# OpenGene/repaq

Hardware: AMD Instinct MI355X
Metric: raw FASTQ MB/s encode+decode (higher is better)
Workload: dtype u8; 1 GPU; configs[2]: synthetic NovaSeq PE150 two files (-i/-I), 2 x 4.01 GB FASTQ (fqgen profile 1, 11200000 pairs, seed 3, N 20 ppm), -k 1000, encode + decode; chunks_per_gpu=3360, parity=unchecked (checked with --full)

## Files before the change

### repaq_amd/csrc/enc/gather_tiles.h

```cpp
#pragma once
#define G2_CAP 23552u
#define G2_SE_OK 1
#define G2_CNT 256u
struct __attribute__((packed, aligned(1))) GU16g { uint32_t a, b, c, d; };
__device__ __forceinline__ void pack4_codes(uint32_t w, uint32_t& code, uint32_t& nb, uint32_t& bad) {
    const uint32_t idx = (w >> 1) & 0x03030303u;
    const uint32_t ok = eq_bytes_full(__builtin_amdgcn_perm(0u, 0x47544341u, idx), w);
    code = ((__builtin_amdgcn_perm(0u, 0x00020301u, idx) & ok) * 0x01041040u) >> 24;
    nb = 0; bad = 0;
    if (ok != 0xFFFFFFFFu) { const uint32_t isn = eq_bytes_full(w, 0x4E4E4E4Eu); nb = ((isn & 0x01010101u) * 0x01020408u) >> 24;
            bad = (((~ok & ~isn) & 0x01010101u) * 0x01020408u) >> 24; }
}
__device__ __forceinline__ void pack4_codes_rc(uint32_t w, uint32_t& code, uint32_t& nb) {
    const uint32_t u = w & 0xDFDFDFDFu, idx = (u >> 1) & 0x03030303u;
    const uint32_t ok = eq_bytes_full(__builtin_amdgcn_perm(0u, 0x47544341u, idx), u);
    code = ((__builtin_amdgcn_perm(0u, 0x03010002u, idx) & ok) * 0x01041040u) >> 24;
    nb = ((~ok & 0x01010101u) * 0x01020408u) >> 24;
}
__device__ __forceinline__ bool pack16_fast(const uint32_t (&w)[4], uint32_t& code) {
    uint32_t diff = 0; code = 0;
#pragma unroll
    for (int i = 0; i < 4; i++) {
        const uint32_t idx = (w[i] >> 1) & 0x03030303u;
        diff |= __builtin_amdgcn_perm(0u, 0x47544341u, idx) ^ w[i];
        code |= ((__builtin_amdgcn_perm(0u, 0x00020301u, idx) * 0x01041040u) >> 24) << (8 * i);
    }
    return diff == 0;
}
__device__ __forceinline__ uint32_t g2_rev2x16(uint32_t v) {
    v = bswap32(v); v = ((v >> 4) & 0x0F0F0F0Fu) | ((v & 0x0F0F0F0Fu) << 4); return ((v >> 2) & 0x33333333u) | ((v & 0x33333333u) << 2);
}
struct G2Geo { uint32_t a00, a01, end0, end1, base1; };
struct G2Read { bool on, rc; uint32_t len, qsrc, ssrc, qpos, ld, gi; };
struct G2Bound { uint32_t l0, l1, q; };
struct G2MRaw { uint4 lo4; uint32_t pg; };
#ifdef RFQ_SIMT_EMULATION
__device__ __forceinline__ uint32_t ld_uniform(const uint32_t* p) { return *p; }
#else
__device__ __forceinline__ uint32_t ld_uniform(const uint32_t* p) { return *(const __attribute__((address_space(4))) uint32_t*)(uintptr_t)p; }
#endif
__device__ __forceinline__ G2Bound g2_bound(const Text& T, bool two, const uint32_t* __restrict__ pq, uint32_t r) {
    G2Bound b;
    if (two) { const size_t k = 4 * (size_t)(r >> 1); b.l0 = ld_uniform(T.lo[0] + k); b.l1 = ld_uniform(T.lo[1] + k); }
    else { b.l0 = ld_uniform(T.lo[0] + 4 * (size_t)r); b.l1 = 0u; }
    b.q = ld_uniform(pq + r);
    return b;
}
__device__ __forceinline__ G2Geo g2_geo(const G2Bound& b, const G2Bound& e, bool two) {
    G2Geo g; g.a00 = b.l0 & ~15u; g.end0 = e.l0; g.a01 = two ? b.l1 & ~15u : 0u; g.end1 = two ? e.l1 : 0u;
    g.base1 = two ? (((g.end0 - g.a00 + 15u) & ~15u) + 16u) : 0u;
    return g;
}
__device__ __forceinline__ void g2_stage1(const uint8_t* __restrict__ fq, uint32_t n, uint32_t a0, uint32_t end, uint4* l4, uint32_t tid) {
    const uint32_t nb = end - a0, ng = (nb + 15u) / 16u;
    const uint8_t* src = fq + a0;
    const uint32_t nfull = (uint64_t)a0 + 16ull * ng <= (uint64_t)n ? ng : ng - 1u;
    for (uint32_t i = tid; i < nfull; i += blockDim.x)
        __builtin_amdgcn_global_load_lds((const __attribute__((address_space(1))) void*)(src + 16 * (size_t)i),
                (__attribute__((address_space(3))) void*)(l4 + (i - (tid & 63u))), 16, 0, 0);
    if (nfull < ng && tid == 0) { uint8_t* const bytes = (uint8_t*)l4;
            for (uint32_t k = 0; k < 16 && a0 + 16 * nfull + k < n; k++) bytes[16 * nfull + k] = src[16 * (size_t)nfull + k]; }
}
__device__ __forceinline__ void g2_stage(const Text& T, bool two, const G2Geo& g, uint4* buf4, uint32_t tid) {
    g2_stage1(T.fq[0], T.n[0], g.a00, g.end0, buf4, tid);
    if (two) g2_stage1(T.fq[1], T.n[1], g.a01, g.end1, buf4 + g.base1 / 16, tid);
}
__device__ __forceinline__ G2MRaw g2_mraw(const Text& T, const uint32_t* __restrict__ pq, uint32_t cur, uint32_t j, uint32_t cnt) {
    G2MRaw r; r.lo4 = make_uint4(0, 0, 0, 0); r.pg = 0;
    if (j < cnt) { const uint32_t gi = cur + j; int s_; uint32_t r_; read_loc(T, gi, s_, r_); r.lo4 = *(const uint4*)(t_lo(T, s_) + 4 * (size_t)r_); r.pg = pq[gi]; }
    return r;
}
__device__ __forceinline__ G2Read g2_read(const Text& T, const G2MRaw& r, const G2Geo& g, uint32_t f, uint32_t pq0, bool il, uint32_t cur, uint32_t j, uint32_t cnt) {
    G2Read m; m.on = j < cnt; m.rc = false; m.len = m.qsrc = m.ssrc = m.qpos = m.ld = 0; m.gi = cur + j;
    if (m.on) {
        const uint32_t gi = cur + j; int s_; uint32_t r_; read_loc(T, gi, s_, r_);
        const uint32_t lb = s_ ? g.base1 : 0u, a = s_ ? g.a01 : g.a00;
        m.len = r.lo4.z - 1u - r.lo4.y; m.ssrc = lb + (r.lo4.y - a); m.qsrc = lb + (r.lo4.w - a);
        m.qpos = r.pg - pq0; m.ld = (r.pg >> 4) + gi;
        m.rc = il && ((gi - f) & 1u);
    }
    return m;
}
__device__ __forceinline__ void g2_bases(const uint8_t* s_text, const G2Read& m, uint32_t part, uint32_t P, uint32_t* __restrict__ lpk, uint16_t* __restrict__ lnb,
        uint8_t* __restrict__ rflag, uint8_t* __restrict__ rn) {
    const uint32_t ng = (m.len + 15u) >> 4;
    for (uint32_t gi = part; gi < ng; gi += P) {
        uint32_t w[4], code = 0, nbits = 0;
        const uint32_t nv0 = m.len - 16u * gi;
        const bool tail = nv0 < 16u && m.len >= 16u; const uint32_t tsh = tail ? 16u - nv0 : 0u;
        auto blank = [&](uint32_t from, uint32_t to) { for (uint32_t k = from; k < to; k++) { uint32_t& x = w[k >> 2]; const uint32_t sh = 8u * (k & 3u);
                x = (x & ~(0xFFu << sh)) | (0x41u << sh); } };
        if (!m.rc) {
            lds_get16(s_text, m.ssrc + (tail ? m.len - 16u : 16u * gi), w);
            if (nv0 < 16u && !tail) blank(nv0, 16u);
            if (!pack16_fast(w, code)) {
                uint32_t bad = 0; code = 0;
#pragma unroll
                for (int i = 0; i < 4; i++) { uint32_t c4, n4, b4; pack4_codes(w[i], c4, n4, b4); code |= c4 << (8 * i); nbits |= n4 << (4 * i); bad |= b4 << (4 * i); }
                if (bad) rflag[m.gi] = 1;
            }
        } else {
            lds_get16(s_text, tail ? m.ssrc : m.ssrc + m.len - 16u * gi - 16u, w);
            if (nv0 < 16u && !tail) blank(0u, 16u - nv0);
            if (pack16_fast(w, code)) code = ~g2_rev2x16(code);
            else {
                const uint32_t x0 = bswap32(w[3]), x1 = bswap32(w[2]), x2 = bswap32(w[1]), x3 = bswap32(w[0]); w[0] = x0; w[1] = x1; w[2] = x2; w[3] = x3; code = 0;
#pragma unroll
                for (int i = 0; i < 4; i++) { uint32_t c4, n4; pack4_codes_rc(w[i], c4, n4); code |= c4 << (8 * i); nbits |= n4 << (4 * i); }
            }
        }
        code >>= 2u * tsh; nbits >>= tsh;
        if (nv0 < 16u) { code &= (1u << (2u * nv0)) - 1u; nbits &= (1u << nv0) - 1u; }
        lpk[m.ld + gi] = code; lnb[m.ld + gi] = (uint16_t)nbits;
        if (nbits) rn[m.gi] = 1;
    }
}
__device__ __forceinline__ void g2_compose(const uint8_t* s_text, const G2Read& m, uint32_t part, uint32_t P, uint8_t* qd, uint32_t* __restrict__ lpk,
        uint16_t* __restrict__ lnb, uint8_t* __restrict__ rflag, uint8_t* __restrict__ rn, QualCount& qc) {
    if (!m.on) return;
    {
        const uint32_t n = m.len; uint8_t* const o = qd + m.qpos; const bool rc = m.rc;
        if (n >= 16u) {
            const uint32_t ng = (n + 15u) >> 4;
            for (uint32_t gi = part; gi < ng; gi += P) {
                uint32_t p0 = 16u * gi, dup = 0; if (p0 + 16u > n) { dup = p0 + 16u - n; p0 = n - 16u; }
                uint32_t w[4]; lds_get16(s_text, rc ? m.qsrc + n - p0 - 16u : m.qsrc + p0, w);
                if (rc) { const uint32_t x0 = bswap32(w[3]), x1 = bswap32(w[2]), x2 = bswap32(w[1]), x3 = bswap32(w[0]); w[0] = x0; w[1] = x1; w[2] = x2; w[3] = x3; }
                { GU16g v; v.a = w[0]; v.b = w[1]; v.c = w[2]; v.d = w[3]; *(GU16g*)(o + p0) = v; }
                if (!dup) qc.group(m.qpos + p0, w[0], w[1], w[2], w[3]);
                else for (uint32_t k = dup; k < 16u; k++) qc(m.qpos + p0 + k, (uint8_t)(w[k >> 2] >> (8u * (k & 3u))));
            }
        } else for (uint32_t i = part; i < n; i += P) { const uint8_t q = s_text[rc ? m.qsrc + n - 1u - i : m.qsrc + i]; o[i] = q; qc(m.qpos + i, q); }
    }
    g2_bases(s_text, m, part, P, lpk, lnb, rflag, rn);
}
#define G2_REFN 256u
#define G2_REFS 128u
struct G2Ref { uint32_t nl, n1l, n2o, len, stl, lane, tile, nb, tb; int s; };
struct G2Acc { uint32_t bits, fail; };
__device__ __forceinline__ bool lane_bytes_eq(const uint8_t* tx, uint32_t a, uint32_t b, uint32_t n, bool on) {
    bool eq = true;
    for (uint32_t o = 0; __any(on && eq && o < n); o += 16u) {
        if (on && eq && o < n) {
            uint32_t p0 = o, v = n - o; if (v < 16u && n >= 16u) { p0 = n - 16u; v = 16u; }
// ... 54 lines not shown
        for (int p = 0; p < 4; p++) { uint32_t w[4]; lds_get16(tx, nsrc + 16u * (uint32_t)p, w); const uint4 q = make_uint4(w[0], w[1], w[2], w[3]);
                c[p] = eq_mask16c(q, 0x3A3A3A3Au); sp_[p] = eq_mask16c(q, 0x20202020u); }
        const unsigned long long keep = !on ? 0ull : (nl >= 64u ? ~0ull : (1ull << nl) - 1ull);
        Cm = ((((unsigned long long)(c[2] | (c[3] << 16))) << 32) | (c[0] | (c[1] << 16))) & keep;
        Sm = ((((unsigned long long)(sp_[2] | (sp_[3] << 16))) << 32) | (sp_[0] | (sp_[1] << 16))) & keep;
    }
    const uint32_t sp = ctz64_or64(Sm);
    unsigned long long cb = sp < 64u ? Cm & ((1ull << sp) - 1ull) : Cm;
    const uint32_t k = (uint32_t)__popcll(cb);
    uint32_t cpos[8];
#pragma unroll
    for (int i = 1; i <= 7; i++) { cpos[i] = ctz64_or64(cb); cb &= cb - 1ull; }
    const bool at7 = cpos[7] < 64u, at_sp = !at7 && sp < 64u;
    const bool undecided = on && !at7 && !at_sp && nl > 64u;
    uint32_t ok = 0, n1l = nl, n2o = nl, lane_v = 0, tile_v = 0, x_v = 0, y_v = 0;
    if (on && (at7 || (at_sp && k >= 4u))) {
        ok = 1; n2o = at7 ? cpos[7] : sp;
        const bool k4 = at_sp && k == 4u, k5 = at_sp && k == 5u;
        n1l = k4 ? cpos[4] : cpos[3];
        const uint32_t ls = (k4 ? cpos[4] : cpos[3]) + 1u, le = k4 ? sp : cpos[4];
        lane_v = g2_atoi(tx, nsrc + ls, le - ls) & 0xFFu;
        if (k >= 5u) { const uint32_t ts = (k5 ? cpos[5] : cpos[4]) + 1u, te = k5 ? sp : cpos[5]; tile_v = g2_atoi(tx, nsrc + ts, te - ts) & 0xFFFFu; }
        if (k >= 6u) x_v = g2_atoi(tx, nsrc + cpos[5] + 1u, cpos[6] - cpos[5] - 1u);
        if (at7) y_v = g2_atoi(tx, nsrc + cpos[6] + 1u, cpos[7] - cpos[6] - 1u);
        else if (k == 6u) y_v = g2_atoi(tx, nsrc + cpos[6] + 1u, sp - cpos[6] - 1u);
    }
    if (__any(undecided)) {
        if (undecided) { const Meta m = dev_parse_name(tx + nsrc, nl); ok = m.ok; n1l = m.name1_len; n2o = m.name2_off; lane_v = m.lane; tile_v = m.tile; x_v = m.x;
                y_v = m.y; }
    }
    if (on) { R.name1_len[gi] = n1l; R.name2_off[gi] = n2o; R.x[gi] = x_v; R.y[gi] = y_v; R.tile[gi] = (uint16_t)tile_v; R.lane[gi] = (uint8_t)lane_v;
            R.ok[gi] = (uint8_t)ok; }
    const uint32_t n2l = nl - n2o, n2l0 = r0.nl - r0.n2o;
    const uint8_t* g0n = t_fq(T, r0.s) + r0.nb; const uint8_t* g0s = t_fq(T, r0.s) + r0.tb;
    const bool st_eq = g2_eq_ref(tx, tsrc, refs, G2_REFS, g0s, 0u, r0.stl, tl, on && tl == r0.stl);
    const bool n1_eq = g2_eq_ref(tx, nsrc, refn, G2_REFN, g0n, 0u, r0.nl, n1l, on && n1l == r0.n1l);
    const bool n2_eq = g2_eq_ref(tx, nsrc + n2o, refn, G2_REFN, g0n, r0.n2o, r0.nl, n2l, on && n2l == n2l0);
    const uint32_t pn = wave_shr1(nsrc, 0u), pnl = wave_shr1(nl, 0u), pn2o = wave_shr1(n2o, 0u), plane = wave_shr1(lane_v, 0u), ptile = wave_shr1(tile_v,
            0u), px = wave_shr1(x_v, 0u), py = wave_shr1(y_v, 0u);
    const uint32_t rel = gi - f; const bool odd = on && can0 && (rel & 1u);
    bool fa = false;
    if (__any(odd)) {
        const uint32_t pn2l = pnl - pn2o; const bool same_len = odd && pn2l == n2l;
        if (odd && !same_len) fa = true;
        const uint32_t ma = pn + pn2o, mb = nsrc + n2o; const bool small = same_len && n2l <= 16u, big = same_len && !small;
        if (small && n2l) {
            uint32_t x[4], y[4]; lds_get16(tx, ma, x); lds_get16(tx, mb, y);
            if (dch != 0u && dpos < n2l) {
                const uint32_t sh = 8u * (dpos & 3u);
#pragma unroll
                for (int q = 0; q < 4; q++) if ((dpos >> 2) == (uint32_t)q) x[q] = (x[q] & ~(0xFFu << sh)) | (dch << sh);
            }
            unsigned long long dl = (((unsigned long long)(x[1] ^ y[1])) << 32) | (x[0] ^ y[0]), dh = (((unsigned long long)(x[3] ^ y[3])) << 32) | (x[2] ^ y[2]);
            if (n2l < 16u) { dl &= n2l >= 8u ? ~0ull : (1ull << (8u * n2l)) - 1ull; dh &= n2l > 8u ? (1ull << (8u * (n2l - 8u))) - 1ull : 0ull; }
            if (dl | dh) fa = true;
        }
        if (__any(big)) {
            if (!lane_bytes_eq(tx, ma, mb, dpos < n2l ? dpos : n2l, big)) fa = true;
            if (big && dpos < n2l) { if ((dch != 0u ? dch : (uint32_t)tx[ma + dpos]) != (uint32_t)tx[mb + dpos]) fa = true; }
            if (!lane_bytes_eq(tx, ma + dpos + 1u, mb + dpos + 1u, n2l > dpos + 1u ? n2l - dpos - 1u : 0u, big && dpos + 1u < n2l)) fa = true;
        }
    }
    if (on) {
        uint32_t b = 0;
        if (sl == r0.len) b |= 1u << 0;
        if (n1l == r0.n1l) b |= 1u << 1;
        if (n2l == n2l0) b |= 1u << 2;
        if (tl == r0.stl) b |= 1u << 3;
        if (tl == r0.stl && st_eq) b |= 1u << 4;
        if (lane_v == r0.lane) b |= 1u << 5;
        if (tile_v == r0.tile) b |= 1u << 6;
        if (n1l == r0.n1l && n1_eq) b |= 1u << 7;
        const bool e2 = n2l == n2l0 && n2_eq;
        if (e2) b |= 1u << 8;
        if (e2 || (rel & 1u)) b |= 1u << 9;
        acc.bits &= b;
        R.eq2[gi] = e2 ? 1 : 0;
        if (odd) {
            const bool fb = plane != lane_v || ptile != tile_v || px != x_v || py != y_v;
            if (fa || fb) { const uint32_t key = (rel << 1) | (fa ? 0u : 1u); if (key < acc.fail) acc.fail = key; }
        }
    }
}
#define G2_PLANES 5u
#define G2_PLANE_EXC 4u
#define G2_RARE_LIST 255u
struct G2Planes { uint32_t* planes; uint64_t pstride; uint32_t pw, nd; uint32_t* rare; };
__device__ __forceinline__ void g2_rare_or(uint32_t* __restrict__ gpl, uint64_t pstride, uint32_t* __restrict__ rare_c, uint32_t plane, uint32_t pos) {
    const uint32_t old = atomicOr(&gpl[(size_t)plane * pstride + (pos >> 5)], 1u << (pos & 31u));
    if (old == 0u) { const uint32_t k = atomicAdd(rare_c, 1u); if (k < G2_RARE_LIST) rare_c[1u + k] = (plane << 28) | (pos >> 5); }
}
__device__ __forceinline__ void g2_quals_masks(const uint8_t* tx, const G2Read& m, uint32_t part, uint32_t P, uint32_t* pl, uint32_t pw, uint32_t wbase, uint32_t nd,
                                               uint32_t pat0, uint32_t pat1, uint32_t pat2, uint32_t patm, const DevHeader* __restrict__ D, uint8_t* qd, uint32_t* __restrict__ gpl, uint64_t pstride,
                                               uint32_t* __restrict__ segm_c, int* __restrict__ segc_c, uint32_t n_seg, uint32_t* __restrict__ rare_c) {
    if (!m.on) return;
    const uint32_t n = m.len, ng = (n + 15u) >> 4; const bool rc = m.rc;
    for (uint32_t gi = part; gi < ng; gi += P) {
        const uint32_t p0 = 16u * gi, nv = n - p0;
        uint32_t w[4]; lds_get16(tx, rc ? m.qsrc + n - p0 - 16u : m.qsrc + p0, w);
        if (rc) { const uint32_t x0 = bswap32(w[3]), x1 = bswap32(w[2]), x2 = bswap32(w[1]), x3 = bswap32(w[0]); w[0] = x0; w[1] = x1; w[2] = x2; w[3] = x3; }
        const uint32_t valid = nv >= 16u ? 0xFFFFu : (1u << nv) - 1u;
        const uint4 q = make_uint4(w[0], w[1], w[2], w[3]);
        const uint32_t bit = m.qpos + p0 - wbase, wi = bit >> 5, sh = bit & 31u;
        uint32_t known = eq_mask16c(q, patm);
        auto plane = [&](uint32_t d, uint32_t pat) {
            const uint32_t mv = eq_mask16c(q, pat); known |= mv;
            const unsigned long long x = (unsigned long long)(mv & valid) << sh;
            if ((uint32_t)x) atomicOr(&pl[d * pw + wi], (uint32_t)x);
            if ((uint32_t)(x >> 32)) atomicOr(&pl[d * pw + wi + 1u], (uint32_t)(x >> 32));
        };
        if (nd > 0u) plane(0u, pat0);
        if (nd > 1u) plane(1u, pat1);
        if (nd > 2u) plane(2u, pat2);
        uint32_t rest = ~known & valid;
        while (rest) {
            const uint32_t k = (uint32_t)__ffs((int)rest) - 1u; rest &= rest - 1u;
            const uint32_t ww = k < 8u ? (k < 4u ? w[0] : w[1]) : (k < 12u ? w[2] : w[3]), pos = m.qpos + p0 + k, b = (ww >> (8u * (k & 3u))) & 0xFFu;
            const uint32_t j = D->stream_of[b];
            if (j < 4u && j < D->n_normal) { const size_t si = (size_t)j * n_seg + pos / PC_SEG_POS; g2_rare_or(gpl, pstride, rare_c, j, pos); atomicAdd(&segm_c[si], 1u);
                    atomicMax(&segc_c[si], (int)pos); }
            else { qd[pos] = (uint8_t)b; g2_rare_or(gpl, pstride, rare_c, G2_PLANE_EXC, pos); atomicAdd(&segm_c[(size_t)EXC_SLOT * n_seg + pos / PC_SEG_POS], 1u); }
        }
    }
}
__device__ __forceinline__ void g2_flush_masks(uint32_t* pl, uint32_t pw, uint32_t nd, uint32_t dense3 , uint32_t* s_carry, uint32_t* __restrict__ gpl, uint64_t pstride,
                                               uint32_t gw0, uint32_t nw, bool carry, bool or_first, bool or_last,
                                               size_t seg_index0 , uint32_t n_seg, uint32_t* __restrict__ segm, int* __restrict__ segc) {
    const uint32_t tid = threadIdx.x, seg0 = (gw0 << 5) / PC_SEG_POS;
    for (uint32_t d = 0; d < nd; d++) {
        const uint32_t v = (dense3 >> (8u * d)) & 0xFFu;
        uint32_t c01 = 0; int l0 = -1, l1 = -1;
        for (uint32_t i = tid; i < nw; i += blockDim.x) {
            const uint32_t x = pl[d * pw + i]; pl[d * pw + i] = 0u;
            const bool last = i + 1u == nw;
            if (last && carry) { s_carry[d] = x; continue; }
            const uint32_t gw = gw0 + i; uint32_t* const dst = gpl + (size_t)v * pstride + gw;
            if ((i == 0u && or_first) || (last && or_last)) { if (x) atomicOr(dst, x); } else *dst = x;
            if (x) { const uint32_t sg = ((gw << 5) / PC_SEG_POS) - seg0; const int lp = (int)((gw << 5) + 31u - (uint32_t)__clz((int)x));
                     c01 += (uint32_t)__popc(x) << (16u * sg); if (sg) { if (lp > l1) l1 = lp; } else if (lp > l0) l0 = lp; }
        }
        if (!carry && tid == 0) s_carry[d] = 0u;
        c01 = wave_sum(c01); l0 = wave_max(l0); l1 = wave_max(l1);
        if ((tid & 63u) == 0 && c01) {
            const size_t si = seg_index0 + (size_t)v * n_seg + seg0;
            if (c01 & 0xFFFFu) { atomicAdd(&segm[si], c01 & 0xFFFFu); atomicMax(&segc[si], l0); }
            if ((c01 >> 16) && seg0 + 1u < n_seg) { atomicAdd(&segm[si + 1u], c01 >> 16); atomicMax(&segc[si + 1u], l1); }
        }
    }
}
__global__ void k_mask_bounds(const uint32_t* __restrict__ pq, const uint32_t* __restrict__ first, const uint64_t* __restrict__ qbase, uint32_t* __restrict__ planes,
        uint64_t pstride, const DevHeader* __restrict__ D, uint32_t nd, uint32_t bx,
                              const uint32_t* __restrict__ only) {
    const uint32_t c = blockIdx.x; if (only && !only[c]) return;
    const uint32_t f = first[c], e = first[c + 1], pq0 = pq[f];
    uint32_t per = ((e - f) + bx - 1) / bx; per = (per + 1u) & ~1u;
    for (uint32_t b = 1u + threadIdx.x; b < bx; b += blockDim.x) {
        const uint32_t gs = f + b * per; if (gs >= e) break;
        const uint32_t w = (uint32_t)(qbase[c] >> 5) + ((pq[gs] - pq0) >> 5);
        for (uint32_t d = 0; d < nd; d++) planes[(size_t)D->dense[d] * pstride + w] = 0u;
    }
}
template <bool MASKS, int PAIRED = -1> __global__ void __launch_bounds__(256, 6) k_gather2(Text T_, ReadTab R, const uint32_t* __restrict__ first, const uint64_t* __restrict__ qbase,
                                                 const DevHeader* __restrict__ D, uint8_t* __restrict__ qcat, uint32_t* __restrict__ lpk, uint16_t* __restrict__ lnb, uint8_t* __restrict__ rflag,
                                                 uint8_t* __restrict__ rn, uint32_t* __restrict__ segm, int* __restrict__ segc, uint32_t n_seg, uint32_t kshift,
                                                 uint32_t* __restrict__ cbits, uint32_t* __restrict__ cfail, const uint32_t* __restrict__ only, uint32_t text4, G2Planes M) {
    Text T = T_; if (PAIRED >= 0) T.paired = PAIRED;
    constexpr bool PE = PAIRED != 0;
    RFQ_DYN_SHARED(uint4, g2_lds);
    __shared__ uint32_t sh[MASKS ? 1 : G2_CNT]; __shared__ int sh_last[MASKS ? 1 : G2_CNT]; __shared__ uint8_t s_slot[MASKS ? 16 : 256];
            __shared__ uint32_t s_r0[8], s_carry[4];
    const uint32_t REFN = (text4 - 1u) * 16u, REFS = REFN + G2_REFN + 16u;
    uint32_t* const pl = (uint32_t*)(g2_lds + text4 + (G2_REFN + G2_REFS + 32u) / 16u);
    const uint32_t c = blockIdx.y;
    const bool redo = only != nullptr;
    if (redo && !only[c]) return;
    const uint32_t tid = threadIdx.x;
    const uint32_t* __restrict__ pq = R.pq;
    const uint32_t nn_s = D->n_normal < NPOS_SLOT ? D->n_normal : NPOS_SLOT, nslot = nn_s + 1u;
    uint32_t nrep = 1;
    if (!MASKS) {
        for (uint32_t i = tid; i < G2_CNT; i += blockDim.x) { sh[i] = 0; sh_last[i] = -1; }
        while (nrep < 16u && 4u * nrep * nslot <= G2_CNT) nrep *= 2u;
        for (uint32_t i = tid; i < 256; i += blockDim.x) { const uint32_t j = D->stream_of[i]; s_slot[i] = (uint8_t)(j < nn_s ? j : nn_s); }
    } else {
        for (uint32_t i = tid; i < M.nd * M.pw; i += blockDim.x) pl[i] = 0u;
        if (tid < 4u) s_carry[tid] = 0u;
    }
    const uint32_t f = first[c], e = first[c + 1];
    const bool two = PE && T.paired == 1, can0 = PE && T.paired != 0 && D->support_interleaved != 0, il = can0 && !redo;
    const uint32_t dpos = D->name2_diff_pos, dch = D->name2_diff_char;
    uint8_t* const qd = qcat + qbase[c]; const uint32_t pq0 = pq[f];
    uint32_t per = ((e - f) + gridDim.x - 1) / gridDim.x; per = (per + 1u) & ~1u;
    const uint32_t gs = f + blockIdx.x * per, ge = gs + per < e ? gs + per : e;
    const uint32_t K = 1u << kshift, pshift = 8u - kshift, P = 1u << pshift;
    const uint32_t jj = tid >> pshift, j = ((jj << 1) & (K - 1u)) | (jj >> (kshift - 1u)), part = tid & (P - 1u);
    QualCount qc; qc.cnt = sh; qc.last = sh_last; qc.slot = s_slot; qc.major = D->major & 0xFFu; qc.seg0 = 0; qc.nslot = nslot; qc.rep = tid & (nrep - 1u);
            qc.hot_ok = D->stream_of[D->major & 0xFFu] == 0xFF;
    const uint32_t nd = MASKS ? M.nd : 0u, dense3 = (uint32_t)D->dense[0] | ((uint32_t)D->dense[1] << 8) | ((uint32_t)D->dense[2] << 16);
    const uint32_t pat0 = (uint32_t)D->normal[dense3 & 0xFFu] * 0x01010101u, pat1 = (uint32_t)D->normal[(dense3 >> 8) & 0xFFu] * 0x01010101u, pat2 = (uint32_t)D->normal[(dense3 >> 16) & 0xFFu] * 0x01010101u, patm = (D->major & 0xFFu) * 0x01010101u;
    uint32_t* const gpl = M.planes + (MASKS ? (size_t)(qbase[c] >> 5) : (size_t)0);
    uint4* const buf4 = g2_lds + 1; const uint8_t* const tx = (const uint8_t*)buf4;
    G2Ref r0 = {}; G2Acc acc; acc.bits = CF_ALL; acc.fail = 0xFFFFFFFFu;
    const bool parse = !redo && gs < ge;
    if (parse) {
        uint32_t r_; read_loc(T, f, r0.s, r_); const uint32_t* p = t_lo(T, r0.s) + 4 * (size_t)r_;
        const uint32_t p0 = p[0], p1 = p[1], p2 = p[2], p3 = p[3];
        r0.nb = p0; r0.nl = p1 - 1u - p0; r0.len = p2 - 1u - p1; r0.tb = p2; r0.stl = p3 - 1u - p2;
        uint8_t* const wr = (uint8_t*)buf4;
        if (tid < r0.nl) wr[REFN + tid] = t_fq(T, r0.s)[r0.nb + tid];
        if (tid < G2_REFS && tid < r0.stl) wr[REFS + tid] = t_fq(T, r0.s)[r0.tb + tid];
        __syncthreads();
        if (tid == 0) {
            const Meta m0 = r0.nl <= G2_REFN ? dev_parse_name(tx + REFN, r0.nl) : dev_parse_name(t_fq(T, r0.s) + r0.nb, r0.nl);
            s_r0[0] = m0.name1_len; s_r0[1] = m0.name2_off; s_r0[2] = m0.lane; s_r0[3] = m0.tile;
        }
    }
    __syncthreads();
    if (parse) { r0.n1l = s_r0[0]; r0.n2o = s_r0[1]; r0.lane = s_r0[2]; r0.tile = s_r0[3]; }
    uint32_t tix = blockIdx.x + blockIdx.y;
    const uint32_t ntile = gs < ge ? (ge - gs + K - 1u) >> kshift : 0u;
    auto tile_at = [&](uint32_t t_) -> uint32_t { const uint32_t x = gs + (t_ << kshift); return x < ge ? x : ge; };
    G2Bound b0 = g2_bound(T, two, pq, tile_at(0)), b1 = g2_bound(T, two, pq, tile_at(1)), b2 = g2_bound(T, two, pq, tile_at(2));
    G2MRaw mr = g2_mraw(T, pq, gs, j, ntile ? tile_at(1) - gs : 0u);
    if (ntile) g2_stage(T, two, g2_geo(b0, b1, two), buf4, tid);
    for (uint32_t t = 0; t < ntile; t++, tix++) {
        const uint32_t cur = tile_at(t), cnt = tile_at(t + 1u) - cur;
        const G2Geo g = g2_geo(b0, b1, two);
        const G2Read m = g2_read(T, mr, g, f, pq0, il, cur, j, cnt);
        const uint32_t qbeg = b0.q - pq0, qend = b1.q - pq0;
        { const uint32_t ncur = tile_at(t + 1u); mr = g2_mraw(T, pq, ncur, j, tile_at(t + 2u) - ncur); }
        const G2Bound b3 = g2_bound(T, two, pq, tile_at(t + 3u));
        __syncthreads();
        qc.seg0 = qbeg / PC_SEG_POS;
        if (parse && (uint32_t)wave_id() == (tix & 3u)) g2_parse(T, R, tx, REFN, REFS, g, r0, f, cur, cnt, can0, dpos, dch, acc);
        if (MASKS) {
            if (tid < nd && s_carry[tid]) atomicOr(&pl[tid * M.pw], s_carry[tid]);
            g2_quals_masks(tx, m, part, P, pl, M.pw, qbeg & ~31u, nd, pat0, pat1, pat2, patm, D, qd, gpl, M.pstride, segm + (size_t)c * MAX_STREAMS * n_seg,
                    segc + (size_t)c * MAX_STREAMS * n_seg, n_seg, M.rare + (size_t)c * (1u + G2_RARE_LIST));
            g2_bases(tx, m, part, P, lpk, lnb, rflag, rn);
        } else g2_compose(tx, m, part, P, qd, lpk, lnb, rflag, rn, qc);
        __syncthreads();
        if (t + 1u < ntile) g2_stage(T, two, g2_geo(b1, b2, two), buf4, tid);
        if (MASKS) {
            const uint32_t gw0 = qbeg >> 5, nw = ((qend + 31u) >> 5) - gw0; const bool last_tile = cur + cnt >= ge;
            g2_flush_masks(pl, M.pw, nd, dense3, s_carry, gpl, M.pstride, gw0, nw, !last_tile && (qend & 31u) != 0u, cur == gs && gs > f && (qbeg & 31u) != 0u,
                    last_tile && ge < e && (qend & 31u) != 0u,
                           (size_t)c * MAX_STREAMS * n_seg, n_seg, segm, segc);
        } else qual_flush(sh, sh_last, nrep, nslot, qc.seg0, c, nn_s, segm, segc, n_seg);
        b0 = b1; b1 = b2; b2 = b3;
    }
    if (parse) {
        const uint32_t bits = wave_and(acc.bits), fail = wave_min(acc.fail);
        if ((tid & 63u) == 0) { if (bits != CF_ALL) atomicAnd(&cbits[c], bits); if (fail != 0xFFFFFFFFu) atomicMin(&cfail[c], fail); }
    }
}
__device__ __forceinline__ uint32_t dense_mask_of(const DevHeader* __restrict__ D, uint32_t nd) { uint32_t m = 0;
        for (uint32_t d = 0; d < nd; d++) m |= 1u << D->dense[d]; return m; }
__device__ __forceinline__ void k_rare_zero_chunk(uint32_t* __restrict__ planes, uint64_t pstride, uint32_t dense_mask, const uint32_t* __restrict__ pq,
        const uint32_t* __restrict__ first, const uint64_t* __restrict__ qbase, uint32_t c) {
    const uint32_t nw = (pq[first[c + 1]] - pq[first[c]] + 31u) >> 5; const size_t w0 = (size_t)(qbase[c] >> 5);
    for (uint32_t v = 0; v < G2_PLANES; v++) if (!((dense_mask >> v) & 1u)) for (uint32_t i = threadIdx.x; i < nw; i += blockDim.x) planes[(size_t)v * pstride + w0 + i] = 0u;
}
__global__ void k_gather_redo_reset(const uint32_t* __restrict__ only, uint32_t* __restrict__ segm, int* __restrict__ segc, uint32_t n_seg,
                                    uint32_t* __restrict__ xplane, uint64_t pstride, const DevHeader* __restrict__ D, uint32_t nd, const uint32_t* __restrict__ pq, const uint32_t* __restrict__ first, const uint64_t* __restrict__ qbase) {
    const uint32_t c = blockIdx.x; if (!only[c]) return;
    const size_t k = (size_t)c * MAX_STREAMS * n_seg;
    for (uint32_t i = threadIdx.x; i < MAX_STREAMS * n_seg; i += blockDim.x) { segm[k + i] = 0u; segc[k + i] = -1; }
    if (xplane) { k_rare_zero_chunk(xplane, pstride, dense_mask_of(D, nd), pq, first, qbase, c);
            if (threadIdx.x == 0) xplane[(size_t)G2_PLANES * pstride + (size_t)c * (1u + G2_RARE_LIST)] = 0u; }
}
__global__ void k_rare_cleanup(uint32_t* __restrict__ rare, uint32_t* __restrict__ planes, uint64_t pstride, const DevHeader* __restrict__ D, uint32_t nd,
        const uint32_t* __restrict__ pq, const uint32_t* __restrict__ first, const uint64_t* __restrict__ qbase) {
    const uint32_t c = blockIdx.x; uint32_t* const rc = rare + (size_t)c * (1u + G2_RARE_LIST); const uint32_t n = rc[0]; if (!n) return;
    if (n <= G2_RARE_LIST) { const size_t w0 = (size_t)(qbase[c] >> 5); for (uint32_t i = threadIdx.x; i < n; i += blockDim.x) { const uint32_t e = rc[1u + i];
            planes[(size_t)(e >> 28) * pstride + w0 + (e & 0x0FFFFFFFu)] = 0u; } }
    else k_rare_zero_chunk(planes, pstride, dense_mask_of(D, nd), pq, first, qbase, c);
    __syncthreads();
    if (threadIdx.x == 0) rc[0] = 0u;
}
__device__ __forceinline__ uint32_t loose_codes(const uint32_t* __restrict__ lpk, uint32_t ld, uint32_t b) {
    const uint32_t d = ld + (b >> 4), sh = 2u * (b & 15u); const uint32_t lo = lpk[d];
    return sh ? (uint32_t)(((((unsigned long long)lpk[d + 1]) << 32) | lo) >> sh) : lo;
}
__device__ __forceinline__ uint32_t loose_nbits(const uint16_t* __restrict__ lnb, uint32_t ld, uint32_t b) {
    const uint32_t d = ld + (b >> 4), sh = b & 15u; const uint32_t lo = lnb[d];
    return (sh ? ((((uint32_t)lnb[d + 1]) << 16) | lo) >> sh : lo) & 0xFFFFu;
}
#define SP_OWN 4096u
#define SP_EXTRA 8u
#define SP_U 3
struct __attribute__((packed, aligned(4))) SpU8 { uint32_t a, b; };
struct __attribute__((packed, aligned(2))) SpU4 { uint32_t a; };
__global__ void __launch_bounds__(256) k_seqpack(const uint32_t* __restrict__ pq, const uint32_t* __restrict__ sd, const U4* __restrict__ ptot,
        const uint32_t* __restrict__ first, const uint32_t* __restrict__ ilv, const int8_t* __restrict__ ovb,
                                                 const DevHeader* __restrict__ D, const uint64_t* __restrict__ sbase, const uint32_t* __restrict__ lpk, const uint16_t* __restrict__ lnb, const uint8_t* __restrict__ rn,
                                                 uint32_t* __restrict__ spk, uint16_t* __restrict__ snm, uint32_t* __restrict__ ncount, uint32_t* __restrict__ nmap, uint32_t* __restrict__ segm, int* __restrict__ segc, uint32_t n_seg,
                                                 uint32_t rshift) {
    __shared__ uint32_t s_sd[256 + SP_EXTRA + 1], s_ld[256 + SP_EXTRA], s_sk[256 + SP_EXTRA]; __shared__ uint8_t s_own[SP_OWN];
    __shared__ uint8_t s_hn[256 + SP_EXTRA + 8];
    const uint32_t c = blockIdx.y, f = first[c], e = first[c + 1], tid = threadIdx.x;
    const uint32_t ps0 = sd[f], S = ptot[c].d;
    const bool il = ilv[c] != 0, enc = il && (D->flags & H_PE_OVERLAP); const int shift = D->overlap_shift;
    uint32_t* const ok = spk + (size_t)(sbase[c] >> 4); uint16_t* const on = snm + (size_t)(sbase[c] >> 4);
    const uint32_t nshift = nmap_shift(S); uint32_t* const nm = nmap + (size_t)c * NMAP_WORDS;
    const size_t nsi = ((size_t)c * MAX_STREAMS + NPOS_SLOT) * n_seg;
    uint32_t nsum = 0;
    auto skip_of = [&](uint32_t g) -> uint32_t {
        if (enc && ((g - f) & 1u)) { const int ov = (int)ovb[g >> 1] - shift; if (ov > 0) return (uint32_t)ov; }
        return 0u;
    };
    const uint32_t R = 1u << rshift;
    for (uint32_t r0 = f + blockIdx.x * R; r0 < e; r0 += gridDim.x * R) {
        const uint32_t nr = e - r0 < R ? e - r0 : R, nx = e - r0 < R + SP_EXTRA ? e - r0 : R + SP_EXTRA;
        for (uint32_t t = tid; t <= nx; t += blockDim.x) {
            const uint32_t g = r0 + t; s_sd[t] = g < e ? sd[g] - ps0 : S;
            if (t < nx) { s_ld[t] = (pq[g] >> 4) + g; s_sk[t] = skip_of(g); s_hn[t] = rn[g]; } else s_hn[t] = 0;
        }
        __syncthreads();
        const uint32_t kbase = (s_sd[0] + 15u) >> 4, kend = (s_sd[nr] + 15u) >> 4;
        if (tid < nr) { const uint32_t ka = (s_sd[tid] + 15u) >> 4, kb = (s_sd[tid + 1] + 15u) >> 4; for (uint32_t k = ka; k < kb; k++) s_own[k - kbase] = (uint8_t)tid; }
        __syncthreads();
        const uint32_t ndw = kend - kbase;
        for (uint32_t i0 = 0; i0 < ndw; i0 += blockDim.x * SP_U) {
            struct Dw { uint32_t k, need, t1, jj, sh, sh2, take2, n, n2; unsigned long long c, c2; } q[SP_U]; uint32_t nres[SP_U];
#pragma unroll
            for (int u = 0; u < SP_U; u++) nres[u] = 0;
#pragma unroll
            for (int u = 0; u < SP_U; u++) {
                Dw& x = q[u]; x.need = 0; x.take2 = 0; x.k = x.t1 = x.jj = x.sh = x.sh2 = x.n = x.n2 = 0; x.c = x.c2 = 0;
                const uint32_t i = i0 + (uint32_t)u * blockDim.x + tid;
                if (i < ndw) {
                    const uint32_t k = kbase + i, j = s_own[i];
                    const uint32_t B = 16u * k, si = B - s_sd[j], need = S - B < 16u ? S - B : 16u, av = s_sd[j + 1] - B, t1 = need < av ? need : av;
                    const uint32_t b0 = s_sk[j] + si, d = s_ld[j] + (b0 >> 4);
                    x.k = k; x.need = need; x.t1 = t1; x.sh = b0 & 15u; x.jj = j + 1u;
                    { const SpU8 v = *(const SpU8*)(lpk + d); x.c = (((unsigned long long)v.b) << 32) | v.a; x.n = s_hn[j] ? ((const SpU4*)(lnb + d))->a : 0u; }
// ... 104 lines not shown
```

### repaq_amd/csrc/enc/index.h

```cpp
#pragma once
__device__ __forceinline__ uint32_t eq_mask4(uint32_t w, uint32_t pat) {
    uint32_t v = w ^ pat;
    uint32_t t = ~(((v & 0x7F7F7F7Fu) + 0x7F7F7F7Fu) | v | 0x7F7F7F7Fu);
    return (((t >> 7) * 0x00204081u) >> 21) & 0xFu;
}
__device__ __forceinline__ uint32_t eq_flags4(uint32_t w, uint32_t pat) { const uint32_t v = w ^ pat; return ~(((v & 0x7F7F7F7Fu) + 0x7F7F7F7Fu) | v | 0x7F7F7F7Fu); }
__device__ __forceinline__ uint32_t eq_mask8(uint32_t a, uint32_t b, uint32_t pat) {
    return udot4(eq_flags4(b, pat), 0x80402010u, udot4(eq_flags4(a, pat), 0x08040201u, 0u)) >> 7;
}
__device__ __forceinline__ uint32_t eq_mask16c(const uint4& q, uint32_t pat) {
    const uint32_t lo = udot4(eq_flags4(q.y, pat), 0x80402010u, udot4(eq_flags4(q.x, pat), 0x08040201u, 0u));
    const uint32_t hi = udot4(eq_flags4(q.w, pat), 0x80402010u, udot4(eq_flags4(q.z, pat), 0x08040201u, 0u));
    return ((hi << 8) | lo) >> 7;
}
__device__ __forceinline__ uint32_t has_byte16(const uint4& q, uint32_t pat) {
    const uint32_t a = q.x ^ pat, b = q.y ^ pat, c = q.z ^ pat, d = q.w ^ pat;
    return (((a - 0x01010101u) & ~a) | ((b - 0x01010101u) & ~b) | ((c - 0x01010101u) & ~c) | ((d - 0x01010101u) & ~d)) & 0x80808080u;
}
__device__ __forceinline__ uint32_t eq_mask16(const uint4& q, uint32_t pat) {
    return eq_mask4(q.x, pat) | (eq_mask4(q.y, pat) << 4) | (eq_mask4(q.z, pat) << 8) | (eq_mask4(q.w, pat) << 12);
}
__global__ void k_nl_bitmap(const uint8_t* __restrict__ fq, uint32_t n, uint32_t skip, uint64_t* __restrict__ bitmap, uint32_t* __restrict__ blkcnt, DevStatus* st) {
    const uint64_t w = (uint64_t)blockIdx.x * 256 + threadIdx.x;
    const uint64_t base = w * 64;
// ... 31 lines not shown
typedef __attribute__((address_space(1))) unsigned long long nlf_gu64;
__device__ __forceinline__ void nlf_store(unsigned long long* p, unsigned long long v) { __hip_atomic_store((nlf_gu64*)p, v, __ATOMIC_RELAXED, __HIP_MEMORY_SCOPE_AGENT);
        }
__device__ __forceinline__ unsigned long long nlf_load(const unsigned long long* p) { return __hip_atomic_load((nlf_gu64*)p, __ATOMIC_RELAXED, __HIP_MEMORY_SCOPE_AGENT);
        }
__device__ __forceinline__ void nlf_pause() { __builtin_amdgcn_s_sleep(2); }
#endif
template <int NLF_T> __global__ void __launch_bounds__(256) k_line_index(const uint8_t* __restrict__ fq, uint32_t n, uint32_t skip, uint32_t* __restrict__ lo,
        uint32_t lo_cap, unsigned long long* state,
                                                    uint32_t* ticket, uint32_t* total, DevStatus* st) {
    constexpr uint32_t NLF_BYTES = NLF_T * 16384u;
    __shared__ uint32_t s_blk, s_base, s_wave[4];
    if (threadIdx.x == 0) s_blk = atomicAdd(ticket, 1u);
    __syncthreads();
    const uint32_t blk = s_blk;
    const int lane = lane_id(), wv = wave_id();
    const uint64_t wbase = (uint64_t)blk * NLF_BYTES + (uint64_t)wv * (NLF_T * 4096u) + (uint32_t)lane * 64u;
    uint64_t m[NLF_T]; uint32_t incl[NLF_T], tsum[NLF_T]; bool cr = false;
#pragma unroll
    for (int k = 0; k < NLF_T; k++) {
        const uint64_t base = wbase + (uint32_t)k * 4096u;
        uint64_t mk = 0, crm = 0;
        if (base + 64 <= n) {
            const uint4* p = (const uint4*)(fq + base);
#pragma unroll
            for (int q4 = 0; q4 < 4; q4++) { uint4 q = p[q4]; mk |= (uint64_t)eq_mask16c(q, 0x0A0A0A0Au) << (16 * q4); crm |= has_byte16(q, 0x0D0D0D0Du); }
            if (base == 0 && skip && crm) { crm = 0; for (uint32_t i = skip; i < 64; i++) if (fq[i] == '\r') crm = 1ull << 63; }
        } else if (base < n) {
            for (uint32_t i = 0; i < 64 && base + i < n; i++) { uint8_t c = fq[base + i]; if (c == '\n') mk |= 1ull << i; if (c == '\r') crm |= 1ull << i; }
        }
        if (base == 0 && skip) { const uint64_t keep = ~((1ull << skip) - 1ull); mk &= keep; crm &= keep; }
        m[k] = mk; cr |= crm != 0;
    }
    if (__any(cr) && lane == 0) atomicOr(&st->err, (uint32_t)DE_HAS_CR);
    uint32_t wtot = 0;
#pragma unroll
    for (int k = 0; k < NLF_T; k++) { incl[k] = wave_incl_sum<uint32_t>((uint32_t)__popcll(m[k])); tsum[k] = wave_last(incl[k]); wtot += tsum[k]; }
    if (lane == 0) s_wave[wv] = wtot;
    __syncthreads();
    const uint32_t tot = s_wave[0] + s_wave[1] + s_wave[2] + s_wave[3];
    uint32_t wavebase = 0;
    for (int k = 0; k < wv; k++) wavebase += s_wave[k];
    if (threadIdx.x < 64) {
        if (lane == 0) nlf_store(&state[blk], ((blk == 0 ? 2ull : 1ull) << 62) | tot);
        uint32_t before = 0;
        if (blk) {
            int64_t newest = (int64_t)blk - 1;
            for (uint32_t spins = 0;;) {
                const int64_t j = newest - lane;
                const unsigned long long v = j >= 0 ? nlf_load(&state[j]) : (2ull << 62);
                const unsigned long long pm = __ballot((v >> 62) == 2), zm = __ballot((v >> 62) == 0);
                const int fp = pm ? __ffsll((long long)pm) - 1 : 63;
                const unsigned long long need = (2ull << fp) - 1ull;
                if (zm & need) {
                    if (++spins > NLF_SPINS) { if (lane == 0) atomicOr(&st->err, (uint32_t)DE_INDEX_RETRY); break; }
                    nlf_pause(); continue;
                }
                before += wave_sum<uint32_t>(lane <= fp ? (uint32_t)v : 0u);
                if (pm) break;
                newest -= 64;
            }
            if (lane == 0) nlf_store(&state[blk], (2ull << 62) | (unsigned long long)(uint32_t)(before + tot));
        }
        if (lane == 0) {
            s_base = before;
            if ((uint64_t)(blk + 1) * NLF_BYTES >= n) *total = before + tot;
        }
    }
    __syncthreads();
    uint32_t tbase = s_base + wavebase;
    if ((uint64_t)tbase + wtot + 1u > lo_cap) { if (wtot && lane == 0) atomicOr(&st->err, (uint32_t)DE_INDEX_RETRY); }
    else {
#pragma unroll
        for (int k = 0; k < NLF_T; k++) {
            uint64_t mk = m[k]; uint32_t rank = tbase + incl[k] - (uint32_t)__popcll(mk);
            const uint32_t base = (uint32_t)(wbase + (uint32_t)k * 4096u);
            while (mk) { const int b = __ffsll((long long)mk) - 1; mk &= mk - 1; lo[rank + 1] = base + (uint32_t)b + 1u; rank++; }
            tbase += tsum[k];
        }
    }
    if (blk == 0 && threadIdx.x == 0) lo[0] = skip;
}
__global__ void k_index_totals(const uint32_t* __restrict__ tot0, const uint32_t* __restrict__ tot1, const uint8_t* __restrict__ fq0, uint32_t n0, const uint8_t* __restrict__ fq1, uint32_t n1,
                               uint32_t* lo0, uint32_t* lo1, int final_batch, int paired, uint32_t unit_cap, uint32_t guess, DevStatus* st) {
    if (threadIdx.x || blockIdx.x) return;
    uint32_t rec[2] = { 0, 0 };
    for (int s = 0; s < (paired == 1 ? 2 : 1); s++) {
        const uint32_t nl = s ? *tot1 : *tot0, n = s ? n1 : n0; const uint8_t* fq = s ? fq1 : fq0; uint32_t* lo = s ? lo1 : lo0;
        const uint32_t unterm = (final_batch && n > 0 && fq[n - 1] != '\n') ? 1u : 0u;
        if (unterm) lo[nl + 1] = n + 1;
        st->idx_lines[s] = n ? nl + unterm : 0u; rec[s] = n ? (nl + unterm) / 4 : 0u;
    }
    uint32_t units = paired == 0 ? rec[0] : (paired == 1 ? (rec[0] < rec[1] ? rec[0] : rec[1]) : rec[0] / 2);
    if (units > unit_cap) units = unit_cap;
    st->idx_units_true = units; st->idx_units = units < guess ? units : guess;
    if (units > guess) atomicOr(&st->err, (uint32_t)DE_UNITS_GUESS);
}
__global__ void k_line_tail(uint32_t* lo, uint32_t n_newlines, uint32_t n, int unterminated) {
    if (threadIdx.x == 0 && blockIdx.x == 0 && unterminated) lo[n_newlines + 1] = n + 1;
}

#define FQ_BLOCK_BYTES (1u << 20)
struct NormIn { const uint8_t* fq; uint32_t n; uint64_t file_off, file_end; };
__device__ __forceinline__ bool norm_exc(const NormIn& c, uint32_t j) {
    const uint64_t e = c.file_off + j - 1;
    uint64_t bend = (e | (uint64_t)(FQ_BLOCK_BYTES - 1)) + 1; if (bend > c.file_end) bend = c.file_end;
    return !(e + 1 < bend - 1);
}
__device__ __forceinline__ bool norm_state_at(const NormIn& c, uint32_t j) {
    if (j == 0) return false;
    uint32_t k = 0; while (k < 4 && k < j && c.fq[j - 1 - k] == '\n') k++;
    bool st = (k < 4 && j - k > 0) ? c.fq[j - k - 1] == '\r' : false;
    for (uint32_t i = j - k; i < j; i++) { if (st && !norm_exc(c, i)) st = false; else st = true; }
    return st;
}
__global__ void k_norm_classify(NormIn c, uint64_t* __restrict__ tbits, uint64_t* __restrict__ sbits, uint32_t* __restrict__ blk_keep, uint32_t* __restrict__ blk_term) {
    const uint64_t w = (uint64_t)blockIdx.x * 256 + threadIdx.x; const uint64_t base = w * 64;
    uint64_t tm = 0, sm = 0; uint32_t valid = 0;
    if (base < c.n) {
        valid = (uint32_t)(c.n - base < 64 ? c.n - base : 64);
        bool st = norm_state_at(c, (uint32_t)base);
        for (uint32_t i = 0; i < valid; i++) {
            const uint8_t ch = c.fq[base + i];
            if (ch == '\r') { tm |= 1ull << i; st = true; }
            else if (ch == '\n') { if (st && !norm_exc(c, (uint32_t)base + i)) { sm |= 1ull << i; st = false; } else { tm |= 1ull << i; st = true; } }
            else st = false;
        }
        tbits[w] = tm; sbits[w] = sm;
    }
    uint32_t tk, tt; (void)block_excl_sum<uint32_t>(valid - (uint32_t)__popcll(sm), &tk); (void)block_excl_sum<uint32_t>((uint32_t)__popcll(tm), &tt);
    if (threadIdx.x == 0) { blk_keep[blockIdx.x] = tk; blk_term[blockIdx.x] = tt; }
}
__global__ void k_norm_emit(NormIn c, const uint64_t* __restrict__ tbits, const uint64_t* __restrict__ sbits, const uint32_t* __restrict__ keep_base,
        const uint32_t* __restrict__ term_base,
                            uint8_t* __restrict__ out, uint32_t* __restrict__ ot, uint32_t* __restrict__ onx) {
    const uint64_t w = (uint64_t)blockIdx.x * 256 + threadIdx.x; const uint64_t base = w * 64;
    uint64_t tm = 0, sm = 0; uint32_t valid = 0;
    if (base < c.n) { valid = (uint32_t)(c.n - base < 64 ? c.n - base : 64); tm = tbits[w]; sm = sbits[w]; }
    uint32_t kp = keep_base[blockIdx.x] + block_excl_sum<uint32_t>(valid - (uint32_t)__popcll(sm), (uint32_t*)nullptr);
    uint32_t tr = term_base[blockIdx.x] + block_excl_sum<uint32_t>((uint32_t)__popcll(tm), (uint32_t*)nullptr);
    for (uint32_t i = 0; i < valid; i++) {
        if ((sm >> i) & 1ull) continue;
        const bool t = ((tm >> i) & 1ull) != 0;
        out[kp++] = t ? (uint8_t)'\n' : c.fq[base + i];
        if (t) {
            const uint32_t pos = (uint32_t)base + i;
            bool sw = false;
            if (pos + 1 < c.n) sw = i + 1 < 64 ? ((sm >> (i + 1)) & 1ull) != 0 : (sbits[w + 1] & 1ull) != 0;
            ot[tr] = pos; onx[tr] = pos + 1 + (sw ? 1u : 0u); tr++;
        }
    }
}
__global__ void k_norm_tail(uint32_t* ot, uint32_t* onx, uint32_t n_terms, uint32_t n) {
    if (threadIdx.x == 0 && blockIdx.x == 0) { ot[n_terms] = n; onx[n_terms] = n; }
}
```

### repaq_amd/csrc/rfq_api.hip

```cpp
#include "rfq_ctx.h"
#include <cstring>
#include <algorithm>
#include <new>
#include <cstdlib>
#include <string>
#include <cerrno>

extern "C" const char* rfq_version(void) {
#ifdef RFQ_SIMT_EMULATION
    return "rfq_hip 0.1.0 simt-emulation (test build, not a product path)";
#else
    return "rfq_hip 0.1.0 gfx950";
#endif
}

static bool opt_num(const std::string& v, long long lo, long long hi, long long* out) {
    if (v.empty()) return false;
    errno = 0; char* end = nullptr; const long long x = strtoll(v.c_str(), &end, 10);
    if (errno || !end || *end || end == v.c_str() || x < lo || x > hi) return false;
    *out = x; return true;
}
extern "C" int rfq_set_option(rfq_ctx* c, const char* name, const char* value) {
    if (!c || !name) return RFQ_E_ARG;
    const std::string n = name, v = value ? value : ""; const bool set = !v.empty(); const RfqOpts d; long long num = 0;
#define RFQ_OPT_NUM(LO, HI, WHAT) if (set && !opt_num(v, LO, HI, &num)) return rfq_fail(c, RFQ_E_ARG, "%s is " WHAT " (got \"%s\")", name, v.c_str());
    if (n == "RFQ_GATHER") { if (set && v != "old" && v != "tile") return rfq_fail(c, RFQ_E_ARG, "RFQ_GATHER is old or tile"); c->opt.gather_old = v == "old"; }
    else if (n == "RFQ_QUAL") { if (set && v != "bytes" && v != "masks") return rfq_fail(c, RFQ_E_ARG, "RFQ_QUAL is bytes or masks"); c->opt.qual_bytes = v == "bytes"; }
    else if (n == "RFQ_CODER") { if (set && v != "list" && v != "mask") return rfq_fail(c, RFQ_E_ARG, "RFQ_CODER is list or mask");
            c->opt.coder = v == "list" ? 1 : (v == "mask" ? 2 : 0); }
    else if (n == "RFQ_INDEX") { if (set && v != "2pass" && v != "1pass") return rfq_fail(c, RFQ_E_ARG, "RFQ_INDEX is 2pass or 1pass"); c->opt.index_2pass = v == "2pass"; }
    else if (n == "RFQ_IDX_TILES") { if (set && v != "4" && v != "8" && v != "16") return rfq_fail(c, RFQ_E_ARG, "RFQ_IDX_TILES is 4, 8 or 16");
            c->opt.idx_tiles = set ? atoi(v.c_str()) : d.idx_tiles; }
    else if (n == "RFQ_STREAMS") { if (set && v != "1" && v != "2") return rfq_fail(c, RFQ_E_ARG, "RFQ_STREAMS is 1 or 2"); c->opt.one_stream = v == "1"; }
    else if (n == "RFQ_SLICE_BYTES") { RFQ_OPT_NUM(1024, 0xFFFFFFF0ll - 16, "a number of bytes in 1024 .. 2^32 - 32") c->opt.slice_bytes = set ? (size_t)num : 0; }
    else if (n == "RFQ_SLICE_BASES") { RFQ_OPT_NUM(1, 0xFFFFFFF0ll, "a number of bases in 1 .. 2^32 - 16") c->opt.slice_bases = set ? (uint64_t)num : 0; }
    else if (n == "RFQ_WALK") { if (set && v != "exact" && v != "guess") return rfq_fail(c, RFQ_E_ARG, "RFQ_WALK is guess or exact"); c->opt.walk_exact = v == "exact"; }
    else if (n == "RFQ_GW_SHIFT") { RFQ_OPT_NUM(4, 30, "4 .. 30") c->opt.gw_shift = set ? (int)num : d.gw_shift; }
    else if (n == "RFQ_MATERIALISE") { if (set && v != "0" && v != "1") return rfq_fail(c, RFQ_E_ARG, "RFQ_MATERIALISE is 0 or 1"); c->opt.materialise = v == "1"; }
    else if (n == "RFQ_TRACE") { if (set && v != "0" && v != "1") return rfq_fail(c, RFQ_E_ARG, "RFQ_TRACE is 0 or 1"); c->opt.trace = v == "1"; }
    else if (n == "RFQ_G2_PAD") { RFQ_OPT_NUM(0, 150000, "0 .. 150000 bytes of LDS") c->opt.g2_pad = set ? (uint32_t)num : 0u; }
    else if (n == "RFQ_SP_PAD") { RFQ_OPT_NUM(0, 150000, "0 .. 150000 bytes of LDS") c->opt.sp_pad = set ? (uint32_t)num : d.sp_pad; }
    else if (n == "RFQ_POS_SEG") { if (set && v != "1024" && v != "2048") return rfq_fail(c, RFQ_E_ARG, "RFQ_POS_SEG is 1024 or 2048"); c->opt.pos_seg = set ? atoi(v.c_str()) : 0; }
    else if (n == "RFQ_SPEC") { if (set && v != "0" && v != "1") return rfq_fail(c, RFQ_E_ARG, "RFQ_SPEC is 0 or 1"); c->opt.no_spec = v == "0"; }
    else return rfq_fail(c, RFQ_E_ARG, "unknown option %s", name);
#undef RFQ_OPT_NUM
    return RFQ_OK;
}
static const char* const RFQ_OPTION_NAMES[] = { "RFQ_GATHER", "RFQ_QUAL", "RFQ_CODER", "RFQ_INDEX", "RFQ_IDX_TILES", "RFQ_STREAMS", "RFQ_SLICE_BYTES", "RFQ_SLICE_BASES", "RFQ_WALK", "RFQ_GW_SHIFT", "RFQ_MATERIALISE", "RFQ_TRACE", "RFQ_G2_PAD", "RFQ_SP_PAD", "RFQ_POS_SEG", "RFQ_SPEC" };
extern "C" const char* rfq_option_name(int i) { return (i >= 0 && i < (int)(sizeof RFQ_OPTION_NAMES / sizeof RFQ_OPTION_NAMES[0])) ? RFQ_OPTION_NAMES[i] : nullptr; }
extern "C" int rfq_get_option(const rfq_ctx* c, const char* name, char* out, size_t cap) {
    if (!c || !name || !out || !cap) return RFQ_E_ARG;
    const std::string n = name; const RfqOpts& o = c->opt; const RfqOpts d; std::string v;
    if (n == "RFQ_GATHER") v = o.gather_old ? "old" : "";
    else if (n == "RFQ_QUAL") v = o.qual_bytes ? "bytes" : "";
    else if (n == "RFQ_CODER") v = o.coder == 1 ? "list" : (o.coder == 2 ? "mask" : "");
    else if (n == "RFQ_INDEX") v = o.index_2pass ? "2pass" : "";
    else if (n == "RFQ_IDX_TILES") v = o.idx_tiles != d.idx_tiles ? std::to_string(o.idx_tiles) : "";
    else if (n == "RFQ_STREAMS") v = o.one_stream ? "1" : "";
    else if (n == "RFQ_SLICE_BYTES") v = o.slice_bytes ? std::to_string(o.slice_bytes) : "";
    else if (n == "RFQ_SLICE_BASES") v = o.slice_bases ? std::to_string(o.slice_bases) : "";
    else if (n == "RFQ_WALK") v = o.walk_exact ? "exact" : "";
    else if (n == "RFQ_GW_SHIFT") v = o.gw_shift != d.gw_shift ? std::to_string(o.gw_shift) : "";
    else if (n == "RFQ_MATERIALISE") v = o.materialise ? "1" : "";
    else if (n == "RFQ_TRACE") v = o.trace ? "1" : "";
    else if (n == "RFQ_G2_PAD") v = o.g2_pad ? std::to_string(o.g2_pad) : "";
    else if (n == "RFQ_SP_PAD") v = o.sp_pad != d.sp_pad ? std::to_string(o.sp_pad) : "";
    else if (n == "RFQ_POS_SEG") v = o.pos_seg ? std::to_string(o.pos_seg) : "";
    else if (n == "RFQ_SPEC") v = o.no_spec ? "0" : "";
    else return RFQ_E_ARG;
    if (v.size() + 1 > cap) return RFQ_E_NOSPACE;
    memcpy(out, v.c_str(), v.size() + 1);
    return RFQ_OK;
}

extern "C" int rfq_create(rfq_ctx** out, int device_id) {
    if (!out) return RFQ_E_ARG;
    *out = nullptr;
    int n = 0;
    if (hipGetDeviceCount(&n) != hipSuccess || n <= 0) return RFQ_E_NO_DEVICE;
    if (device_id < 0 || device_id >= n) return RFQ_E_NO_DEVICE;
    if (hipSetDevice(device_id) != hipSuccess) return RFQ_E_NO_DEVICE;
    rfq_ctx* c = new (std::nothrow) rfq_ctx();
    if (!c) return RFQ_E_HIP;
    c->device = device_id;
    { int cu = 0; if (hipDeviceGetAttribute(&cu, hipDeviceAttributeMultiprocessorCount, device_id) == hipSuccess && cu > 0) c->n_cu = (uint32_t)cu; }
    if (hipStreamCreate(&c->stream) != hipSuccess) { delete c; return RFQ_E_NO_DEVICE; }
    c->own_stream = true;
    memset(&c->h_hdr, 0, sizeof c->h_hdr);
    for (const char* nm : RFQ_OPTION_NAMES) { const char* v = getenv(nm); if (v && *v && rfq_set_option(c, nm, v) != RFQ_OK) fprintf(stderr, "rfq_hip: ignoring %s=%s (%s)\n", nm, v, c->err.c_str()); }
    c->err.clear();
    *out = c;
    return RFQ_OK;
}

extern "C" void rfq_destroy(rfq_ctx* c) {
    if (!c) return;
    (void)hipSetDevice(c->device);
    (void)hipDeviceSynchronize();
    for (auto& b : c->b) b.release();
    c->d_hdr.release(); c->d_status.release(); c->d_cmp.release(); c->out_img.release(); c->out_fq1.release(); c->out_fq2.release(); c->out_acc.release();
            c->out_acc1.release(); c->out_acc2.release();
    for (auto& b : c->rows_off) b.release();
    for (auto& b : c->rows_txt) b.release();
    c->rows_stat.release(); c->names_blob.release(); c->names_off.release();
    c->timer.destroy();
    if (c->copy) { (void)hipStreamDestroy(c->copy); for (auto& e : c->copy_ev) if (e) (void)hipEventDestroy(e); }
    if (c->own_stream && c->stream) (void)hipStreamDestroy(c->stream);
    if (c->pin) (void)hipHostFree(c->pin);
    if (c->pin_up) (void)hipHostFree(c->pin_up);
    if (c->ev_up) (void)hipEventDestroy(c->ev_up);
    if (c->aux) (void)hipStreamDestroy(c->aux);
    if (c->ev_fork) (void)hipEventDestroy(c->ev_fork);
    if (c->ev_join) (void)hipEventDestroy(c->ev_join);
    if (c->ev_mid) (void)hipEventDestroy(c->ev_mid);
    if (c->aux2) (void)hipStreamDestroy(c->aux2);
    if (c->ev_f) (void)hipEventDestroy(c->ev_f);
    delete c;
}

extern "C" const char* rfq_last_error(const rfq_ctx* c) { return c ? c->err.c_str() : "null context"; }

extern "C" int rfq_set_stream(rfq_ctx* c, void* s) {
    if (!c) return RFQ_E_ARG;
    if (s) {
        if (c->own_stream && c->stream) (void)hipStreamDestroy(c->stream);
        c->stream = (hipStream_t)s; c->own_stream = false;
    } else if (!c->own_stream) {
        if (hipStreamCreate(&c->stream) != hipSuccess) return rfq_fail(c, RFQ_E_HIP, "hipStreamCreate failed");
        c->own_stream = true;
    }
    return RFQ_OK;
}

int rfq_upload_header(rfq_ctx* c, const uint8_t* h, size_t n);

extern "C" int rfq_set_header(rfq_ctx* c, const uint8_t* h, size_t n) {
    if (!c || !h) return RFQ_E_ARG;
    c->err.clear();
    return rfq_upload_header(c, h, n);
}
extern "C" int rfq_get_header(rfq_ctx* c, uint8_t* out, size_t* len) {
    if (!c || !out || !len) return RFQ_E_ARG;
    if (!c->have_hdr) return rfq_fail(c, RFQ_E_STATE, "no header has been made or set on this context");
    memcpy(out, c->h_hdr.bytes, c->h_hdr.len); *len = c->h_hdr.len;
    return RFQ_OK;
}
extern "C" void rfq_clear_header(rfq_ctx* c) { if (c) { c->have_hdr = false; c->hdr_on_device = false; c->new_file(); memset(&c->h_hdr, 0, sizeof c->h_hdr); } }

extern "C" int rfq_last_timings(const rfq_ctx* c, const char** names, float* ms, int cap) {
    if (!c) return 0;
    int n = 0;
// ... 155 lines not shown
```

### repaq_amd/csrc/rfq_common.h

```cpp
#pragma once
#include <hip/hip_runtime.h>
#include <stdint.h>
#include <stddef.h>

#define H_LANE        (1u << 0)
#define H_TILE        (1u << 1)
#define H_X           (1u << 2)
#define H_Y           (1u << 3)
#define H_NAME2       (1u << 4)
#define H_PAIRED      (1u << 5)
#define H_PE_OVERLAP  (1u << 6)
#define H_QUAL_BY_COL (1u << 7)
#define H_DONT_QUAL   (1u << 8)
#define H_N_POS       (1u << 9)
#define C_READ_LEN_SAME   (1u << 0)
#define C_NAME1_LEN_SAME  (1u << 1)
#define C_NAME2_LEN_SAME  (1u << 2)
#define C_STRAND_LEN_SAME (1u << 3)
#define C_LANE_SAME       (1u << 4)
#define C_TILE_SAME       (1u << 5)
#define C_NAME1_SAME      (1u << 6)
#define C_NAME2_SAME      (1u << 7)
#define C_STRAND_SAME     (1u << 8)
#define C_PE_INTERLEAVED  (1u << 9)
#define C_NO_LB           (1u << 10)
#define C_NO_LB_R2        (1u << 11)

#define WAVE 64
#define NL_BLOCK_BYTES 16384u
#define MAX_STREAMS 66
#define NPOS_SLOT 64
#define EXC_SLOT 65

#define DE_HAS_CR          (1u << 0)
#define DE_EMPTY_LINE      (1u << 1)
#define DE_QUAL_SHORT      (1u << 2)
#define DE_BAD_QUAL        (1u << 3)
#define DE_BAD_BASE        (1u << 4)
#define DE_COORD_RANGE     (1u << 5)
#define DE_QUAL_OVERFLOW   (1u << 6)
#define DE_NO_QUAL_BINS    (1u << 7)
#define DE_CORRUPT         (1u << 8)
#define DE_LIST_ALIAS      (1u << 28)
#define DE_E3_RETRY        (1u << 29)
#define DE_INDEX_RETRY     (1u << 30)
#define DE_CORRUPT_OV      (1u << 10)
#define DE_INTERNAL        (1u << 11)
#define DE_SCRATCH_SMALL   (1u << 12)
#define DE_SCRATCHN_SMALL  (1u << 13)
#define DE_NEED_SCAN       (1u << 14)
#define DE_UNITS_GUESS     (1u << 15)
#define DE_TAIL_BLANK      (1u << 9)

struct DevHeader {
    uint8_t  bytes[17 + 255];
    uint32_t len;
    uint32_t flags;
    uint32_t read_len_bytes;
    uint32_t support_interleaved;
    uint32_t name2_diff_pos, name2_diff_char;
    uint32_t n_base_qual;
    int32_t  overlap_shift;
    uint32_t major;
    uint32_t n_normal;
    uint8_t  normal[256];
    uint8_t  stream_of[256];
    uint8_t  is_exception[256];
    uint8_t  dense[4];
    uint32_t dense_valid;
    uint32_t valid;
};

struct DevStatus {
    uint32_t err;
    uint32_t err_read;
    uint64_t err_key;
    uint64_t coord_key;
    uint64_t total_scratch;
    uint64_t total_scratch_n;
    uint64_t image_bound;
    uint32_t n_chunks;
    uint32_t max_chunk_reads;
    uint32_t max_chunk_bases;
    uint32_t n_units_used;
    uint64_t total_image;
    uint64_t total_bases;
    uint32_t first_empty;
    uint32_t max_rec;
    uint32_t unit_bases;
    uint32_t max_len;
    uint32_t idx_lines[2], idx_units_true, idx_units;
};

struct U4 { uint32_t a, b, c, d; };
__device__ __host__ __forceinline__ U4 operator+(const U4& x, const U4& y) { U4 r; r.a = x.a + y.a; r.b = x.b + y.b; r.c = x.c + y.c; r.d = x.d + y.d; return r; }
__device__ __host__ __forceinline__ U4 operator-(const U4& x, const U4& y) { U4 r; r.a = x.a - y.a; r.b = x.b - y.b; r.c = x.c - y.c; r.d = x.d - y.d; return r; }

#ifdef RFQ_SIMT_EMULATION
#define RFQ_DYN_SHARED(type, name) type* const name = (type*)emu::dyn_shared()
#else
#define RFQ_DYN_SHARED(type, name) extern __shared__ type name[]
#endif

__device__ __forceinline__ int lane_id() { return (int)(threadIdx.x & 63u); }
__device__ __forceinline__ int wave_id() { return (int)(threadIdx.x >> 6); }

#ifdef RFQ_SIMT_EMULATION
template <class T> __device__ __forceinline__ T wave_incl_sum(T v) {
    const int l = lane_id();
#pragma unroll
    for (int d = 1; d < WAVE; d <<= 1) { T t = __shfl_up(v, (unsigned)d); if (l >= d) v = t + v; }
    return v;
}
template <class T> __device__ __forceinline__ T wave_incl_max(T v) {
    const int l = lane_id();
#pragma unroll
    for (int d = 1; d < WAVE; d <<= 1) { T t = __shfl_up(v, (unsigned)d); if (l >= d && t > v) v = t; }
    return v;
}
template <class T> __device__ __forceinline__ T wave_sum(T v) {
#pragma unroll
    for (int d = 32; d >= 1; d >>= 1) v += __shfl_xor(v, d);
    return v;
}
template <class T> __device__ __forceinline__ T wave_min(T v) {
#pragma unroll
    for (int d = 32; d >= 1; d >>= 1) { T t = __shfl_xor(v, d); if (t < v) v = t; }
    return v;
}
template <class T> __device__ __forceinline__ T wave_max(T v) {
#pragma unroll
    for (int d = 32; d >= 1; d >>= 1) { T t = __shfl_xor(v, d); if (t > v) v = t; }
    return v;
}
// ... 130 lines not shown
```

### repaq_amd/csrc/rfq_ctx.h

```cpp
#pragma once
#include "rfq_common.h"
#include "../../include/rfq_hip.h"
#include <cstring>
#include <string>
#include <vector>
#include <cstdio>
#include <cstdarg>
#include <algorithm>

struct DBuf {
    void* p = nullptr; size_t cap = 0;
    hipError_t ensure(size_t n) {
        if (n <= cap) return hipSuccess;
        if (p) { (void)hipFree(p); p = nullptr; cap = 0; }
        size_t want = n + n / 4 + 4096;
        hipError_t e = hipMalloc(&p, want);
        if (e != hipSuccess) { p = nullptr; return e; }
        cap = want; return hipSuccess;
    }
    hipError_t ensure_keep(size_t n, size_t keep, hipStream_t s) {
        if (n <= cap) return hipSuccess;
        void* q = nullptr; const size_t want = n + n / 2 + 4096;
        hipError_t e = hipMalloc(&q, want);
        if (e != hipSuccess) return e;
        if (p && keep) { e = hipMemcpyAsync(q, p, keep, hipMemcpyDeviceToDevice, s); if (e == hipSuccess) e = hipStreamSynchronize(s);
                if (e != hipSuccess) { (void)hipFree(q); return e; } }
        if (p) (void)hipFree(p);
        p = q; cap = want; return hipSuccess;
    }
    void release() { if (p) (void)hipFree(p); p = nullptr; cap = 0; }
    template <class T> T* as() const { return (T*)p; }
};

struct StageTimer {
    struct Stage { const char* name; hipEvent_t a, b; };
    std::vector<Stage> stages; size_t used = 0; std::vector<float> ms; std::vector<const char*> names;
    void reset() { used = 0; }
    void begin(const char* name, hipStream_t s) {
        if (used == stages.size()) { Stage st; st.name = name; (void)hipEventCreate(&st.a); (void)hipEventCreate(&st.b); stages.push_back(st); }
        stages[used].name = name; (void)hipEventRecord(stages[used].a, s);
    }
    void end(hipStream_t s) { (void)hipEventRecord(stages[used].b, s); used++; }
    void collect() {
        ms.assign(used, 0.f); names.assign(used, nullptr);
        for (size_t i = 0; i < used; i++) { (void)hipEventElapsedTime(&ms[i], stages[i].a, stages[i].b); names[i] = stages[i].name; }
    }
    void destroy() { for (auto& s : stages) { (void)hipEventDestroy(s.a); (void)hipEventDestroy(s.b); } stages.clear(); }
};
struct StageSums {
    std::vector<std::pair<const char*, float>> v;
    void add(const StageTimer& t) {
        for (size_t i = 0; i < t.names.size(); i++) {
            auto q = std::find_if(v.begin(), v.end(), [&](const std::pair<const char*, float>& e) { return e.first == t.names[i]; });
            if (q == v.end()) v.emplace_back(t.names[i], t.ms[i]); else q->second += t.ms[i];
        }
    }
    void publish(StageTimer& t) const { t.names.clear(); t.ms.clear(); for (auto& q : v) { t.names.push_back(q.first); t.ms.push_back(q.second); } }
};

static inline uint32_t grid_x_for(uint32_t n_chunks, uint32_t tiles_per_chunk, uint32_t slots) {
    uint32_t best = 1; double best_eff = 0.0;
    if (!n_chunks || !slots) return 1;
    for (uint32_t k = 6; k <= 12; k++) {
        uint32_t bx = (uint32_t)(((uint64_t)k * slots + n_chunks / 2) / n_chunks);
        bx = std::max<uint32_t>(1u, std::min<uint32_t>(std::max<uint32_t>(bx, 1u), tiles_per_chunk));
        const double rounds = (double)bx * n_chunks / slots, full = (double)(uint64_t)(rounds + 0.999999), eff = full > 0 ? rounds / full : 0.0;
        if (eff > best_eff + 1e-3) { best = bx; best_eff = eff; }
    }
    return best;
}
struct RfqOpts {
    int  coder = 0;
    bool qual_bytes = false;
    bool gather_old = false;
    bool index_2pass = false;
    int  idx_tiles = 0;
    bool one_stream = false;
    size_t slice_bytes = 0;
    uint64_t slice_bases = 0;
    bool walk_exact = false;
    int  gw_shift = 16;
    bool materialise = false;
    bool trace = false;
    uint32_t g2_pad = 0;
    uint32_t sp_pad = 0;
    bool no_spec = false;
    int  pos_seg = 0;
};
struct rfq_ctx {
    RfqOpts opt;
    bool e3_pieces_failed = false;
    int device = 0; uint32_t n_cu = 256;
    hipStream_t stream = nullptr; bool own_stream = false;
    hipStream_t aux = nullptr; hipEvent_t ev_fork = nullptr, ev_join = nullptr, ev_mid = nullptr;
    hipStream_t aux2 = nullptr; hipEvent_t ev_f = nullptr;
    hipEvent_t ev_ovl = nullptr;
    hipStream_t copy = nullptr; hipEvent_t copy_ev[64] = {}; uint64_t copy_next = 0, copy_done = 0;
    bool aux_ready() {
        if (aux) return true;
        if (hipStreamCreateWithFlags(&aux, hipStreamNonBlocking) != hipSuccess) { aux = nullptr; return false; }
        if (hipEventCreateWithFlags(&ev_fork, hipEventDisableTiming) != hipSuccess || hipEventCreateWithFlags(&ev_join, hipEventDisableTiming) != hipSuccess ||
            hipEventCreateWithFlags(&ev_mid, hipEventDisableTiming) != hipSuccess) return false;
        if (hipStreamCreateWithFlags(&aux2, hipStreamNonBlocking) != hipSuccess) { aux2 = nullptr; return false; }
        if (hipEventCreateWithFlags(&ev_f, hipEventDisableTiming) != hipSuccess) return false;
        if (hipEventCreateWithFlags(&ev_ovl, hipEventDisableTiming) != hipSuccess) return false;
        return true;
    }
    std::string err;
    uint8_t* pin = nullptr; size_t pin_cap = 0, pin_used = 0;
    struct Pend { void* host; size_t off, n; }; std::vector<Pend> pend;
    hipError_t fetch(void* host, const void* dev, size_t n, hipStream_t s) {
        if (!n) return hipSuccess;
        if (!pin) { if (hipHostMalloc((void**)&pin, 1 << 16, 0) != hipSuccess) { pin = nullptr; (void)hipGetLastError(); } else pin_cap = 1 << 16; }
        const size_t off = (pin_used + 15) & ~(size_t)15;
        if (!pin || off + n > pin_cap) return hipMemcpyAsync(host, dev, n, hipMemcpyDeviceToHost, s);
        pend.push_back(Pend{ host, off, n }); pin_used = off + n;
        return hipMemcpyAsync(pin + off, dev, n, hipMemcpyDeviceToHost, s);
    }
    hipError_t fetch_sync(hipStream_t s) {
        const hipError_t e = hipStreamSynchronize(s);
        if (e == hipSuccess) for (const Pend& q : pend) memcpy(q.host, pin + q.off, q.n);
        pend.clear(); pin_used = 0;
        return e;
    }
    DBuf d_hdr;
    DevHeader h_hdr; bool have_hdr = false;
    bool hdr_on_device = false; uint8_t* pin_up = nullptr; hipEvent_t ev_up = nullptr; bool ev_up_pending = false;
    DBuf d_status; DevStatus h_status;
    DBuf d_cmp;
    DBuf b[120];
    DBuf out_img, out_fq1, out_fq2, out_acc, out_acc1, out_acc2;
    double rec_per_byte = 0.0; bool lazy_block = false;
    bool retried_room = false;
    bool mixed_lengths = false;
    bool dense_ok = false;
    void new_file() { dense_ok = false; e3_pieces_failed = false; mixed_lengths = false; }
    bool qplane_dirty = true;
    uint32_t qplane_nd = 0, qplane_mask = 0;
    size_t qplane_stride = 0;
    DBuf rows_off[2], rows_stat, rows_txt[2];
    DBuf names_blob, names_off;
    std::vector<uint64_t> chunk_off;
    std::vector<uint64_t> scan_end[2];
    StageTimer timer;
};

static inline int rfq_fail(rfq_ctx* c, int code, const char* fmt, ...) {
    char buf[1024]; va_list ap; va_start(ap, fmt); vsnprintf(buf, sizeof buf, fmt, ap); va_end(ap);
    if (c) c->err = buf;
    return code;
}
#define HIPCHK(ctx, call) do { hipError_t e_ = (call); if (e_ != hipSuccess) return rfq_fail(ctx, RFQ_E_HIP, "%s failed: %s", #call, hipGetErrorString(e_)); } while (0)
#define KCHK(ctx, what) do { hipError_t e_ = hipGetLastError(); if (e_ != hipSuccess) return rfq_fail(ctx, RFQ_E_HIP, "launch of %s failed: %s", what, hipGetErrorString(e_)); } while (0)

#define SCAN_TPB 256
#define SCAN_ITEMS 8
#define SCAN_TILE (SCAN_TPB * SCAN_ITEMS)

template <class T> __global__ void k_scan_reduce(const T* __restrict__ in, T* __restrict__ partial, uint64_t n, const uint32_t* __restrict__ skip) {
    if (skip && *skip) return;
    const uint64_t base = (uint64_t)blockIdx.x * SCAN_TILE + (uint64_t)threadIdx.x;
    T v[SCAN_ITEMS];
#pragma unroll
    for (int i = 0; i < SCAN_ITEMS; i++) v[i] = base + (uint64_t)i * SCAN_TPB < n ? in[base + (uint64_t)i * SCAN_TPB] : T();
    T acc = T();
#pragma unroll
    for (int i = 0; i < SCAN_ITEMS; i++) acc = acc + v[i];
    T tot; (void)block_excl_sum<T>(acc, &tot);
    if (threadIdx.x == 0) partial[blockIdx.x] = tot;
}
template <class T> __global__ void k_scan_partials(T* __restrict__ partial, uint32_t nb, T* __restrict__ grand, const uint32_t* __restrict__ skip) {
    if (skip && *skip) return;
    const uint32_t K = (nb + SCAN_TPB - 1) / SCAN_TPB, i0 = threadIdx.x * K, i1 = i0 + K < nb ? i0 + K : nb;
    T acc = T();
    for (uint32_t i = i0; i < i1; i++) acc = acc + partial[i];
    T tot; T run = block_excl_sum<T>(acc, &tot);
    for (uint32_t i = i0; i < i1; i++) { const T v = partial[i]; partial[i] = run; run = run + v; }
    if (threadIdx.x == 0 && grand) *grand = tot;
}
template <class T> __global__ void k_scan_apply(const T* __restrict__ in, T* __restrict__ out, const T* __restrict__ partial, uint64_t n, int write_total, const uint32_t* __restrict__ skip) {
    if (skip && *skip) return;
    const uint64_t base = (uint64_t)blockIdx.x * SCAN_TILE + (uint64_t)threadIdx.x * SCAN_ITEMS;
    T v[SCAN_ITEMS]; T acc = T();
    for (int i = 0; i < SCAN_ITEMS; i++) { v[i] = base + i < n ? in[base + i] : T(); acc = acc + v[i]; }
    T tot; T ex = block_excl_sum<T>(acc, &tot);
    T run = partial[blockIdx.x] + ex;
    for (int i = 0; i < SCAN_ITEMS; i++) { if (base + i < n) out[base + i] = run; run = run + v[i]; }
    if (write_total && base < n && base + SCAN_ITEMS >= n) out[n] = run;
}
#define SCAN_SMALL 16384u
template <class T> __global__ void k_scan_small(const T* in, T* out, uint32_t n, int write_total, const uint32_t* __restrict__ skip) {
    if (skip && *skip) return;
    const uint32_t K = (n + SCAN_TPB - 1) / SCAN_TPB, i0 = threadIdx.x * K, i1 = i0 + K < n ? i0 + K : n;
    T acc = T();
    for (uint32_t i = i0; i < i1; i++) acc = acc + in[i];
    T tot; T run = block_excl_sum<T>(acc, &tot);
    for (uint32_t i = i0; i < i1; i++) { const T v = in[i]; out[i] = run; run = run + v; }
    if (write_total && threadIdx.x == 0) out[n] = tot;
}
template <class T> static inline void scan_exclusive(hipStream_t s, const T* in, T* out, uint64_t n, T* tmp, int write_total, const uint32_t* skip = nullptr) {
    if (n == 0) { if (write_total) (void)hipMemsetAsync(out, 0, sizeof(T), s); return; }
    if (n <= SCAN_SMALL) { hipLaunchKernelGGL((k_scan_small<T>), dim3(1), dim3(SCAN_TPB), 0, s, in, out, (uint32_t)n, write_total, skip); return; }
    const uint32_t nb = (uint32_t)((n + SCAN_TILE - 1) / SCAN_TILE);
    hipLaunchKernelGGL((k_scan_reduce<T>), dim3(nb), dim3(SCAN_TPB), 0, s, in, tmp, n, skip);
    hipLaunchKernelGGL((k_scan_partials<T>), dim3(1), dim3(SCAN_TPB), 0, s, tmp, nb, (T*)nullptr, skip);
    hipLaunchKernelGGL((k_scan_apply<T>), dim3(nb), dim3(SCAN_TPB), 0, s, in, out, (const T*)tmp, n, write_total, skip);
}

#define CLEAR_MAX 8
struct ClearList { uint32_t* p[CLEAR_MAX]; uint64_t words[CLEAR_MAX]; uint32_t val[CLEAR_MAX]; uint32_t n;
    bool add(void* p_, size_t bytes, uint32_t v) { if (n >= CLEAR_MAX) return false; p[n] = (uint32_t*)p_; words[n] = (bytes + 3) / 4; val[n] = v; n++; return true; } };
template <int UNUSED> __global__ void k_clear_list(ClearList z) {
    const uint64_t t0 = (uint64_t)blockIdx.x * blockDim.x + threadIdx.x, NT = (uint64_t)gridDim.x * blockDim.x;
    for (uint32_t r = 0; r < z.n; r++) {
        uint32_t* const p = z.p[r]; const uint32_t v = z.val[r]; const uint64_t n4 = z.words[r] >> 2;
        for (uint64_t i = t0; i < n4; i += NT) ((uint4*)p)[i] = make_uint4(v, v, v, v);
        for (uint64_t i = (n4 << 2) + t0; i < z.words[r]; i += NT) p[i] = v;
    }
}
// ... 5 lines not shown
```

### repaq_amd/csrc/rfq_encode.hip

```cpp
#include "rfq_ctx.h"
#include "rfq_encode_kernels.h"
#include <algorithm>
#include <cstring>
#include <cstdlib>
#include <cstddef>

enum EncBuf {
    B_BITMAP0 = 0, B_BITMAP1, B_BLK0, B_BLK1, B_LO0, B_LO1, B_SCANTMP,
    B_LEN, B_N1LEN, B_N2OFF, B_X, B_Y, B_TILE, B_LANE, B_OK, B_CHUNK, B_STORED, B_EQ2, B_PQ, B_PV, B_PVIN,
    B_ULEN, B_P, B_MINMAX, B_FIRST, B_CFLAGS, B_IL, B_HIST, B_NCOUNT, B_SCAP, B_SOFF, B_SSIZE, B_XSIZE, B_YSIZE, B_QBASE, B_SBASE,
    B_IMGSIZE, B_IMGOFF, B_CTOTAL, B_CBASE, B_LAYOUT, B_HSTATS, B_OVB, B_OVRAW, B_QCAT, B_SCAT, B_SCRATCH, B_XS, B_YS, B_SEGB, B_SEGC,
    B_NORM0, B_NORM1, B_OT0, B_OT1, B_ONX0, B_ONX1, B_TBITS, B_SBITS, B_NKEEP, B_NTERM, B_NMAP, B_ADJ, B_PINFO, B_SEGM, B_LPK, B_LNB, B_SPK, B_SNM, B_RFLAG, B_SCANTMP2, B_CTOTALN, B_CBASEN, B_SCRATCHN, B_PTOT, B_QPLANE, B_SEGD, B_SEGS, B_SD, B_RN, B_ENC_END
};

static_assert(B_ENC_END <= 80, "encode buffers must stay below the decode buffer indices of rfq_ctx::b");

static int fetch_bytes(rfq_ctx* ctx, const uint8_t* d, size_t n, std::string& out) {
    out.resize(n);
    if (n) HIPCHK(ctx, hipMemcpy(&out[0], d, n, hipMemcpyDeviceToHost));
    return RFQ_OK;
}
static int fetch_line(rfq_ctx* ctx, const Text& T, uint32_t g, int k, std::string& out) {
    int s = 0; uint32_t r = g; if (T.paired == 1) { s = (int)(g & 1u); r = g >> 1; }
    uint32_t lo2[2];
    HIPCHK(ctx, hipMemcpy(lo2, T.lo[s] + 4 * (size_t)r + k, 8, hipMemcpyDeviceToHost));
    return fetch_bytes(ctx, T.fq[s] + lo2[0], lo2[1] - 1 - lo2[0], out);
}

int rfq_upload_header(rfq_ctx* c, const uint8_t* h, size_t n) {
    if (n < 17) return rfq_fail(c, RFQ_E_FORMAT, "Not a valid repaq file!");
    if (h[8] != 2) return rfq_fail(c, RFQ_E_FORMAT, "The data is encoded by different version of repaq, please try repaq v%.5s. \nSee: https://github.com/OpenGene/repaq/releases", (const char*)h + 3);
    const size_t len = 17u + h[16];
    if (n < len) return rfq_fail(c, RFQ_E_FORMAT, "Not a valid repaq file!");
    if (h[0] != 'R' || h[1] != 'F' || h[2] != 'Q') return rfq_fail(c, RFQ_E_FORMAT, "Not a valid repaq file!");
    HIPCHK(c, hipSetDevice(c->device));
    HIPCHK(c, c->d_hdr.ensure(sizeof(DevHeader)));
    DevHeader tmp; memset(&tmp, 0, sizeof tmp); memcpy(tmp.bytes, h, len); hdr_derive(&tmp);
    const bool same = c->have_hdr && c->hdr_on_device && c->h_hdr.len == tmp.len && !memcmp(c->h_hdr.bytes, tmp.bytes, tmp.len);
    if (!same) {
        if (!c->pin_up) { if (hipHostMalloc((void**)&c->pin_up, sizeof(DevHeader), 0) != hipSuccess) { c->pin_up = nullptr; (void)hipGetLastError(); } }
        if (c->pin_up) {
            if (c->ev_up_pending) { HIPCHK(c, hipEventSynchronize(c->ev_up)); c->ev_up_pending = false; }
            if (!c->ev_up) HIPCHK(c, hipEventCreateWithFlags(&c->ev_up, hipEventDisableTiming));
            memcpy(c->pin_up, &tmp, sizeof tmp);
            HIPCHK(c, hipMemcpyAsync(c->d_hdr.p, c->pin_up, sizeof tmp, hipMemcpyHostToDevice, c->stream));
            HIPCHK(c, hipEventRecord(c->ev_up, c->stream)); c->ev_up_pending = true;
        } else { HIPCHK(c, hipMemcpyAsync(c->d_hdr.p, &tmp, sizeof tmp, hipMemcpyHostToDevice, c->stream)); HIPCHK(c, hipStreamSynchronize(c->stream)); }
        c->h_hdr = tmp; c->hdr_on_device = true;
    }
    c->have_hdr = true; c->new_file();
    return RFQ_OK;
}

struct NormMap { const uint32_t* ot[2]; const uint32_t* onx[2]; size_t orig_n[2]; };
#define RFQ_NEED_NORM 1
#define RFQ_RETRY_ROOM 3

static int normalize_stream(rfq_ctx* ctx, const uint8_t* fq, size_t n, uint64_t file_off, bool final, int s, NormMap& nm, const uint8_t** out, size_t* out_n) {
    hipStream_t S = ctx->stream; DBuf* B = ctx->b;
    nm.orig_n[s] = n; nm.ot[s] = nm.onx[s] = nullptr; *out = nullptr; *out_n = 0;
    if (n == 0) return RFQ_OK;
    const uint64_t nwords = (n + 63) / 64; const uint32_t nblk = (uint32_t)((nwords + 255) / 256);
    HIPCHK(ctx, B[B_TBITS].ensure(nwords * 8 + 64)); HIPCHK(ctx, B[B_SBITS].ensure(nwords * 8 + 64));
    HIPCHK(ctx, B[B_NKEEP].ensure(((size_t)nblk + 2) * 4)); HIPCHK(ctx, B[B_NTERM].ensure(((size_t)nblk + 2) * 4));
    HIPCHK(ctx, B[B_SCANTMP].ensure(std::max<size_t>(1024, ((size_t)nblk / SCAN_TILE + 2) * 16)));
    NormIn in; in.fq = fq; in.n = (uint32_t)n; in.file_off = file_off; in.file_end = final ? file_off + n : ~0ull;
    hipLaunchKernelGGL(k_norm_classify, dim3(nblk), dim3(256), 0, S, in, B[B_TBITS].as<uint64_t>(), B[B_SBITS].as<uint64_t>(), B[B_NKEEP].as<uint32_t>(),
            B[B_NTERM].as<uint32_t>());
    KCHK(ctx, "k_norm_classify");
    scan_exclusive<uint32_t>(S, B[B_NKEEP].as<uint32_t>(), B[B_NKEEP].as<uint32_t>(), nblk, B[B_SCANTMP].as<uint32_t>(), 1);
    scan_exclusive<uint32_t>(S, B[B_NTERM].as<uint32_t>(), B[B_NTERM].as<uint32_t>(), nblk, B[B_SCANTMP].as<uint32_t>(), 1);
    uint32_t keep = 0, terms = 0;
    HIPCHK(ctx, ctx->fetch(&keep, B[B_NKEEP].as<uint32_t>() + nblk, 4, S));
    HIPCHK(ctx, ctx->fetch(&terms, B[B_NTERM].as<uint32_t>() + nblk, 4, S));
    HIPCHK(ctx, ctx->fetch_sync(S));
    HIPCHK(ctx, B[B_NORM0 + s].ensure((size_t)keep + 64)); HIPCHK(ctx, B[B_OT0 + s].ensure(((size_t)terms + 4) * 4));
            HIPCHK(ctx, B[B_ONX0 + s].ensure(((size_t)terms + 4) * 4));
    hipLaunchKernelGGL(k_norm_emit, dim3(nblk), dim3(256), 0, S, in, (const uint64_t*)B[B_TBITS].as<uint64_t>(), (const uint64_t*)B[B_SBITS].as<uint64_t>(),
                       (const uint32_t*)B[B_NKEEP].as<uint32_t>(), (const uint32_t*)B[B_NTERM].as<uint32_t>(), B[B_NORM0 + s].as<uint8_t>(), B[B_OT0 + s].as<uint32_t>(), B[B_ONX0 + s].as<uint32_t>());
    hipLaunchKernelGGL(k_norm_tail, dim3(1), dim3(64), 0, S, B[B_OT0 + s].as<uint32_t>(), B[B_ONX0 + s].as<uint32_t>(), terms, (uint32_t)n);
    KCHK(ctx, "k_norm_emit");
    nm.ot[s] = B[B_OT0 + s].as<uint32_t>(); nm.onx[s] = B[B_ONX0 + s].as<uint32_t>();
    *out = B[B_NORM0 + s].as<uint8_t>(); *out_n = keep;
    return RFQ_OK;
}
#define RFQ_AGAIN_LAZY 2
#define RFQ_AGAIN_ENDED 4
struct EncAgain { uint32_t unit_cap = ~0u; bool ended = false; };
struct EncBatch {
    const rfq_encode_args* a; const NormMap* nm; const uint32_t* skip; bool scan_only, ended, fin, is_pe; uint32_t unit_cap; int nstreams; const uint8_t* fq[2]; size_t nbytes[2]; Text T; DevStatus* dst; DevStatus hs;
    uint64_t orig_n(int s) const { return nm ? nm->orig_n[s] : nbytes[s]; }
};
struct EncCut {
    bool lazy; uint32_t guess_units, nlines[2], nrec[2], n_units, n_reads, n_chunks, cap_chunks, units_used, reads_used, max_reads, max_rec, max_len, max_chunk_bases; uint64_t total_bases;
};
struct EncTables {
    ReadTab R; ChunkTab C; Layout* L; DevHeader* D; int8_t* ovb; int16_t* ovraw; uint32_t *cbits, *cfail, *redo; void* scantmp;
    size_t nr, nc, nsb, catbytes; uint32_t n_seg; uint32_t *segb, *segm; int* segc; uint64_t *ctot, *cbase, *ctot_n, *cbase_n;
    uint8_t* qcat; uint32_t* spk; uint16_t* snm; uint32_t* qplane; uint8_t *scratch, *scratch_n, *xs, *ys, *img; uint64_t img_cap, hdr_bytes;
};
struct EncForm { bool fast; uint32_t kshift; bool make_header, hdr_aside, masks, coder_list; uint32_t nqg; bool aux_chain, coder_waits; };
struct AuxGuard { rfq_ctx* c; bool armed; ~AuxGuard() { if (armed) (void)hipStreamSynchronize(c->aux); } };
template <class T> static hipError_t table(DBuf& d, size_t bytes, T*& p) { const hipError_t e = d.ensure(bytes); p = (T*)d.p; return e; }
static int empty_result(rfq_ctx* ctx, rfq_encode_result* res) { ctx->chunk_off.assign(1, 0); res->h_chunk_off = ctx->chunk_off.data(); return RFQ_OK; }
static hipError_t fresh_status(rfq_ctx* ctx, EncBatch& b) {
    memset(&b.hs, 0, sizeof b.hs); b.hs.err_key = ~0ull; b.hs.coord_key = ~0ull; b.hs.first_empty = ~0u;
    return hipMemcpyAsync(b.dst, &b.hs, sizeof b.hs, hipMemcpyHostToDevice, ctx->stream);
}
static uint64_t consumed_of(const EncBatch& b, int s, uint64_t v) { const uint64_t lim = b.orig_n(s); if (v > lim) v = lim; return b.nm ? v : v - b.skip[s]; }

static int enc_index(rfq_ctx* ctx, EncBatch& b, EncCut& cut) {
    hipStream_t S = ctx->stream; DBuf* B = ctx->b;
    ctx->timer.begin("index", S);
    uint32_t nblk[2] = { 0, 0 }; uint64_t nwords[2] = { 0, 0 };
    for (int s = 0; s < b.nstreams; s++) { nwords[s] = (b.nbytes[s] + 63) / 64; nblk[s] = (uint32_t)((nwords[s] + 255) / 256); }
    int idx_tiles = ctx->opt.idx_tiles ? ctx->opt.idx_tiles : NLF_TILES;
    if (idx_tiles != 4 && idx_tiles != 8 && idx_tiles != 16) idx_tiles = NLF_TILES;
    uint32_t nidx[2] = { 0, 0 };
    for (int s = 0; s < b.nstreams; s++) nidx[s] = (uint32_t)((b.nbytes[s] + idx_tiles * 16384u - 1) / (idx_tiles * 16384u));
    uint32_t n_newlines[2] = { 0, 0 }; uint8_t lastbyte[2] = { '\n', '\n' };
    bool one_pass = !ctx->opt.index_2pass;
    const bool lazy_allowed = !ctx->lazy_block; ctx->lazy_block = false;
    bool lazy = one_pass && lazy_allowed && ctx->rec_per_byte > 0.0 && !ctx->mixed_lengths && b.unit_cap == ~0u && !b.ended;
    uint32_t guess_units = 0;
    if (lazy) {
        double g = 1e300;
        for (int s = 0; s < b.nstreams; s++) g = std::min(g, (double)b.nbytes[s] * ctx->rec_per_byte * 1.03 + 64.0);
        if (b.a->paired == RFQ_PE_INTERLEAVED) g *= 0.5;
        if (g > 2.0e9 || g < 1.0) lazy = false; else guess_units = (uint32_t)g;
        for (int s = 0; s < b.nstreams; s++) if (!nblk[s]) lazy = false;
    }
    if (one_pass) {
        size_t cap[2] = { 0, 0 };
        for (int s = 0; s < b.nstreams; s++) {
            if (!nblk[s]) continue;
            cap[s] = std::max(B[B_LO0 + s].cap / 4, b.nbytes[s] / 16 + 4096);
            HIPCHK(ctx, B[B_LO0 + s].ensure(cap[s] * 4));
            HIPCHK(ctx, B[B_BLK0 + s].ensure((size_t)nidx[s] * 8 + 64));
            HIPCHK(ctx, hipMemsetAsync(B[B_BLK0 + s].p, 0, (size_t)nidx[s] * 8 + 64, S));
            unsigned long long* state = B[B_BLK0 + s].as<unsigned long long>();
            uint32_t* tt = (uint32_t*)(state + nidx[s]);
            const uint32_t lo_cap = (uint32_t)std::min<size_t>(cap[s] - 4, 0xFFFFFFF0u);
            auto kern = idx_tiles == 16 ? k_line_index<16> : (idx_tiles == 4 ? k_line_index<4> : k_line_index<8>);
            hipLaunchKernelGGL(kern, dim3(nidx[s]), dim3(256), 0, S, b.fq[s], (uint32_t)b.nbytes[s], b.skip[s], B[B_LO0 + s].as<uint32_t>(), lo_cap, state, tt, tt + 1, b.dst);
            KCHK(ctx, "k_line_index");
            if (lazy) continue;
            HIPCHK(ctx, ctx->fetch(&n_newlines[s], tt + 1, 4, S));
            HIPCHK(ctx, ctx->fetch(&lastbyte[s], b.fq[s] + b.nbytes[s] - 1, 1, S));
        }
        if (lazy) {
            const uint32_t* t0 = (const uint32_t*)(B[B_BLK0].as<unsigned long long>() + nidx[0]) + 1;
            const uint32_t* t1 = b.nstreams == 2 ? (const uint32_t*)(B[B_BLK1].as<unsigned long long>() + nidx[1]) + 1 : t0;
            hipLaunchKernelGGL(k_index_totals, dim3(1), dim3(64), 0, S, t0, t1, b.fq[0], (uint32_t)b.nbytes[0], b.fq[1], (uint32_t)b.nbytes[1], B[B_LO0].as<uint32_t>(),
                               b.nstreams == 2 ? B[B_LO1].as<uint32_t>() : (uint32_t*)nullptr, b.a->final ? 1 : 0, (int)b.a->paired, b.unit_cap, guess_units, b.dst);
            KCHK(ctx, "k_index_totals");
        } else {
            HIPCHK(ctx, ctx->fetch(&b.hs, b.dst, sizeof b.hs, S));
            HIPCHK(ctx, ctx->fetch_sync(S));
        }
        if (!lazy && (b.hs.err & DE_INDEX_RETRY)) {
            one_pass = false;
            HIPCHK(ctx, fresh_status(ctx, b));
            HIPCHK(ctx, hipStreamSynchronize(S));
            n_newlines[0] = n_newlines[1] = 0;
        }
    }
    if (!one_pass) {
        ctx->timer.end(S); ctx->timer.begin("index_2pass", S);
        size_t scantmp = 1024;
        for (int s = 0; s < b.nstreams; s++) {
            HIPCHK(ctx, B[B_BITMAP0 + s].ensure(nwords[s] * 8 + 64));
            HIPCHK(ctx, B[B_BLK0 + s].ensure(((size_t)nblk[s] + 2) * 4));
            scantmp = std::max(scantmp, ((size_t)nblk[s] / SCAN_TILE + 2) * 16);
        }
        HIPCHK(ctx, B[B_SCANTMP].ensure(scantmp));
        for (int s = 0; s < b.nstreams; s++) {
            if (!nblk[s]) continue;
            hipLaunchKernelGGL(k_nl_bitmap, dim3(nblk[s]), dim3(256), 0, S, b.fq[s], (uint32_t)b.nbytes[s], b.skip[s], B[B_BITMAP0 + s].as<uint64_t>(),
                    B[B_BLK0 + s].as<uint32_t>(), b.dst);
            KCHK(ctx, "k_nl_bitmap");
            scan_exclusive<uint32_t>(S, B[B_BLK0 + s].as<uint32_t>(), B[B_BLK0 + s].as<uint32_t>(), nblk[s], B[B_SCANTMP].as<uint32_t>(), 1);
        }
        for (int s = 0; s < b.nstreams; s++) {
            if (!nblk[s]) continue;
            HIPCHK(ctx, ctx->fetch(&n_newlines[s], B[B_BLK0 + s].as<uint32_t>() + nblk[s], 4, S));
            HIPCHK(ctx, ctx->fetch(&lastbyte[s], b.fq[s] + b.nbytes[s] - 1, 1, S));
        }
        HIPCHK(ctx, ctx->fetch(&b.hs, b.dst, sizeof b.hs, S));
        HIPCHK(ctx, ctx->fetch_sync(S));
    }
    if (!lazy && (b.hs.err & DE_HAS_CR)) return b.nm ? rfq_fail(ctx, RFQ_E_HIP, "internal: '\\r' in normalised text") : RFQ_NEED_NORM;
    cut.nlines[0] = cut.nlines[1] = cut.nrec[0] = cut.nrec[1] = 0;
    for (int s = 0; s < b.nstreams && !lazy; s++) {
        const int unterm = b.a->final && b.nbytes[s] > 0 && lastbyte[s] != '\n';
        cut.nlines[s] = n_newlines[s] + (unterm ? 1u : 0u); cut.nrec[s] = cut.nlines[s] / 4;
        if (!one_pass || !nblk[s]) HIPCHK(ctx, B[B_LO0 + s].ensure(((size_t)cut.nlines[s] + 4) * 4));
        if (nblk[s]) {
            if (!one_pass) hipLaunchKernelGGL(k_line_offsets, dim3(nblk[s]), dim3(256), 0, S, B[B_BITMAP0 + s].as<uint64_t>(), B[B_BLK0 + s].as<uint32_t>(),
                    (uint32_t)b.nbytes[s], b.skip[s], B[B_LO0 + s].as<uint32_t>());
            hipLaunchKernelGGL(k_line_tail, dim3(1), dim3(64), 0, S, B[B_LO0 + s].as<uint32_t>(), n_newlines[s], (uint32_t)b.nbytes[s], unterm);
            KCHK(ctx, "k_line_offsets");
        }
    }
    ctx->timer.end(S);
    if (lazy) { ctx->timer.begin("lazy_index", S); ctx->timer.end(S); }
    cut.lazy = lazy; cut.guess_units = guess_units;
    Text& T = b.T; memset(&T, 0, sizeof T);
    for (int s = 0; s < 2; s++) { T.fq[s] = b.fq[s]; T.n[s] = (uint32_t)b.nbytes[s]; T.lo[s] = s < b.nstreams ? B[B_LO0 + s].as<uint32_t>() : nullptr;
            T.ot[s] = b.nm && s < b.nstreams ? b.nm->ot[s] : nullptr; }
    T.paired = b.a->paired; T.upr = b.a->paired == RFQ_SE ? 1u : 2u;
    return RFQ_OK;
}
static int enc_cut(rfq_ctx* ctx, EncBatch& b, EncCut& cut, EncTables& t, rfq_encode_result* res, EncAgain* again) {
    hipStream_t S = ctx->stream; DBuf* B = ctx->b;
    uint32_t n_units = b.a->paired == RFQ_SE ? cut.nrec[0] : (b.a->paired == RFQ_PE_TWO_FILES ? std::min(cut.nrec[0], cut.nrec[1]) : cut.nrec[0] / 2);
    if (n_units > b.unit_cap) n_units = b.unit_cap;
    if (cut.lazy) n_units = cut.guess_units;
    uint32_t n_reads = n_units * b.T.upr; b.T.n_reads = n_reads;
    const uint32_t* const nu = cut.lazy ? &b.dst->idx_units : (const uint32_t*)nullptr;
    if (n_units == 0) return empty_result(ctx, res);
    ctx->timer.begin("lens+cut", S);
    const size_t nr = t.nr = (size_t)n_reads + 2;
    HIPCHK(ctx, table(B[B_LEN], nr * 4, t.R.len)); HIPCHK(ctx, table(B[B_N1LEN], nr * 4, t.R.name1_len)); HIPCHK(ctx, table(B[B_N2OFF], nr * 4, t.R.name2_off)); HIPCHK(ctx, table(B[B_X], nr * 4, t.R.x));
    HIPCHK(ctx, table(B[B_Y], nr * 4, t.R.y)); HIPCHK(ctx, table(B[B_TILE], nr * 2, t.R.tile)); HIPCHK(ctx, table(B[B_LANE], nr, t.R.lane)); HIPCHK(ctx, table(B[B_OK], nr, t.R.ok)); HIPCHK(ctx, table(B[B_CHUNK], nr * 4, t.R.chunk));
    HIPCHK(ctx, table(B[B_STORED], nr * 4, t.R.stored)); HIPCHK(ctx, table(B[B_EQ2], nr, t.R.eq2)); HIPCHK(ctx, table(B[B_PQ], nr * 4, t.R.pq)); HIPCHK(ctx, table(B[B_PV], nr * 16, t.R.pv)); HIPCHK(ctx, table(B[B_SD], nr * 4, t.R.sd));
    uint64_t *ulen, *P; HIPCHK(ctx, table(B[B_ULEN], ((size_t)n_units + 2) * 8, ulen)); HIPCHK(ctx, table(B[B_P], ((size_t)n_units + 2) * 8, P)); HIPCHK(ctx, B[B_PVIN].ensure(nr * 16));
    HIPCHK(ctx, table(B[B_SCANTMP], std::max<size_t>(1024, (nr / SCAN_TILE + 2) * 16), t.scantmp));
    const uint32_t ublocks = (n_units + 255) / 256; uint32_t* minmax; HIPCHK(ctx, table(B[B_MINMAX], ((size_t)ublocks + 2) * LENS_BLK * 4, minmax));
    hipLaunchKernelGGL(k_read_lens, dim3(ublocks), dim3(256), 0, S, b.T, t.R.len, t.R.stored, ulen, n_units, b.T.upr, minmax, b.dst, nu);
    KCHK(ctx, "k_read_lens");
    uint32_t* const uni = minmax + (size_t)ublocks * LENS_BLK;
    hipLaunchKernelGGL(k_lens_uniform, dim3(1), dim3(1024), 0, S, (const uint32_t*)minmax, ublocks, n_units, uni, nu);
    auto prefix_scans = [&]() {
        scan_exclusive<uint64_t>(S, ulen, P, n_units, (uint64_t*)t.scantmp, 1, uni);
        scan_exclusive<uint32_t>(S, t.R.len, t.R.pq, n_reads, (uint32_t*)t.scantmp, 1, uni);
    };
    bool have_scans = ctx->mixed_lengths;
    if (have_scans) prefix_scans();
    hipLaunchKernelGGL(k_fill_pq, dim3(n_reads / 256 + 1), dim3(256), 0, S, t.R.pq, n_reads, (const uint32_t*)uni, nu, b.T.upr);
    const uint64_t cap64 = (uint64_t)(b.nbytes[0] + b.nbytes[1]) / (2ull * b.a->chunk_bases) + 3;
    const uint32_t cap_chunks = cut.cap_chunks = (uint32_t)std::min<uint64_t>(cap64, (uint64_t)n_units + 1);
    HIPCHK(ctx, B[B_FIRST].ensure(((size_t)cap_chunks + 2) * 4));
    memset(&t.C, 0, sizeof t.C);
    t.C.first = B[B_FIRST].as<uint32_t>();
    if (b.a->carry_bases && !b.scan_only) return rfq_fail(ctx, RFQ_E_ARG, "carry_bases is for the plan pass (rfq_scan_batch): an encode starts on a chunk boundary");
    if (b.a->carry_bases >= b.a->chunk_bases) return rfq_fail(ctx, RFQ_E_ARG, "carry_bases must be < chunk_bases");
    for (;;) {
        hipLaunchKernelGGL(k_partition, dim3(1), dim3(1024), 0, S, (const uint64_t*)(P + 1), n_units, b.T.upr, b.a->chunk_bases, b.a->carry_bases, b.fin ? 1 : 0,
                           (const uint32_t*)minmax, ublocks, t.C.first, cap_chunks + 1, b.dst, (const uint32_t*)uni, have_scans ? 1 : 0, nu);
        KCHK(ctx, "k_partition");
        HIPCHK(ctx, ctx->fetch(&b.hs, b.dst, sizeof b.hs, S));
        HIPCHK(ctx, ctx->fetch_sync(S));
        if (have_scans || !(b.hs.err & DE_NEED_SCAN)) break;
        ctx->mixed_lengths = true; have_scans = true; prefix_scans();
    }
    b.hs.err &= ~(uint32_t)DE_NEED_SCAN;
    ctx->timer.end(S);
    if (cut.lazy) {
        if (b.hs.err & (DE_INDEX_RETRY | DE_UNITS_GUESS | DE_NEED_SCAN)) { ctx->lazy_block = true; if (b.hs.err & DE_NEED_SCAN) ctx->mixed_lengths = true;
                return RFQ_AGAIN_LAZY; }
        if (b.hs.err & DE_HAS_CR) return b.nm ? rfq_fail(ctx, RFQ_E_HIP, "internal: '\\r' in normalised text") : RFQ_NEED_NORM;
        for (int s = 0; s < b.nstreams; s++) { cut.nlines[s] = b.hs.idx_lines[s]; cut.nrec[s] = cut.nlines[s] / 4; }
        n_units = b.hs.idx_units_true; n_reads = n_units * b.T.upr; b.T.n_reads = n_reads;
        if (n_units == 0) return empty_result(ctx, res);
    }
    { double r = 0.0; for (int s = 0; s < b.nstreams; s++) if (b.nbytes[s]) r = std::max(r, (double)cut.nrec[s] / (double)b.nbytes[s]); if (r > 0.0) ctx->rec_per_byte = r; }
    if (b.hs.err & DE_EMPTY_LINE) {
        if (!b.nm) return RFQ_NEED_NORM;
        again->unit_cap = b.hs.first_empty / b.T.upr; again->ended = true;
        return RFQ_AGAIN_ENDED;
    }
    if (b.hs.err & DE_INTERNAL) return rfq_fail(ctx, RFQ_E_HIP, "internal: reads of one length, units of several (k_lens_uniform / k_partition disagree)");
    if (b.hs.err & DE_QUAL_SHORT) return rfq_fail(ctx, RFQ_E_UNPINNED, "a quality line is shorter than its sequence line (the reference reads past the string: undefined)");
    cut.n_units = n_units; cut.n_reads = n_reads; cut.n_chunks = b.hs.n_chunks;
    if (cut.n_chunks > cap_chunks) return rfq_fail(ctx, RFQ_E_HIP, "internal: chunk table overflow (%u > %u)", cut.n_chunks, cap_chunks);
    if (cut.n_chunks == 0) return empty_result(ctx, res);
    cut.units_used = b.hs.n_units_used; cut.reads_used = cut.units_used * b.T.upr; cut.total_bases = b.hs.total_bases;
    cut.max_reads = std::max(b.hs.max_chunk_reads, 1u); cut.max_rec = b.hs.max_rec; cut.max_len = b.hs.max_len; cut.max_chunk_bases = b.hs.max_chunk_bases;
    return RFQ_OK;
}
static int enc_chunk_ends(rfq_ctx* ctx, const EncBatch& b, const EncCut& cut, const EncTables& t, rfq_encode_result* res) {
    hipStream_t S = ctx->stream;
    HIPCHK(ctx, ctx->b[B_P].ensure(((size_t)cut.n_chunks + 2) * 16));
    uint64_t* e1 = ctx->b[B_P].as<uint64_t>(); uint64_t* e2 = e1 + cut.n_chunks + 1;
    hipLaunchKernelGGL(k_chunk_ends, dim3((cut.n_chunks + 255) / 256), dim3(256), 0, S, b.T, (const uint32_t*)t.C.first, cut.n_chunks,
                       b.nm ? b.nm->onx[0] : nullptr, (b.nm && b.nstreams == 2) ? b.nm->onx[1] : nullptr, e1, e2);
    KCHK(ctx, "k_chunk_ends");
    ctx->scan_end[0].assign(cut.n_chunks, 0); ctx->scan_end[1].assign(b.nstreams == 2 ? cut.n_chunks : 0, 0);
    HIPCHK(ctx, ctx->fetch(ctx->scan_end[0].data(), e1, (size_t)cut.n_chunks * 8, S));
    if (b.nstreams == 2) HIPCHK(ctx, ctx->fetch(ctx->scan_end[1].data(), e2, (size_t)cut.n_chunks * 8, S));
    HIPCHK(ctx, ctx->fetch_sync(S));
    for (int s = 0; s < 2; s++) for (auto& v : ctx->scan_end[s]) v = consumed_of(b, s, v);
    res->n_chunks = cut.n_chunks; res->n_reads = cut.reads_used; res->n_bases = cut.total_bases; res->reserved = (int32_t)b.hs.unit_bases;
    res->consumed1 = (size_t)ctx->scan_end[0].back(); res->consumed2 = b.nstreams == 2 ? (size_t)ctx->scan_end[1].back() : 0;
    ctx->timer.collect();
    return RFQ_OK;
}
static void enc_form(const rfq_ctx* ctx, const EncCut& cut, EncForm& f, bool header) {
    const DevHeader& HH = ctx->h_hdr;
    if (!header) { f.kshift = 6; while (f.kshift >= 1 && ((uint64_t)cut.max_rec << f.kshift) + 64u > G2_CAP) f.kshift--; f.fast = f.kshift >= 1 && !ctx->opt.gather_old; return; }
    f.masks = f.fast && !ctx->opt.qual_bytes && HH.valid && (HH.flags & H_QUAL_BY_COL) && !(HH.flags & H_DONT_QUAL) && HH.n_normal >= 1u && HH.n_normal <= 4u;
    f.nqg = (std::min<uint32_t>(HH.n_normal, NPOS_SLOT) + PC_G - 1) / PC_G;
    f.coder_list = !f.masks && !(HH.flags & H_DONT_QUAL) && (HH.flags & H_QUAL_BY_COL) && HH.n_normal >= 1 && (ctx->opt.coder == 1 || (ctx->opt.coder == 0 && HH.n_normal >= 5));
}
static int header_errors(rfq_ctx* ctx, const EncBatch& b, const EncForm& f) {
    if (b.hs.err & (DE_BAD_QUAL | DE_BAD_BASE)) {
        const uint32_t g = b.hs.err_read, i = (uint32_t)b.hs.err_key; std::string ln;
        if (b.hs.err & DE_BAD_QUAL) { if (fetch_line(ctx, b.T, g, 3, ln)) return RFQ_E_HIP; return rfq_fail(ctx, RFQ_E_DATA, "bad quality value: %d", (int)(int8_t)ln[i]); }
        if (fetch_line(ctx, b.T, g, 1, ln)) return RFQ_E_HIP;
        const char c = ln[i];
        if (c == 'a' || c == 't' || c == 'c') return rfq_fail(ctx, RFQ_E_DATA, "repaq doesn't support FASTQ with lowercase bases (a/t/c/g)\nbut we get:\n%s", ln.c_str());
        return rfq_fail(ctx, RFQ_E_DATA, "repaq only supports FASTQ with uppercase bases (A/T/C/G/N)\nbut we get:\n%s", ln.c_str());
    }
    if (b.hs.err & DE_NO_QUAL_BINS) return rfq_fail(ctx, RFQ_E_DATA, "bad quality string, is this a valid FASTQ file?");
    if (f.make_header) { if (!ctx->h_hdr.valid) return rfq_fail(ctx, RFQ_E_HIP, "internal: header was not finalised"); ctx->have_hdr = true; ctx->hdr_on_device = true; }
    return RFQ_OK;
}
static int enc_tables(rfq_ctx* ctx, const EncBatch& b, const EncCut& cut, EncTables& t) {
    DBuf* B = ctx->b; ChunkTab& C = t.C; const size_t nc = t.nc = (size_t)cut.n_chunks + 2;
    HIPCHK(ctx, table(B[B_CFLAGS], nc * 4, C.flags)); HIPCHK(ctx, table(B[B_IL], nc * 4, C.il)); HIPCHK(ctx, table(B[B_NCOUNT], nc * 4, C.ncount)); HIPCHK(ctx, table(B[B_NMAP], nc * NMAP_WORDS * 4, C.nmap));
    HIPCHK(ctx, table(B[B_SCAP], nc * MAX_STREAMS * 4, C.scap)); HIPCHK(ctx, table(B[B_SOFF], nc * MAX_STREAMS * 8, C.soff)); HIPCHK(ctx, table(B[B_SSIZE], nc * MAX_STREAMS * 4, C.ssize));
    HIPCHK(ctx, table(B[B_XSIZE], nc * 4, C.xsize)); HIPCHK(ctx, table(B[B_YSIZE], nc * 4, C.ysize)); HIPCHK(ctx, table(B[B_QBASE], nc * 8, C.qbase)); HIPCHK(ctx, table(B[B_SBASE], nc * 8, C.sbase)); HIPCHK(ctx, table(B[B_PTOT], nc * sizeof(U4), C.ptot));
    HIPCHK(ctx, table(B[B_IMGSIZE], nc * 8, C.img_size)); HIPCHK(ctx, table(B[B_IMGOFF], nc * 8, C.img_off)); HIPCHK(ctx, table(B[B_CTOTAL], nc * 8, t.ctot)); HIPCHK(ctx, table(B[B_CBASE], nc * 8, t.cbase));
    HIPCHK(ctx, table(B[B_CTOTALN], nc * 8, t.ctot_n)); HIPCHK(ctx, table(B[B_CBASEN], nc * 8, t.cbase_n)); HIPCHK(ctx, table(B[B_LAYOUT], nc * sizeof(Layout), t.L)); HIPCHK(ctx, table(B[B_OVB], t.nr / 2 + 16, t.ovb));
    HIPCHK(ctx, B[B_HSTATS].ensure(sizeof(HdrStats) + 8192)); HIPCHK(ctx, table(ctx->d_hdr, sizeof(DevHeader), t.D)); HIPCHK(ctx, table(B[B_OVRAW], (size_t)(b.is_pe ? cut.n_units : 0) * 2 + 64, t.ovraw));
    HIPCHK(ctx, B[B_SCANTMP2].ensure(std::max<size_t>(4096, (t.nr / SCAN_TILE + 2) * 16 + (nc / SCAN_TILE + 2) * 8)));
    t.catbytes = (size_t)cut.total_bases + 64 * nc + 256; HIPCHK(ctx, table(B[B_QCAT], t.catbytes, t.qcat));
    HIPCHK(ctx, table(B[B_SPK], (t.catbytes >> 4) * 4 + 64, t.spk)); HIPCHK(ctx, table(B[B_SNM], (t.catbytes >> 4) * 2 + 64, t.snm));
    HIPCHK(ctx, table(B[B_ADJ], 3 * nc * 4, t.cbits)); t.cfail = t.cbits + nc; t.redo = t.cfail + nc;
    const uint32_t pc_max_steps = (cut.max_chunk_bases + 4095u) / 4096u; t.n_seg = std::max(1u, (pc_max_steps + PC_SEG_STEPS - 1) / PC_SEG_STEPS);
    const size_t nsb = t.nsb = nc * MAX_STREAMS * (size_t)t.n_seg;
    HIPCHK(ctx, table(B[B_SEGB], nsb * 4, t.segb)); HIPCHK(ctx, table(B[B_SEGC], nsb * 4, t.segc)); HIPCHK(ctx, table(B[B_SEGM], nsb * 4, t.segm));
    return RFQ_OK;
}
static int enc_header(rfq_ctx* ctx, EncBatch& b, const EncCut& cut, EncTables& t, EncForm& f) {
    hipStream_t S = ctx->stream;
    const bool make_header = f.make_header = !ctx->have_hdr;
    const bool hdr_aside = f.hdr_aside = make_header && !b.is_pe && ctx->aux_ready();
    hipStream_t HS = hdr_aside ? ctx->aux : S;
    if (hdr_aside) { HIPCHK(ctx, hipEventRecord(ctx->ev_fork, S)); HIPCHK(ctx, hipStreamWaitEvent(HS, ctx->ev_fork, 0)); }
    ctx->timer.begin("header", S);
    if (!f.fast) hipLaunchKernelGGL(k_chunk_ids, dim3((cut.max_reads + 255) / 256, cut.n_chunks), dim3(256), 0, S, t.C, t.R);
    const uint32_t c0_reads = std::max(1u, std::min(cut.max_reads, cut.reads_used));
    if (!f.fast) hipLaunchKernelGGL(k_read_table, dim3((cut.n_reads + 255) / 256), dim3(256), 0, S, b.T, t.R, cut.n_reads);
    else if (make_header) hipLaunchKernelGGL(k_read_table, dim3((c0_reads + 255) / 256), dim3(256), 0, S, b.T, t.R, c0_reads);
    if (hdr_aside) { HIPCHK(ctx, hipEventRecord(ctx->ev_fork, S)); HIPCHK(ctx, hipStreamWaitEvent(HS, ctx->ev_fork, 0)); }
    HdrStats* H = ctx->b[B_HSTATS].as<HdrStats>();
    const uint32_t hb = std::min<uint32_t>(1024, (c0_reads + 3) / 4);
    if (make_header) {
        hipLaunchKernelGGL(k_hdr_init, dim3(1), dim3(128), 0, HS, H);
        hipLaunchKernelGGL(k_hdr_stats, dim3(hb), dim3(256), 0, HS, b.T, t.R, (const uint32_t*)t.C.first, H);
        hipLaunchKernelGGL(k_hdr_q0, dim3(1), dim3(64), 0, HS, b.T, H);
        hipLaunchKernelGGL(k_hdr_pass2, dim3(hb), dim3(256), 0, HS, b.T, t.R, (const uint32_t*)t.C.first, H);
        if (b.is_pe) hipLaunchKernelGGL(k_hdr_pe, dim3((c0_reads / 2 + 255) / 256), dim3(256), 0, HS, b.T, t.R, (const uint32_t*)t.C.first, H);
        hipLaunchKernelGGL(k_hdr_finalize, dim3(1), dim3(64), 0, HS, b.T, H, t.D, b.is_pe ? 1 : 0, b.dst);
        if (f.fast) { hipLaunchKernelGGL(k_dense_order, dim3(1), dim3(64), 0, HS, (const HdrStats*)H, t.D); ctx->dense_ok = true; }
        KCHK(ctx, "k_hdr_*");
        if (hdr_aside) HIPCHK(ctx, hipEventRecord(ctx->ev_mid, HS));
    } else if (f.fast && !ctx->dense_ok) {
        hipLaunchKernelGGL(k_hdr_init, dim3(1), dim3(128), 0, S, H);
        hipLaunchKernelGGL(k_hdr_stats, dim3(hb), dim3(256), 0, S, b.T, t.R, (const uint32_t*)t.C.first, H);
        hipLaunchKernelGGL(k_dense_order, dim3(1), dim3(64), 0, S, (const HdrStats*)H, t.D);
        ctx->dense_ok = true;
        HIPCHK(ctx, ctx->fetch(ctx->h_hdr.dense, (const uint8_t*)t.D + offsetof(DevHeader, dense), 4, S));
        HIPCHK(ctx, ctx->fetch_sync(S));
    }
    if (make_header && f.fast) {
        if (hdr_aside) HIPCHK(ctx, hipStreamWaitEvent(S, ctx->ev_mid, 0));
        HIPCHK(ctx, ctx->fetch(&ctx->h_hdr, t.D, sizeof(DevHeader), S));
        { DevStatus h2; HIPCHK(ctx, ctx->fetch(&h2, b.dst, sizeof h2, S)); HIPCHK(ctx, ctx->fetch_sync(S)); b.hs.err |= h2.err; b.hs.err_read = h2.err_read; b.hs.err_key = h2.err_key; }
    }
    ctx->timer.end(S);
    if (f.fast && make_header) { const int rc = header_errors(ctx, b, f); if (rc) return rc; }
    if (f.fast) enc_form(ctx, cut, f, true);
    return RFQ_OK;
}
static void chunk_layout(hipStream_t Q, const EncBatch& b, const EncCut& cut, const EncTables& t, uint64_t* tmp, int exact) {
    hipLaunchKernelGGL(k_chunk_layout, dim3((cut.n_chunks + 63) / 64), dim3(64), 0, Q, b.T, t.R, t.C, (const DevHeader*)t.D, t.L, cut.n_chunks, exact, b.dst);
    scan_exclusive<uint64_t>(Q, t.C.img_size, t.C.img_off, cut.n_chunks, tmp, 1);
}
static int enc_gather_tiles(rfq_ctx* ctx, const EncBatch& b, const EncCut& cut, EncTables& t, EncForm& f, AuxGuard& guard) {
    hipStream_t S = ctx->stream; DBuf* B = ctx->b;
    const uint32_t np = cut.reads_used / 2;
    uint8_t *rflag, *rn; HIPCHK(ctx, table(B[B_RFLAG], (t.nr + 15) & ~(size_t)15, rflag)); HIPCHK(ctx, table(B[B_RN], (t.nr + 15) & ~(size_t)15, rn));
    ClearList z; memset(&z, 0, sizeof z);
    if (!(z.add(t.cbits, 2 * t.nc * 4, 0xFFFFFFFFu) && z.add(t.C.ncount, t.nc * 4, 0u) && z.add(t.C.nmap, t.nc * NMAP_WORDS * 4, 0u) && z.add(t.segb, t.nsb * 4, 0u) &&
          z.add(t.segm, t.nsb * 4, 0u) && z.add(t.segc, t.nsb * 4, 0xFFFFFFFFu) && z.add(rflag, t.nr, 0u) && z.add(rn, t.nr, 0u)))
        return rfq_fail(ctx, RFQ_E_HIP, "internal: more than %d regions in one clear list", CLEAR_MAX);
    clear_list(S, z);
    ctx->timer.begin("chunk_flags", S);
    hipLaunchKernelGGL(k_chunk_bases, dim3((cut.n_chunks + 255) / 256), dim3(256), 0, S, t.R, t.C, cut.n_chunks, 1);
    if (f.hdr_aside) HIPCHK(ctx, hipStreamWaitEvent(S, ctx->ev_mid, 0));
    ctx->timer.end(S);

    if (f.masks) { ctx->timer.begin("quality_masks", S); ctx->timer.end(S); }
    ctx->timer.begin("gather", S);
    const size_t nld = (size_t)(cut.total_bases >> 4) + cut.reads_used + 16;
    uint32_t* lpk; uint16_t* lnb; HIPCHK(ctx, table(B[B_LPK], nld * 4, lpk)); HIPCHK(ctx, table(B[B_LNB], nld * 2, lnb));
    const uint32_t K = 1u << f.kshift;
    const uint32_t bx = grid_x_for(cut.n_chunks, (cut.max_reads + K - 1) / K, 6u * ctx->n_cu);
    const uint32_t text4 = (uint32_t)((((uint64_t)cut.max_rec << f.kshift) + 64u + 15u) / 16u) + 8u;
    G2Planes M; M.planes = nullptr; M.rare = nullptr; M.pstride = 0; M.nd = 0; M.pw = (uint32_t)((((uint64_t)cut.max_len << f.kshift) + 31u) / 32u) + 2u;
    auto dyn_of = [&](uint32_t nd_) -> uint32_t { return text4 * 16u + (G2_REFN + G2_REFS + 32u) + 4u * nd_ * M.pw; };
    if (f.masks) {
        M.nd = std::min<uint32_t>(ctx->h_hdr.n_normal, 3u);
        if (M.nd == 3u && dyn_of(3u) + 64u > 26880u) M.nd = 2u;
        const size_t need_w = (t.catbytes >> 5) + 16, extra_w = t.nc * (1u + G2_RARE_LIST) / G2_PLANES + 16;
        if (B[B_QPLANE].cap / 4 / G2_PLANES < need_w + extra_w || ctx->qplane_stride < need_w) {
            HIPCHK(ctx, B[B_QPLANE].ensure((need_w + extra_w) * G2_PLANES * 4)); ctx->qplane_stride = B[B_QPLANE].cap / 4 / G2_PLANES - extra_w;
                    ctx->qplane_dirty = true;
        }
        if ((ctx->qplane_stride + extra_w) * G2_PLANES * 4 > B[B_QPLANE].cap) { ctx->qplane_stride = B[B_QPLANE].cap / 4 / G2_PLANES - extra_w;
                ctx->qplane_dirty = true; }
        uint32_t dmask = 0; for (uint32_t d = 0; d < M.nd; d++) dmask |= 1u << (ctx->h_hdr.dense[d] & 7u);
        if (ctx->qplane_mask & ~dmask) ctx->qplane_dirty = true;
        ctx->qplane_mask = dmask;
        M.planes = B[B_QPLANE].as<uint32_t>(); M.pstride = ctx->qplane_stride; M.rare = M.planes + G2_PLANES * M.pstride;
        if (ctx->qplane_dirty) HIPCHK(ctx, hipMemsetAsync(M.planes, 0, ((size_t)M.pstride * G2_PLANES + t.nc * (1u + G2_RARE_LIST)) * 4, S));
        ctx->qplane_dirty = true; ctx->qplane_nd = M.nd;
    }
    t.qplane = f.masks ? M.planes : nullptr;
    const uint32_t dyn = dyn_of(M.nd) + ctx->opt.g2_pad; (void)dyn;
    for (int phase = 1; phase <= (b.is_pe ? 2 : 1); phase++) {
        const uint32_t* only = phase == 2 ? (const uint32_t*)t.redo : (const uint32_t*)nullptr;
        if (phase == 2) hipLaunchKernelGGL(k_gather_redo_reset, dim3(cut.n_chunks), dim3(64), 0, S, only, t.segm, t.segc, t.n_seg,
                                           f.masks ? M.planes : (uint32_t*)nullptr, M.pstride, (const DevHeader*)t.D, M.nd, (const uint32_t*)t.R.pq, (const uint32_t*)t.C.first, (const uint64_t*)t.C.qbase);
        if (f.masks) hipLaunchKernelGGL(k_mask_bounds, dim3(cut.n_chunks), dim3(64), 0, S, (const uint32_t*)t.R.pq, (const uint32_t*)t.C.first, (const uint64_t*)t.C.qbase,
                M.planes, M.pstride, (const DevHeader*)t.D, M.nd, bx, only);
#define RFQ_G2_ARGS b.T, t.R, (const uint32_t*)t.C.first, (const uint64_t*)t.C.qbase, (const DevHeader*)t.D, t.qcat, lpk, lnb, rflag, \
                    rn, t.segm, t.segc, t.n_seg, f.kshift, t.cbits, t.cfail, only, text4, M
        if (f.masks && !b.is_pe && G2_SE_OK) hipLaunchKernelGGL((k_gather2<true, 0>), dim3(bx, cut.n_chunks), dim3(256), dyn, S, RFQ_G2_ARGS);
        else if (f.masks && b.a->paired == RFQ_PE_TWO_FILES && G2_SE_OK) hipLaunchKernelGGL((k_gather2<true, 1>), dim3(bx, cut.n_chunks), dim3(256), dyn, S, RFQ_G2_ARGS);
        else if (f.masks) hipLaunchKernelGGL(k_gather2<true>, dim3(bx, cut.n_chunks), dim3(256), dyn, S, RFQ_G2_ARGS);
        else hipLaunchKernelGGL(k_gather2<false>, dim3(bx, cut.n_chunks), dim3(256), dyn, S, RFQ_G2_ARGS);
#undef RFQ_G2_ARGS
        if (phase == 1) hipLaunchKernelGGL(k_chunk_flags_b, dim3(cut.n_chunks), dim3(64), 0, S, t.R, t.C, (const DevHeader*)t.D, b.is_pe ? 1 : 0, (const uint32_t*)t.cbits,
                (const uint32_t*)t.cfail, t.redo);
    }
    HIPCHK(ctx, table(B[B_SCRATCH], std::max<size_t>(B[B_SCRATCH].cap, (size_t)(f.masks ? cut.total_bases / 8 : cut.total_bases + cut.total_bases / 4) + t.nc * 4096 + 256), t.scratch));
    HIPCHK(ctx, table(B[B_SCRATCHN], std::max<size_t>(B[B_SCRATCHN].cap, (size_t)(cut.total_bases / 64) + t.nc * 1024 + 256), t.scratch_n));
    hipLaunchKernelGGL(k_stream_plan, dim3(cut.n_chunks), dim3(64), 0, S, t.R, t.C, (const DevHeader*)t.D, t.ctot, t.ctot_n, cut.n_chunks, (const uint32_t*)t.segm, t.n_seg, 1);
    scan_exclusive<uint64_t>(S, t.ctot, t.cbase, cut.n_chunks, (uint64_t*)t.scantmp, 1);
    hipLaunchKernelGGL(k_enc_totals, dim3(1), dim3(64), 0, S, t.C, (const uint64_t*)t.cbase, cut.n_chunks, 0, b.dst, (uint64_t)B[B_SCRATCH].cap);
    const bool aux_chain = f.aux_chain = ctx->aux_ready() && !ctx->opt.one_stream; hipStream_t A = aux_chain ? ctx->aux : S;
    if (aux_chain) { HIPCHK(ctx, hipEventRecord(ctx->ev_fork, S)); HIPCHK(ctx, hipStreamWaitEvent(A, ctx->ev_fork, 0)); guard.armed = true; }
    if (b.is_pe) {
        const OvLoose Z = { (const uint32_t*)t.R.pq, (const uint32_t*)lpk, (const uint16_t*)lnb, (const uint8_t*)rflag };
        const uint32_t ob = std::min<uint32_t>((np + 255) / 256, 65535u * 16u);
        if (cut.max_len <= 160u) hipLaunchKernelGGL((k_overlap<true, 160u>), dim3(ob), dim3(256), 0, A, b.T, Z, t.ovraw, np);
        else hipLaunchKernelGGL(k_overlap<true>, dim3(ob), dim3(256), 0, A, b.T, Z, t.ovraw, np);
    }
    if (aux_chain) { HIPCHK(ctx, hipEventRecord(ctx->ev_ovl, A)); f.coder_waits = true; }
    hipLaunchKernelGGL(k_chunk_prefix, dim3(cut.n_chunks), dim3(256), 0, A, b.T, t.R, t.C, (const DevHeader*)t.D, (const int16_t*)t.ovraw, t.ovb);
    {
        const uint32_t max_len = cut.max_rec / 2u;
        uint32_t rshift = 8; while (rshift && ((uint64_t)(max_len / 16u + 1u) << rshift) > SP_OWN) rshift--;
        uint32_t sx = grid_x_for(cut.n_chunks, (cut.max_reads >> rshift) + 1u, 8u * ctx->n_cu);
        hipLaunchKernelGGL(k_seqpack, dim3(sx, cut.n_chunks), dim3(256), aux_chain ? ctx->opt.sp_pad : 0u, A, (const uint32_t*)t.R.pq, (const uint32_t*)t.R.sd, (const U4*)t.C.ptot,
                (const uint32_t*)t.C.first, (const uint32_t*)t.C.il, (const int8_t*)t.ovb, (const DevHeader*)t.D,
                           (const uint64_t*)t.C.sbase, (const uint32_t*)lpk, (const uint16_t*)lnb, (const uint8_t*)rn, t.spk, t.snm,
                           t.C.ncount, t.C.nmap, t.segm, t.segc, t.n_seg, rshift);
    }
    uint64_t* tmp2 = B[B_SCANTMP2].as<uint64_t>() + (t.nr / SCAN_TILE + 2) * 2;
    hipLaunchKernelGGL(k_stream_plan, dim3(cut.n_chunks), dim3(64), 0, A, t.R, t.C, (const DevHeader*)t.D, t.ctot, t.ctot_n, cut.n_chunks, (const uint32_t*)t.segm, t.n_seg, 2);
    scan_exclusive<uint64_t>(A, t.ctot_n, t.cbase_n, cut.n_chunks, tmp2, 1);
    chunk_layout(A, b, cut, t, tmp2, 0);
    hipLaunchKernelGGL(k_enc_totals, dim3(1), dim3(64), 0, A, t.C, (const uint64_t*)t.cbase_n, cut.n_chunks, 2, b.dst, (uint64_t)B[B_SCRATCHN].cap);
    KCHK(ctx, "k_gather2");
    ctx->timer.end(S);
    return RFQ_OK;
}
static int enc_gather_bytes(rfq_ctx* ctx, EncBatch& b, const EncCut& cut, EncTables& t, EncForm& f) {
    hipStream_t S = ctx->stream; DBuf* B = ctx->b;
    uint64_t* const tmp = (uint64_t*)t.scantmp;
    HIPCHK(ctx, hipMemsetAsync(t.cbits, 0xFF, 2 * t.nc * 4, S));
    ctx->timer.begin("chunk_flags", S);
    hipLaunchKernelGGL(k_chunk_bases, dim3((cut.n_chunks + 255) / 256), dim3(256), 0, S, t.R, t.C, cut.n_chunks, 1);
    if (f.hdr_aside) HIPCHK(ctx, hipStreamWaitEvent(S, ctx->ev_mid, 0));
    const uint32_t fbx = std::max(1u, std::min<uint32_t>((cut.max_reads + 255) / 256, std::max(1u, 4096u / cut.n_chunks)));
    hipLaunchKernelGGL(k_chunk_flags_a, dim3(fbx, cut.n_chunks), dim3(256), 0, S, b.T, t.R, t.C, (const DevHeader*)t.D, b.is_pe ? 1 : 0, t.cbits, t.cfail);
    hipLaunchKernelGGL(k_chunk_flags_b, dim3(cut.n_chunks), dim3(64), 0, S, t.R, t.C, (const DevHeader*)t.D, b.is_pe ? 1 : 0, (const uint32_t*)t.cbits, (const uint32_t*)t.cfail,
            (uint32_t*)nullptr);
    if (b.is_pe) {
        const OvLoose noz = { nullptr, nullptr, nullptr, nullptr };
        const uint32_t ob = std::min<uint32_t>((cut.n_units + 255) / 256, 65535u * 16u);
// ... 42 lines not shown
                (const uint8_t*)t.qcat, t.scratch, (const uint64_t*)t.cbase, t.segb, (const int*)t.segc, (const uint32_t*)t.segm, t.n_seg, cut.n_chunks, b.dst);
        g0 = f.nqg; gn -= f.nqg;
        if (gn == 0) return RFQ_OK;
    }
    const uint64_t pc_blocks = (uint64_t)((cut.n_chunks + 7) / 8) * 8ull * gn * t.n_seg;
    if (pc_blocks > 0x7FFFFFFFull) return rfq_fail(ctx, RFQ_E_ARG, "batch too large for the position-coder grid");
    hipLaunchKernelGGL(k_pos_coder, dim3((uint32_t)pc_blocks), dim3(64), 0, Q, t.R, t.C, (const DevHeader*)t.D, (const uint8_t*)t.qcat, (const uint16_t*)t.snm,
                       t.scratch, (const uint64_t*)t.cbase, t.scratch_n, (const uint64_t*)t.cbase_n,
                       t.segb, (const int*)t.segc, (const uint32_t*)t.segm, t.n_seg, cut.n_chunks, f.nqg, g0, gn, b.dst,
                       (const uint32_t*)t.qplane, (uint64_t)ctx->qplane_stride);
    return RFQ_OK;
}
static int enc_coders(rfq_ctx* ctx, const EncBatch& b, const EncCut& cut, EncTables& t, const EncForm& f) {
    hipStream_t S = ctx->stream; DBuf* B = ctx->b;
    HIPCHK(ctx, table(B[B_XS], 3 * t.nr + 64, t.xs)); HIPCHK(ctx, table(B[B_YS], 3 * t.nr + 64, t.ys));
    ctx->timer.begin("pos_coder", S);
    const bool fork_coords = ctx->aux_ready();
    if (f.fast) {
        if (f.coder_waits) HIPCHK(ctx, hipStreamWaitEvent(S, ctx->ev_ovl, 0));
        { const int rc = launch_coder(ctx, S, b, cut, t, f, 0, f.nqg + 1); if (rc) return rc; }
        hipLaunchKernelGGL(k_coords, dim3(2, cut.n_chunks), dim3(64), 0, S, t.R, t.C, (const DevHeader*)t.D, t.xs, t.ys, b.dst);
    } else if (fork_coords) { HIPCHK(ctx, hipEventRecord(ctx->ev_fork, S)); HIPCHK(ctx, hipStreamWaitEvent(ctx->aux, ctx->ev_fork, 0)); }
    t.hdr_bytes = b.a->emit_header ? ctx->h_hdr.len : 0;
    if (b.a->d_out) { t.img = b.a->d_out; t.img_cap = b.a->out_cap; } else {
        const size_t nb_all = b.nbytes[0] + b.nbytes[1];
        const size_t want = f.fast ? std::max<size_t>(ctx->out_img.cap, (f.masks ? nb_all / 3 : nb_all - nb_all / 8) + (1u << 20)) : (size_t)(b.hs.image_bound + t.hdr_bytes + 64);
        HIPCHK(ctx, ctx->out_img.ensure(want)); t.img = ctx->out_img.as<uint8_t>(); t.img_cap = ctx->out_img.cap;
    }
    if (t.hdr_bytes) {
        if (t.img_cap < t.hdr_bytes) return rfq_fail(ctx, RFQ_E_NOSPACE, "output buffer too small for the header");
        HIPCHK(ctx, hipMemcpyAsync(t.img, ctx->h_hdr.bytes, t.hdr_bytes, hipMemcpyHostToDevice, S));
    }
    hipStream_t A2 = (f.fast ? f.aux_chain : fork_coords) ? ctx->aux : S;
    if (f.fast) { const int rc = launch_coder(ctx, A2, b, cut, t, f, f.nqg + 1, 1); if (rc) return rc; }
    else { hipLaunchKernelGGL(k_coords, dim3(2, cut.n_chunks), dim3(64), 0, A2, t.R, t.C, (const DevHeader*)t.D, t.xs, t.ys, b.dst); const int rc = launch_coder(ctx, S, b, cut, t, f, 0, f.nqg + 2); if (rc) return rc; }
    if (A2 != S) { HIPCHK(ctx, hipEventRecord(ctx->ev_join, A2)); HIPCHK(ctx, hipStreamWaitEvent(S, ctx->ev_join, 0)); }
    KCHK(ctx, "k_pos_coder");
    if (f.masks) {
        hipLaunchKernelGGL(k_rare_cleanup, dim3(cut.n_chunks), dim3(256), 0, S, t.qplane + G2_PLANES * ctx->qplane_stride, t.qplane, (uint64_t)ctx->qplane_stride,
                           (const DevHeader*)t.D, ctx->qplane_nd, (const uint32_t*)t.R.pq, (const uint32_t*)t.C.first, (const uint64_t*)t.C.qbase);
        ctx->qplane_dirty = false;
    }
    ctx->timer.end(S);
    return RFQ_OK;
}
static int enc_assemble(rfq_ctx* ctx, const EncBatch& b, const EncCut& cut, EncTables& t) {
    hipStream_t S = ctx->stream; DBuf* B = ctx->b;
    ctx->timer.begin("coords+layout", S);
    uint32_t *segd, *segs; HIPCHK(ctx, table(B[B_SEGD], t.nsb * 4, segd)); HIPCHK(ctx, table(B[B_SEGS], t.nsb * 4, segs));
    hipLaunchKernelGGL(k_pos_sizes, dim3(cut.n_chunks), dim3(64), 0, S, t.C, (const DevHeader*)t.D, (const uint32_t*)t.segb, (const uint32_t*)t.segm, t.n_seg, segd, segs);
    chunk_layout(S, b, cut, t, (uint64_t*)t.scantmp, 1);
    hipLaunchKernelGGL(k_enc_totals, dim3(1), dim3(64), 0, S, t.C, (const uint64_t*)t.cbase, cut.n_chunks, 1, b.dst, ~0ull);
    KCHK(ctx, "k_coords");
    ctx->timer.end(S);
    ctx->timer.begin("assemble", S);
    const uint32_t tail_bases = ((b.a->final && !b.a->flush_all) || b.ended) ? b.a->chunk_bases : 0u;
    const uint32_t bpc = grid_x_for(cut.n_chunks, 64u, 8u * ctx->n_cu);
    hipLaunchKernelGGL(k_assemble, dim3(bpc, cut.n_chunks), dim3(256), 0, S, b.T, t.R, t.C, (const DevHeader*)t.D, (const Layout*)t.L,
                       (const uint8_t*)t.qcat, (const uint32_t*)t.spk, (const uint8_t*)t.scratch, (const uint64_t*)t.cbase,
                       (const uint8_t*)t.scratch_n, (const uint64_t*)t.cbase_n,
                       (const uint8_t*)t.xs, (const uint8_t*)t.ys, (const int8_t*)t.ovb, t.img, t.img_cap, t.hdr_bytes,
                       b.a->file_off1, b.a->file_off2, b.a->nolb_from1, b.a->nolb_from2,
                       (const uint32_t*)t.segb, (const uint32_t*)segd, (const uint32_t*)segs, t.n_seg, b.dst,
                       tail_bases, cut.units_used, cut.nlines[0], cut.nlines[1], b.orig_n(0), b.orig_n(1));
    const uint32_t bx = std::max(1u, std::min<uint32_t>((cut.max_reads + 31) / 32, std::max(1u, 16384u / cut.n_chunks)));
    hipLaunchKernelGGL(k_assemble_names, dim3(bx, cut.n_chunks), dim3(256), 0, S, b.T, t.R, t.C, (const DevHeader*)t.D, (const Layout*)t.L, t.img, t.img_cap, t.hdr_bytes);
    KCHK(ctx, "k_assemble");
    ctx->timer.end(S);
    return RFQ_OK;
}
static int enc_verdict(rfq_ctx* ctx, EncBatch& b, const EncCut& cut, const EncTables& t, const EncForm& f, AuxGuard& guard, rfq_encode_result* res) {
    hipStream_t S = ctx->stream; DBuf* B = ctx->b;
    ctx->chunk_off.resize((size_t)cut.n_chunks + 1);
    HIPCHK(ctx, ctx->fetch(ctx->chunk_off.data(), t.C.img_off, ((size_t)cut.n_chunks + 1) * 8, S));
    uint32_t cons[2] = { 0, 0 };
    for (int s = 0; s < b.nstreams; s++) {
        const uint32_t recs = b.a->paired == RFQ_PE_TWO_FILES ? cut.units_used : cut.reads_used;
        if (b.nm) { cons[s] = 0; if (recs) HIPCHK(ctx, ctx->fetch(&cons[s], b.nm->onx[s] + 4 * (size_t)recs - 1, 4, S)); }
        else HIPCHK(ctx, ctx->fetch(&cons[s], b.T.lo[s] + 4 * (size_t)recs, 4, S));
    }
    HIPCHK(ctx, ctx->fetch(&b.hs, b.dst, sizeof b.hs, S));
    HIPCHK(ctx, ctx->fetch_sync(S));
    guard.armed = false; ctx->timer.collect();
    if (b.hs.err & DE_COORD_RANGE) {
        const uint32_t c = (uint32_t)(b.hs.coord_key >> 34), axis = (uint32_t)((b.hs.coord_key >> 33) & 1u), i = (uint32_t)(b.hs.coord_key & 0xFFFFFFFFu);
        uint32_t first = 0, ilv = 0, v = 0;
        HIPCHK(ctx, hipMemcpy(&first, t.C.first + c, 4, hipMemcpyDeviceToHost)); HIPCHK(ctx, hipMemcpy(&ilv, t.C.il + c, 4, hipMemcpyDeviceToHost));
        HIPCHK(ctx, hipMemcpy(&v, (axis ? t.R.y : t.R.x) + first + (size_t)i * (ilv ? 2 : 1), 4, hipMemcpyDeviceToHost));
        return rfq_fail(ctx, RFQ_E_DATA, "The X/Y coordinate cannot be larger than 2M, but we get: %u", v);
    }
    if ((b.hs.err & DE_TAIL_BLANK) && !b.nm) return RFQ_NEED_NORM;
    if (f.fast && ((b.hs.err & (DE_SCRATCH_SMALL | DE_SCRATCHN_SMALL)) || ((b.hs.err & (1u << 31)) && !b.a->d_out))) {
        HIPCHK(ctx, B[B_SCRATCH].ensure((size_t)b.hs.total_scratch + 256)); HIPCHK(ctx, B[B_SCRATCHN].ensure((size_t)b.hs.total_scratch_n + 256));
        if (!b.a->d_out) HIPCHK(ctx, ctx->out_img.ensure((size_t)(b.hs.image_bound + t.hdr_bytes + 64)));
        ctx->retried_room = true; return RFQ_RETRY_ROOM;
    }
    if (b.hs.err & DE_QUAL_OVERFLOW) return rfq_fail(ctx, RFQ_E_UNPINNED, "quality payload exceeds the reference's 1.5x scratch buffer (reference heap overflow, SURVEY.md App. C Q6)");
    if (b.hs.err & DE_CORRUPT) return rfq_fail(ctx, RFQ_E_HIP, "internal: a stream exceeded its scratch capacity");
    if (b.hs.err & (1u << 31)) return rfq_fail(ctx, RFQ_E_NOSPACE, "output buffer too small: need %llu bytes", (unsigned long long)(b.hs.total_image + t.hdr_bytes));
    for (auto& o : ctx->chunk_off) o += t.hdr_bytes;
    res->d_rfq = t.img; res->rfq_len = (size_t)(b.hs.total_image + t.hdr_bytes); res->n_chunks = cut.n_chunks; res->n_reads = cut.reads_used; res->n_bases = cut.total_bases;
    res->consumed1 = (size_t)consumed_of(b, 0, cons[0]); res->consumed2 = b.nstreams == 2 ? (size_t)consumed_of(b, 1, cons[1]) : 0;
    res->h_chunk_off = ctx->chunk_off.data();
    return RFQ_OK;
}
static int encode_impl(rfq_ctx* ctx, const rfq_encode_args* a, rfq_encode_result* res, const NormMap* nm, EncAgain* again, bool scan_only, const uint32_t* skip) {
    EncBatch b = {}; EncCut cut = {}; EncTables t = {}; AuxGuard guard = { ctx, false }; int rc;
    memset(res, 0, sizeof *res); res->input_ended = again->ended ? 1 : 0;
    b.a = a; b.nm = nm; b.skip = skip; b.scan_only = scan_only; b.ended = again->ended; b.unit_cap = again->unit_cap;
    b.fin = a->final || again->ended || a->flush_all; b.is_pe = a->paired != RFQ_SE;
    if (a->chunk_bases == 0) return rfq_fail(ctx, RFQ_E_ARG, "chunk_bases must be >= 1");
    const int nstreams = b.nstreams = a->paired == RFQ_PE_TWO_FILES ? 2 : 1;
    b.fq[0] = a->d_fq1; b.fq[1] = nstreams == 2 ? a->d_fq2 : nullptr;
    b.nbytes[0] = a->n1 > skip[0] ? a->n1 : 0; b.nbytes[1] = nstreams == 2 ? (a->n2 > skip[1] ? a->n2 : 0) : 0;
    for (int s = 0; s < nstreams; s++) {
        if (b.nbytes[s] >= 0xFFFFFFF0ull) return rfq_fail(ctx, RFQ_E_ARG, "a FASTQ stream of one batch must be < 4 GiB (got %zu bytes); split at record boundaries",
                b.nbytes[s]);
        if (b.nbytes[s] && !b.fq[s]) return rfq_fail(ctx, RFQ_E_ARG, "null FASTQ pointer");
        if (((uintptr_t)b.fq[s]) & 15u) return rfq_fail(ctx, RFQ_E_ARG, "FASTQ device pointers must be 16-byte aligned");
    }
    ctx->timer.reset();
    ctx->pend.clear(); ctx->pin_used = 0;
    HIPCHK(ctx, hipSetDevice(ctx->device));
    if (ctx->retried_room) { ctx->timer.begin("retry_room", ctx->stream); ctx->timer.end(ctx->stream); ctx->retried_room = false; }
    HIPCHK(ctx, table(ctx->d_status, sizeof(DevStatus), b.dst));
    HIPCHK(ctx, fresh_status(ctx, b));
    if ((rc = enc_index(ctx, b, cut)) != RFQ_OK) return rc;
    if ((rc = enc_cut(ctx, b, cut, t, res, again)) != RFQ_OK || cut.n_chunks == 0) return rc;
    if (scan_only) return enc_chunk_ends(ctx, b, cut, t, res);
    EncForm f = {}; enc_form(ctx, cut, f, false);
    if ((rc = enc_tables(ctx, b, cut, t)) != RFQ_OK) return rc;
    if ((rc = enc_header(ctx, b, cut, t, f)) != RFQ_OK) return rc;
    if ((rc = f.fast ? enc_gather_tiles(ctx, b, cut, t, f, guard) : enc_gather_bytes(ctx, b, cut, t, f)) != RFQ_OK) return rc;
    if ((rc = enc_coders(ctx, b, cut, t, f)) != RFQ_OK) return rc;
    if ((rc = enc_assemble(ctx, b, cut, t)) != RFQ_OK) return rc;
    return enc_verdict(ctx, b, cut, t, f, guard, res);
}
static int encode_settled(rfq_ctx* ctx, const rfq_encode_args* a, rfq_encode_result* res, const NormMap* nm, bool scan_only, const uint32_t* skip) {
    for (int attempt = 0; attempt < 3; attempt++) {
        EncAgain g; int rc, lazy_repeats = 0;
        while ((rc = encode_impl(ctx, a, res, nm, &g, scan_only, skip)) == RFQ_AGAIN_LAZY || rc == RFQ_AGAIN_ENDED)
            if (rc == RFQ_AGAIN_LAZY && ++lazy_repeats > 1) return rfq_fail(ctx, RFQ_E_HIP, "internal: the index without a read-back ran again in the repeat it asked for");
        if (rc != RFQ_RETRY_ROOM) return rc;
    }
    return rfq_fail(ctx, RFQ_E_HIP, "internal: the stream arenas did not settle");
}

static void align_streams(const rfq_encode_args* a, rfq_encode_args& al, uint32_t (&skip)[2]) {
    al = *a; skip[0] = skip[1] = 0;
    if (a->n1 && a->d_fq1) { skip[0] = (uint32_t)((uintptr_t)a->d_fq1 & 15u); al.d_fq1 = a->d_fq1 - skip[0]; al.n1 = a->n1 + skip[0];
            al.file_off1 = a->file_off1 - skip[0]; }
    if (a->paired == RFQ_PE_TWO_FILES && a->n2 && a->d_fq2) { skip[1] = (uint32_t)((uintptr_t)a->d_fq2 & 15u); al.d_fq2 = a->d_fq2 - skip[1]; al.n2 = a->n2 + skip[1];
            al.file_off2 = a->file_off2 - skip[1]; }
}
static int normalize_streams(rfq_ctx* ctx, const rfq_encode_args* a, rfq_encode_args& a2, NormMap& nm) {
    memset(&nm, 0, sizeof nm); a2 = *a;
    const uint8_t* p; size_t pn; int rc;
    if ((rc = normalize_stream(ctx, a->d_fq1, a->n1, a->file_off1, a->final != 0, 0, nm, &p, &pn)) != RFQ_OK) return rc;
    a2.d_fq1 = p; a2.n1 = pn;
    if (a->paired == RFQ_PE_TWO_FILES) {
        if ((rc = normalize_stream(ctx, a->d_fq2, a->n2, a->file_off2, a->final != 0, 1, nm, &p, &pn)) != RFQ_OK) return rc;
        a2.d_fq2 = p; a2.n2 = pn;
    }
    return RFQ_OK;
}
#define RFQ_SLICE ((size_t)3 << 30)
static void slice_limits(const rfq_ctx* ctx, size_t& slice, size_t& lim) {
    const size_t slice_env = ctx->opt.slice_bytes;
    slice = slice_env ? slice_env : RFQ_SLICE; lim = slice_env ? slice_env : 0xFFFFFFF0ull - 16;
}
static int encode_one(rfq_ctx* ctx, const rfq_encode_args* a, rfq_encode_result* res, bool scan_only) {
    rfq_encode_args al; uint32_t skip[2];
    align_streams(a, al, skip);
    int rc = encode_settled(ctx, &al, res, nullptr, scan_only, skip);
    if (rc != RFQ_NEED_NORM) return rc;
    NormMap nm; rfq_encode_args a2; const uint32_t noskip[2] = { 0, 0 };
    if ((rc = normalize_streams(ctx, a, a2, nm)) != RFQ_OK) return rc;
    rc = encode_settled(ctx, &a2, res, &nm, scan_only, noskip);
    return rc == RFQ_NEED_NORM ? rfq_fail(ctx, RFQ_E_HIP, "internal: normalised text still needs normalisation") : rc;
}

static int encode_or_scan(rfq_ctx* ctx, const rfq_encode_args* a, rfq_encode_result* res, bool scan_only) {
    if (!ctx || !a || !res) return RFQ_E_ARG;
    memset(res, 0, sizeof *res);
    ctx->err.clear();
    if (a->paired < 0 || a->paired > 2) return rfq_fail(ctx, RFQ_E_ARG, "paired must be RFQ_SE, RFQ_PE_TWO_FILES or RFQ_PE_INTERLEAVED");
    const bool two = a->paired == RFQ_PE_TWO_FILES;
    const size_t slice_env = ctx->opt.slice_bytes; size_t slice, lim;
    slice_limits(ctx, slice, lim);
    if (a->n1 < lim && (!two || a->n2 < lim)) return encode_one(ctx, a, res, scan_only);
    HIPCHK(ctx, hipSetDevice(ctx->device));
    size_t pos1 = 0, pos2 = 0, written = 0; bool first = true;
    std::vector<uint64_t> offs(1, 0), e1, e2; StageSums sums;
    uint32_t chunks = 0; uint64_t reads = 0, bases = 0; int ended = 0; int32_t ub = 0;
    for (;;) {
        const size_t r1 = a->n1 - pos1, r2 = two ? a->n2 - pos2 : 0;
        size_t t1 = std::min(r1, slice), t2 = std::min(r2, slice);
        if (two && (t1 == r1) != (t2 == r2)) { const size_t grow = slice_env ? 64 * slice_env : lim; if (t1 == r1) t2 = std::min(r2, grow); else t1 = std::min(r1, grow);
                }
        const bool last = t1 == r1 && t2 == r2;
        rfq_encode_args s = *a;
        s.d_fq1 = a->d_fq1 + pos1; s.n1 = t1; s.file_off1 = a->file_off1 + pos1;
        if (two) { s.d_fq2 = a->d_fq2 + pos2; s.n2 = t2; s.file_off2 = a->file_off2 + pos2; }
        s.final = last ? a->final : 0; s.flush_all = last ? a->flush_all : 0; s.emit_header = first ? a->emit_header : 0; s.carry_bases = first ? a->carry_bases : 0u;
        if (a->d_out) { s.d_out = a->d_out + written; s.out_cap = a->out_cap > written ? a->out_cap - written : 0; }
        rfq_encode_result r;
        const int rc = encode_one(ctx, &s, &r, scan_only);
        if (rc != RFQ_OK) return rc;
        sums.add(ctx->timer);
        if (scan_only) {
            for (uint32_t c = 0; c < r.n_chunks; c++) { e1.push_back(ctx->scan_end[0][c] + pos1); if (two) e2.push_back(ctx->scan_end[1][c] + pos2); }
        } else if (r.rfq_len) {
            if (!a->d_out) {
                HIPCHK(ctx, ctx->out_acc.ensure_keep(written + r.rfq_len + 64, written, ctx->stream));
                HIPCHK(ctx, hipMemcpyAsync(ctx->out_acc.as<uint8_t>() + written, r.d_rfq, r.rfq_len, hipMemcpyDeviceToDevice, ctx->stream));
                HIPCHK(ctx, hipStreamSynchronize(ctx->stream));
            }
            for (uint32_t c = 1; c <= r.n_chunks; c++) offs.push_back(written + r.h_chunk_off[c]);
            if (first && r.n_chunks) offs[0] = r.h_chunk_off[0];
            written += r.rfq_len;
        }
        if (first) ub = r.reserved; else if (r.reserved != ub) ub = 0;
        chunks += r.n_chunks; reads += r.n_reads; bases += r.n_bases; pos1 += r.consumed1; pos2 += r.consumed2; first = false;
        if (r.input_ended) { ended = 1; break; }
        if (last) break;
        if (r.consumed1 == 0) return rfq_fail(ctx, RFQ_E_ARG, "no whole chunk inside %zu bytes of text: chunk_bases is too large for a sliced call", slice);
    }
    sums.publish(ctx->timer);
    res->n_chunks = chunks; res->n_reads = reads; res->n_bases = bases; res->consumed1 = pos1; res->consumed2 = pos2; res->input_ended = ended;
            res->reserved = scan_only ? ub : 0;
    if (scan_only) { ctx->scan_end[0] = e1; ctx->scan_end[1] = e2; return RFQ_OK; }
    ctx->chunk_off = offs; res->h_chunk_off = ctx->chunk_off.data();
    res->rfq_len = written; res->d_rfq = written ? (a->d_out ? a->d_out : ctx->out_acc.as<uint8_t>()) : nullptr;
    return RFQ_OK;
}
extern "C" int rfq_encode_batch(rfq_ctx* ctx, const rfq_encode_args* a, rfq_encode_result* res) { return encode_or_scan(ctx, a, res, false); }
extern "C" int rfq_scan_batch(rfq_ctx* ctx, const rfq_encode_args* a, rfq_scan_result* out) {
    if (!out) return RFQ_E_ARG;
    memset(out, 0, sizeof *out);
    rfq_encode_result r;
    const int rc = encode_or_scan(ctx, a, &r, true);
    if (rc != RFQ_OK) return rc;
    out->n_chunks = r.n_chunks; out->n_reads = r.n_reads; out->consumed1 = r.consumed1; out->consumed2 = r.consumed2; out->input_ended = r.input_ended;
            out->unit_bases = (uint32_t)r.reserved;
    out->h_end1 = r.n_chunks ? ctx->scan_end[0].data() : nullptr;
    out->h_end2 = (r.n_chunks && a->paired == RFQ_PE_TWO_FILES) ? ctx->scan_end[1].data() : nullptr;
    return RFQ_OK;
}
static int rows_text_impl(rfq_ctx* ctx, const rfq_rows_in* in, int32_t paired, uint8_t* d_out1, size_t cap1, uint8_t* d_out2, size_t cap2, bool size_only,
        rfq_rows_text_result* res) {
    memset(res, 0, sizeof *res);
    if (paired < 0 || paired > 2) return rfq_fail(ctx, RFQ_E_ARG, "paired must be RFQ_SE, RFQ_PE_TWO_FILES or RFQ_PE_INTERLEAVED");
    const bool two = paired == RFQ_PE_TWO_FILES; const int nt = two ? 2 : 1;
    const uint64_t n = in->n_rows;
    if (in->row_len == 0) return rfq_fail(ctx, RFQ_E_ARG, "row_len must be >= 1");
    if (in->base_mode != RFQ_ROWS_ASCII && in->base_mode != RFQ_ROWS_CODE) return rfq_fail(ctx, RFQ_E_ARG, "base_mode must be RFQ_ROWS_ASCII or RFQ_ROWS_CODE");
// ... 229 lines not shown
```

Before: 1.095 million MB/s.

## Reuse file-1 line index for file 2 when paired files mirror byte layout

When the two paired-end inputs have equal size and alignment, the encoder skips building the newline index for the second file and points its line-offset table at the first file's. The assumption is checked speculatively: the gather kernel confirms that file 2 has newlines at the borrowed record ends and counts control bytes per tile, and a new tail kernel compares newline and CR positions past the last used unit. If any check fails, the batch is re-encoded without mirroring and mirroring stays off for that file. This removes one full index pass over file 2, at the cost of extra verification work in the gather kernel and the risk of paying for a full re-encode on inputs that do not mirror.

```diff
diff --git a/repaq_amd/csrc/enc/gather_tiles.h b/repaq_amd/csrc/enc/gather_tiles.h
--- a/repaq_amd/csrc/enc/gather_tiles.h
+++ b/repaq_amd/csrc/enc/gather_tiles.h
@@ -59,7 +59,7 @@
         __builtin_amdgcn_global_load_lds((const __attribute__((address_space(1))) void*)(src + 16 * (size_t)i),
                 (__attribute__((address_space(3))) void*)(l4 + (i - (tid & 63u))), 16, 0, 0);
     if (nfull < ng && tid == 0) { uint8_t* const bytes = (uint8_t*)l4;
-            for (uint32_t k = 0; k < 16 && a0 + 16 * nfull + k < n; k++) bytes[16 * nfull + k] = src[16 * (size_t)nfull + k]; }
+            for (uint32_t k = 0; k < 16; k++) bytes[16 * nfull + k] = a0 + 16 * nfull + k < n ? src[16 * (size_t)nfull + k] : (uint8_t)0xFF; }
 }
 __device__ __forceinline__ void g2_stage(const Text& T, bool two, const G2Geo& g, uint4* buf4, uint32_t tid) {
     g2_stage1(T.fq[0], T.n[0], g.a00, g.end0, buf4, tid);
@@ -280,10 +280,35 @@
         }
     }
 }
+__device__ __forceinline__ void g2_mirror_ends(const Text& T, const uint8_t* tx, const G2Geo& g, uint32_t cur, uint32_t cnt, uint32_t* mirror_err) {
+    const uint32_t l = (uint32_t)lane_id(); bool bad = false;
+    if (l < cnt) {
+        int s_; uint32_t r_; read_loc(T, cur + l, s_, r_);
+        if (s_ == 1) {
+            const uint32_t* const p = t_lo(T, 1) + 4 * (size_t)r_; const uint32_t o = g.base1 - g.a01, n = T.n[1];
+            const uint32_t e1 = p[1], e2 = p[2], e3 = p[3], e4 = p[4];
+            bad = tx[o + e1 - 1u] != '\n' || tx[o + e2 - 1u] != '\n' || tx[o + e3 - 1u] != '\n' || (e4 - 1u < n && tx[o + e4 - 1u] != '\n');
+        }
+    }
+    if (__any(bad)) { if (l == 0u) atomicOr(mirror_err, (uint32_t)DE_MIRROR_FAIL); }
+}
 #define G2_PLANES 5u
 #define G2_PLANE_EXC 4u
 #define G2_RARE_LIST 255u
-struct G2Planes { uint32_t* planes; uint64_t pstride; uint32_t pw, nd; uint32_t* rare; };
+struct G2Planes { uint32_t* planes; uint64_t pstride; uint32_t pw, nd; uint32_t* rare; uint32_t* mirror_err; };
+__device__ __forceinline__ uint32_t ctl_flags4(uint32_t w) { return (w - 0x10101010u) & ~w & 0x80808080u; }
+__device__ __forceinline__ uint32_t ctl_count16(const uint4& q) {
+    return (uint32_t)__popc(ctl_flags4(q.x)) + (uint32_t)__popc(ctl_flags4(q.y)) + (uint32_t)__popc(ctl_flags4(q.z)) + (uint32_t)__popc(ctl_flags4(q.w));
+}
+__device__ __forceinline__ uint32_t g2_ctl_count(const uint4* l4, uint32_t head, uint32_t nb, uint32_t tid) {
+    const uint32_t ng = (nb + 15u) >> 4; uint32_t c = 0;
+    for (uint32_t i0 = 0; i0 < ng; i0 += 256u) { const uint32_t i = i0 + tid; if (i < ng) c += ctl_count16(l4[i]); }
+    if (tid < 32u) {
+        const uint32_t k = tid & 15u, p = tid < 16u ? k : nb + k;
+        if (tid < 16u ? k < head : p < 16u * ng) c -= ((const uint8_t*)l4)[p] < 0x10u ? 1u : 0u;
+    }
+    return c;
+}
 __device__ __forceinline__ void g2_rare_or(uint32_t* __restrict__ gpl, uint64_t pstride, uint32_t* __restrict__ rare_c, uint32_t plane, uint32_t pos) {
     const uint32_t old = atomicOr(&gpl[(size_t)plane * pstride + (pos >> 5)], 1u << (pos & 31u));
     if (old == 0u) { const uint32_t k = atomicAdd(rare_c, 1u); if (k < G2_RARE_LIST) rare_c[1u + k] = (plane << 28) | (pos >> 5); }
@@ -366,7 +391,7 @@
     constexpr bool PE = PAIRED != 0;
     RFQ_DYN_SHARED(uint4, g2_lds);
     __shared__ uint32_t sh[MASKS ? 1 : G2_CNT]; __shared__ int sh_last[MASKS ? 1 : G2_CNT]; __shared__ uint8_t s_slot[MASKS ? 16 : 256];
-            __shared__ uint32_t s_r0[8], s_carry[4];
+            __shared__ uint32_t s_r0[8], s_carry[4], s_mctl;
     const uint32_t REFN = (text4 - 1u) * 16u, REFS = REFN + G2_REFN + 16u;
     uint32_t* const pl = (uint32_t*)(g2_lds + text4 + (G2_REFN + G2_REFS + 32u) / 16u);
     const uint32_t c = blockIdx.y;
@@ -384,6 +409,7 @@
         for (uint32_t i = tid; i < M.nd * M.pw; i += blockDim.x) pl[i] = 0u;
         if (tid < 4u) s_carry[tid] = 0u;
     }
+    if (tid == 0) s_mctl = 0u;
     const uint32_t f = first[c], e = first[c + 1];
     const bool two = PE && T.paired == 1, can0 = PE && T.paired != 0 && D->support_interleaved != 0, il = can0 && !redo;
     const uint32_t dpos = D->name2_diff_pos, dch = D->name2_diff_char;
@@ -400,6 +426,8 @@
     uint4* const buf4 = g2_lds + 1; const uint8_t* const tx = (const uint8_t*)buf4;
     G2Ref r0 = {}; G2Acc acc; acc.bits = CF_ALL; acc.fail = 0xFFFFFFFFu;
     const bool parse = !redo && gs < ge;
+    const bool mirror = (PAIRED == 1 || (PAIRED == -1 && !MASKS)) && two && !redo && M.mirror_err != nullptr;
+    uint32_t mwant = 0;
     if (parse) {
         uint32_t r_; read_loc(T, f, r0.s, r_); const uint32_t* p = t_lo(T, r0.s) + 4 * (size_t)r_;
         const uint32_t p0 = p[0], p1 = p[1], p2 = p[2], p3 = p[3];
@@ -430,13 +458,20 @@
         const G2Bound b3 = g2_bound(T, two, pq, tile_at(t + 3u));
         __syncthreads();
         qc.seg0 = qbeg / PC_SEG_POS;
-        if (parse && (uint32_t)wave_id() == (tix & 3u)) g2_parse(T, R, tx, REFN, REFS, g, r0, f, cur, cnt, can0, dpos, dch, acc);
+        if (parse && (uint32_t)wave_id() == (tix & 3u)) { g2_parse(T, R, tx, REFN, REFS, g, r0, f, cur, cnt, can0, dpos, dch, acc);
+                if (mirror) g2_mirror_ends(T, tx, g, cur, cnt, M.mirror_err); }
         if (MASKS) {
             if (tid < nd && s_carry[tid]) atomicOr(&pl[tid * M.pw], s_carry[tid]);
             g2_quals_masks(tx, m, part, P, pl, M.pw, qbeg & ~31u, nd, pat0, pat1, pat2, patm, D, qd, gpl, M.pstride, segm + (size_t)c * MAX_STREAMS * n_seg,
                     segc + (size_t)c * MAX_STREAMS * n_seg, n_seg, M.rare + (size_t)c * (1u + G2_RARE_LIST));
             g2_bases(tx, m, part, P, lpk, lnb, rflag, rn);
         } else g2_compose(tx, m, part, P, qd, lpk, lnb, rflag, rn, qc);
+        if (mirror) {
+            const uint32_t end1 = g.end1 < T.n[1] ? g.end1 : T.n[1];
+            const uint32_t mctl = wave_sum(g2_ctl_count(buf4 + g.base1 / 16u, b0.l1 - g.a01, end1 - g.a01, tid));
+            if ((tid & 63u) == 0 && mctl) atomicAdd(&s_mctl, mctl);
+            mwant += 2u * cnt - (g.end1 > T.n[1] ? 1u : 0u);
+        }
         __syncthreads();
         if (t + 1u < ntile) g2_stage(T, two, g2_geo(b1, b2, two), buf4, tid);
         if (MASKS) {
@@ -450,6 +485,10 @@
     if (parse) {
         const uint32_t bits = wave_and(acc.bits), fail = wave_min(acc.fail);
         if ((tid & 63u) == 0) { if (bits != CF_ALL) atomicAnd(&cbits[c], bits); if (fail != 0xFFFFFFFFu) atomicMin(&cfail[c], fail); }
+    }
+    if (mirror) {
+        __syncthreads();
+        if (tid == 0 && s_mctl != mwant) atomicOr(M.mirror_err, (uint32_t)DE_MIRROR_FAIL);
     }
 }
 __device__ __forceinline__ uint32_t dense_mask_of(const DevHeader* __restrict__ D, uint32_t nd) { uint32_t m = 0;
diff --git a/repaq_amd/csrc/enc/index.h b/repaq_amd/csrc/enc/index.h
--- a/repaq_amd/csrc/enc/index.h
+++ b/repaq_amd/csrc/enc/index.h
@@ -137,9 +137,10 @@
     if (blk == 0 && threadIdx.x == 0) lo[0] = skip;
 }
 __global__ void k_index_totals(const uint32_t* __restrict__ tot0, const uint32_t* __restrict__ tot1, const uint8_t* __restrict__ fq0, uint32_t n0, const uint8_t* __restrict__ fq1, uint32_t n1,
-                               uint32_t* lo0, uint32_t* lo1, int final_batch, int paired, uint32_t unit_cap, uint32_t guess, DevStatus* st) {
+                               uint32_t* lo0, uint32_t* lo1, int final_batch, int paired, uint32_t unit_cap, uint32_t guess, DevStatus* st, int mirror) {
     if (threadIdx.x || blockIdx.x) return;
     uint32_t rec[2] = { 0, 0 };
+    if (mirror && n0 > 0 && (fq0[n0 - 1] != '\n') != (fq1[n1 - 1] != '\n')) atomicOr(&st->err, (uint32_t)DE_MIRROR_FAIL);
     for (int s = 0; s < (paired == 1 ? 2 : 1); s++) {
         const uint32_t nl = s ? *tot1 : *tot0, n = s ? n1 : n0; const uint8_t* fq = s ? fq1 : fq0; uint32_t* lo = s ? lo1 : lo0;
         const uint32_t unterm = (final_batch && n > 0 && fq[n - 1] != '\n') ? 1u : 0u;
@@ -150,6 +151,26 @@
     if (units > unit_cap) units = unit_cap;
     st->idx_units_true = units; st->idx_units = units < guess ? units : guess;
     if (units > guess) atomicOr(&st->err, (uint32_t)DE_UNITS_GUESS);
+}
+__global__ void __launch_bounds__(256) k_mirror_tail(const uint8_t* __restrict__ fq0, const uint8_t* __restrict__ fq1, uint32_t n, const uint32_t* __restrict__ lo0,
+        uint32_t units_used, DevStatus* st) {
+    uint32_t start = lo0[4 * (size_t)units_used]; if (start > n) start = n;
+    bool bad = false;
+    for (uint64_t g = (uint64_t)(start >> 4) + (uint64_t)blockIdx.x * blockDim.x + threadIdx.x; g * 16ull < n; g += (uint64_t)gridDim.x * blockDim.x) {
+        const uint32_t base = (uint32_t)(g * 16ull), have = n - base < 16u ? n - base : 16u;
+        uint32_t lf0 = 0, lf1 = 0, cr0 = 0, cr1 = 0;
+        if (have == 16u) {
+            const uint4 a = *(const uint4*)(fq0 + base), b = *(const uint4*)(fq1 + base);
+            lf0 = eq_mask16c(a, 0x0A0A0A0Au); lf1 = eq_mask16c(b, 0x0A0A0A0Au); cr0 = eq_mask16c(a, 0x0D0D0D0Du); cr1 = eq_mask16c(b, 0x0D0D0D0Du);
+        } else for (uint32_t i = 0; i < have; i++) {
+            const uint8_t a = fq0[base + i], b = fq1[base + i];
+            if (a == '\n') lf0 |= 1u << i; if (b == '\n') lf1 |= 1u << i; if (a == '\r') cr0 |= 1u << i; if (b == '\r') cr1 |= 1u << i;
+        }
+        const uint32_t from = start > base ? start - base : 0u;
+        const uint32_t valid = from >= 16u ? 0u : (0xFFFFu << from) & 0xFFFFu;
+        if (((lf0 ^ lf1) | (cr0 ^ cr1)) & valid) bad = true;
+    }
+    if (__any(bad) && lane_id() == 0) atomicOr(&st->err, (uint32_t)DE_MIRROR_FAIL);
 }
 __global__ void k_line_tail(uint32_t* lo, uint32_t n_newlines, uint32_t n, int unterminated) {
     if (threadIdx.x == 0 && blockIdx.x == 0 && unterminated) lo[n_newlines + 1] = n + 1;
diff --git a/repaq_amd/csrc/rfq_api.hip b/repaq_amd/csrc/rfq_api.hip
--- a/repaq_amd/csrc/rfq_api.hip
+++ b/repaq_amd/csrc/rfq_api.hip
@@ -42,11 +42,12 @@
     else if (n == "RFQ_SP_PAD") { RFQ_OPT_NUM(0, 150000, "0 .. 150000 bytes of LDS") c->opt.sp_pad = set ? (uint32_t)num : d.sp_pad; }
     else if (n == "RFQ_POS_SEG") { if (set && v != "1024" && v != "2048") return rfq_fail(c, RFQ_E_ARG, "RFQ_POS_SEG is 1024 or 2048"); c->opt.pos_seg = set ? atoi(v.c_str()) : 0; }
     else if (n == "RFQ_SPEC") { if (set && v != "0" && v != "1") return rfq_fail(c, RFQ_E_ARG, "RFQ_SPEC is 0 or 1"); c->opt.no_spec = v == "0"; }
+    else if (n == "RFQ_MIRROR") { if (set && v != "0" && v != "1") return rfq_fail(c, RFQ_E_ARG, "RFQ_MIRROR is 0 or 1"); c->opt.no_mirror = v == "0"; }
     else return rfq_fail(c, RFQ_E_ARG, "unknown option %s", name);
 #undef RFQ_OPT_NUM
     return RFQ_OK;
 }
-static const char* const RFQ_OPTION_NAMES[] = { "RFQ_GATHER", "RFQ_QUAL", "RFQ_CODER", "RFQ_INDEX", "RFQ_IDX_TILES", "RFQ_STREAMS", "RFQ_SLICE_BYTES", "RFQ_SLICE_BASES", "RFQ_WALK", "RFQ_GW_SHIFT", "RFQ_MATERIALISE", "RFQ_TRACE", "RFQ_G2_PAD", "RFQ_SP_PAD", "RFQ_POS_SEG", "RFQ_SPEC" };
+static const char* const RFQ_OPTION_NAMES[] = { "RFQ_GATHER", "RFQ_QUAL", "RFQ_CODER", "RFQ_INDEX", "RFQ_IDX_TILES", "RFQ_STREAMS", "RFQ_SLICE_BYTES", "RFQ_SLICE_BASES", "RFQ_WALK", "RFQ_GW_SHIFT", "RFQ_MATERIALISE", "RFQ_TRACE", "RFQ_G2_PAD", "RFQ_SP_PAD", "RFQ_POS_SEG", "RFQ_SPEC", "RFQ_MIRROR" };
 extern "C" const char* rfq_option_name(int i) { return (i >= 0 && i < (int)(sizeof RFQ_OPTION_NAMES / sizeof RFQ_OPTION_NAMES[0])) ? RFQ_OPTION_NAMES[i] : nullptr; }
 extern "C" int rfq_get_option(const rfq_ctx* c, const char* name, char* out, size_t cap) {
     if (!c || !name || !out || !cap) return RFQ_E_ARG;
@@ -67,6 +68,7 @@
     else if (n == "RFQ_SP_PAD") v = o.sp_pad != d.sp_pad ? std::to_string(o.sp_pad) : "";
     else if (n == "RFQ_POS_SEG") v = o.pos_seg ? std::to_string(o.pos_seg) : "";
     else if (n == "RFQ_SPEC") v = o.no_spec ? "0" : "";
+    else if (n == "RFQ_MIRROR") v = o.no_mirror ? "0" : "";
     else return RFQ_E_ARG;
     if (v.size() + 1 > cap) return RFQ_E_NOSPACE;
     memcpy(out, v.c_str(), v.size() + 1);
diff --git a/repaq_amd/csrc/rfq_common.h b/repaq_amd/csrc/rfq_common.h
--- a/repaq_amd/csrc/rfq_common.h
+++ b/repaq_amd/csrc/rfq_common.h
@@ -50,6 +50,7 @@
 #define DE_SCRATCHN_SMALL  (1u << 13)
 #define DE_NEED_SCAN       (1u << 14)
 #define DE_UNITS_GUESS     (1u << 15)
+#define DE_MIRROR_FAIL     (1u << 16)
 #define DE_TAIL_BLANK      (1u << 9)
 
 struct DevHeader {
diff --git a/repaq_amd/csrc/rfq_ctx.h b/repaq_amd/csrc/rfq_ctx.h
--- a/repaq_amd/csrc/rfq_ctx.h
+++ b/repaq_amd/csrc/rfq_ctx.h
@@ -86,6 +86,7 @@
     uint32_t sp_pad = 0;
     bool no_spec = false;
     int  pos_seg = 0;
+    bool no_mirror = false;
 };
 struct rfq_ctx {
     RfqOpts opt;
@@ -134,7 +135,8 @@
     bool retried_room = false;
     bool mixed_lengths = false;
     bool dense_ok = false;
-    void new_file() { dense_ok = false; e3_pieces_failed = false; mixed_lengths = false; }
+    void new_file() { dense_ok = false; e3_pieces_failed = false; mixed_lengths = false; mirror_block = false; }
+    bool mirror_block = false, mirror_fell = false;
     bool qplane_dirty = true;
     uint32_t qplane_nd = 0, qplane_mask = 0;
     size_t qplane_stride = 0;
diff --git a/repaq_amd/csrc/rfq_encode.hip b/repaq_amd/csrc/rfq_encode.hip
--- a/repaq_amd/csrc/rfq_encode.hip
+++ b/repaq_amd/csrc/rfq_encode.hip
@@ -86,9 +86,11 @@
 }
 #define RFQ_AGAIN_LAZY 2
 #define RFQ_AGAIN_ENDED 4
+#define RFQ_AGAIN_MIRROR 5
 struct EncAgain { uint32_t unit_cap = ~0u; bool ended = false; };
 struct EncBatch {
-    const rfq_encode_args* a; const NormMap* nm; const uint32_t* skip; bool scan_only, ended, fin, is_pe; uint32_t unit_cap; int nstreams; const uint8_t* fq[2]; size_t nbytes[2]; Text T; DevStatus* dst; DevStatus hs;
+    const rfq_encode_args* a; const NormMap* nm; const uint32_t* skip; bool scan_only, ended, fin, is_pe;
+    bool mirror_ok, mirrored, mirror_proven; uint32_t unit_cap; int nstreams; const uint8_t* fq[2]; size_t nbytes[2]; Text T; DevStatus* dst; DevStatus hs;
     uint64_t orig_n(int s) const { return nm ? nm->orig_n[s] : nbytes[s]; }
 };
 struct EncCut {
@@ -120,6 +122,8 @@
     for (int s = 0; s < b.nstreams; s++) nidx[s] = (uint32_t)((b.nbytes[s] + idx_tiles * 16384u - 1) / (idx_tiles * 16384u));
     uint32_t n_newlines[2] = { 0, 0 }; uint8_t lastbyte[2] = { '\n', '\n' };
     bool one_pass = !ctx->opt.index_2pass;
+    const bool mirror = b.mirrored = b.mirror_ok && one_pass && b.nstreams == 2 && !b.nm && !ctx->opt.no_mirror && !ctx->mirror_block && nblk[0] != 0 &&
+                                     b.nbytes[0] == b.nbytes[1] && b.skip[0] == b.skip[1];
     const bool lazy_allowed = !ctx->lazy_block; ctx->lazy_block = false;
     bool lazy = one_pass && lazy_allowed && ctx->rec_per_byte > 0.0 && !ctx->mixed_lengths && b.unit_cap == ~0u && !b.ended;
     uint32_t guess_units = 0;
@@ -134,6 +138,7 @@
         size_t cap[2] = { 0, 0 };
         for (int s = 0; s < b.nstreams; s++) {
             if (!nblk[s]) continue;
+            if (mirror && s == 1) { if (!lazy) HIPCHK(ctx, ctx->fetch(&lastbyte[1], b.fq[1] + b.nbytes[1] - 1, 1, S)); continue; }
             cap[s] = std::max(B[B_LO0 + s].cap / 4, b.nbytes[s] / 16 + 4096);
             HIPCHK(ctx, B[B_LO0 + s].ensure(cap[s] * 4));
             HIPCHK(ctx, B[B_BLK0 + s].ensure((size_t)nidx[s] * 8 + 64));
@@ -150,13 +155,18 @@
         }
         if (lazy) {
             const uint32_t* t0 = (const uint32_t*)(B[B_BLK0].as<unsigned long long>() + nidx[0]) + 1;
-            const uint32_t* t1 = b.nstreams == 2 ? (const uint32_t*)(B[B_BLK1].as<unsigned long long>() + nidx[1]) + 1 : t0;
+            const uint32_t* t1 = b.nstreams == 2 && !mirror ? (const uint32_t*)(B[B_BLK1].as<unsigned long long>() + nidx[1]) + 1 : t0;
             hipLaunchKernelGGL(k_index_totals, dim3(1), dim3(64), 0, S, t0, t1, b.fq[0], (uint32_t)b.nbytes[0], b.fq[1], (uint32_t)b.nbytes[1], B[B_LO0].as<uint32_t>(),
-                               b.nstreams == 2 ? B[B_LO1].as<uint32_t>() : (uint32_t*)nullptr, b.a->final ? 1 : 0, (int)b.a->paired, b.unit_cap, guess_units, b.dst);
+                               b.nstreams == 2 ? B[mirror ? B_LO0 : B_LO1].as<uint32_t>() : (uint32_t*)nullptr, b.a->final ? 1 : 0, (int)b.a->paired, b.unit_cap, guess_units, b.dst,
+                               mirror ? 1 : 0);
             KCHK(ctx, "k_index_totals");
         } else {
             HIPCHK(ctx, ctx->fetch(&b.hs, b.dst, sizeof b.hs, S));
             HIPCHK(ctx, ctx->fetch_sync(S));
+            if (mirror) {
+                n_newlines[1] = n_newlines[0];
+                if ((b.hs.err & DE_INDEX_RETRY) || (lastbyte[0] != '\n') != (lastbyte[1] != '\n')) return RFQ_AGAIN_MIRROR;
+            }
         }
         if (!lazy && (b.hs.err & DE_INDEX_RETRY)) {
             one_pass = false;
@@ -194,6 +204,7 @@
     for (int s = 0; s < b.nstreams && !lazy; s++) {
         const int unterm = b.a->final && b.nbytes[s] > 0 && lastbyte[s] != '\n';
         cut.nlines[s] = n_newlines[s] + (unterm ? 1u : 0u); cut.nrec[s] = cut.nlines[s] / 4;
+        if (mirror && s == 1) continue;
         if (!one_pass || !nblk[s]) HIPCHK(ctx, B[B_LO0 + s].ensure(((size_t)cut.nlines[s] + 4) * 4));
         if (nblk[s]) {
             if (!one_pass) hipLaunchKernelGGL(k_line_offsets, dim3(nblk[s]), dim3(256), 0, S, B[B_BITMAP0 + s].as<uint64_t>(), B[B_BLK0 + s].as<uint32_t>(),
@@ -204,9 +215,10 @@
     }
     ctx->timer.end(S);
     if (lazy) { ctx->timer.begin("lazy_index", S); ctx->timer.end(S); }
+    if (mirror) { ctx->timer.begin("mirror_index", S); ctx->timer.end(S); }
     cut.lazy = lazy; cut.guess_units = guess_units;
     Text& T = b.T; memset(&T, 0, sizeof T);
-    for (int s = 0; s < 2; s++) { T.fq[s] = b.fq[s]; T.n[s] = (uint32_t)b.nbytes[s]; T.lo[s] = s < b.nstreams ? B[B_LO0 + s].as<uint32_t>() : nullptr;
+    for (int s = 0; s < 2; s++) { T.fq[s] = b.fq[s]; T.n[s] = (uint32_t)b.nbytes[s]; T.lo[s] = s < b.nstreams ? B[mirror ? B_LO0 : B_LO0 + s].as<uint32_t>() : nullptr;
             T.ot[s] = b.nm && s < b.nstreams ? b.nm->ot[s] : nullptr; }
     T.paired = b.a->paired; T.upr = b.a->paired == RFQ_SE ? 1u : 2u;
     return RFQ_OK;
@@ -256,6 +268,7 @@
     }
     b.hs.err &= ~(uint32_t)DE_NEED_SCAN;
     ctx->timer.end(S);
+    if (b.mirrored && (b.hs.err & DE_MIRROR_FAIL)) return RFQ_AGAIN_MIRROR;
     if (cut.lazy) {
         if (b.hs.err & (DE_INDEX_RETRY | DE_UNITS_GUESS | DE_NEED_SCAN)) { ctx->lazy_block = true; if (b.hs.err & DE_NEED_SCAN) ctx->mixed_lengths = true;
                 return RFQ_AGAIN_LAZY; }
@@ -382,6 +395,7 @@
 static int enc_gather_tiles(rfq_ctx* ctx, const EncBatch& b, const EncCut& cut, EncTables& t, EncForm& f, AuxGuard& guard) {
     hipStream_t S = ctx->stream; DBuf* B = ctx->b;
     const uint32_t np = cut.reads_used / 2;
+    if (b.mirrored && f.masks && !G2_SE_OK) return RFQ_AGAIN_MIRROR;
     uint8_t *rflag, *rn; HIPCHK(ctx, table(B[B_RFLAG], (t.nr + 15) & ~(size_t)15, rflag)); HIPCHK(ctx, table(B[B_RN], (t.nr + 15) & ~(size_t)15, rn));
     ClearList z; memset(&z, 0, sizeof z);
     if (!(z.add(t.cbits, 2 * t.nc * 4, 0xFFFFFFFFu) && z.add(t.C.ncount, t.nc * 4, 0u) && z.add(t.C.nmap, t.nc * NMAP_WORDS * 4, 0u) && z.add(t.segb, t.nsb * 4, 0u) &&
@@ -400,7 +414,7 @@
     const uint32_t K = 1u << f.kshift;
     const uint32_t bx = grid_x_for(cut.n_chunks, (cut.max_reads + K - 1) / K, 6u * ctx->n_cu);
     const uint32_t text4 = (uint32_t)((((uint64_t)cut.max_rec << f.kshift) + 64u + 15u) / 16u) + 8u;
-    G2Planes M; M.planes = nullptr; M.rare = nullptr; M.pstride = 0; M.nd = 0; M.pw = (uint32_t)((((uint64_t)cut.max_len << f.kshift) + 31u) / 32u) + 2u;
+    G2Planes M; M.planes = nullptr; M.rare = nullptr; M.pstride = 0; M.nd = 0; M.mirror_err = b.mirrored ? &b.dst->err : (uint32_t*)nullptr; M.pw = (uint32_t)((((uint64_t)cut.max_len << f.kshift) + 31u) / 32u) + 2u;
     auto dyn_of = [&](uint32_t nd_) -> uint32_t { return text4 * 16u + (G2_REFN + G2_REFS + 32u) + 4u * nd_ * M.pw; };
     if (f.masks) {
         M.nd = std::min<uint32_t>(ctx->h_hdr.n_normal, 3u);
@@ -609,6 +623,7 @@
     HIPCHK(ctx, ctx->fetch(&b.hs, b.dst, sizeof b.hs, S));
     HIPCHK(ctx, ctx->fetch_sync(S));
     guard.armed = false; ctx->timer.collect();
+    if (b.mirrored) { if (b.hs.err & DE_MIRROR_FAIL) return RFQ_AGAIN_MIRROR; b.mirror_proven = true; }
     if (b.hs.err & DE_COORD_RANGE) {
         const uint32_t c = (uint32_t)(b.hs.coord_key >> 34), axis = (uint32_t)((b.hs.coord_key >> 33) & 1u), i = (uint32_t)(b.hs.coord_key & 0xFFFFFFFFu);
         uint32_t first = 0, ilv = 0, v = 0;
@@ -631,10 +646,12 @@
     res->h_chunk_off = ctx->chunk_off.data();
     return RFQ_OK;
 }
-static int encode_impl(rfq_ctx* ctx, const rfq_encode_args* a, rfq_encode_result* res, const NormMap* nm, EncAgain* again, bool scan_only, const uint32_t* skip) {
+static int encode_attempt(rfq_ctx* ctx, const rfq_encode_args* a, rfq_encode_result* res, const NormMap* nm, EncAgain* again, bool scan_only, const uint32_t* skip, bool mirror_ok,
+        int* mirror) {
     EncBatch b = {}; EncCut cut = {}; EncTables t = {}; AuxGuard guard = { ctx, false }; int rc;
+    struct MirrorOut { const EncBatch& b; int* out; ~MirrorOut() { *out = b.mirrored ? (b.mirror_proven ? 2 : 1) : 0; } } mirror_out = { b, mirror };
     memset(res, 0, sizeof *res); res->input_ended = again->ended ? 1 : 0;
-    b.a = a; b.nm = nm; b.skip = skip; b.scan_only = scan_only; b.ended = again->ended; b.unit_cap = again->unit_cap;
+    b.a = a; b.nm = nm; b.skip = skip; b.scan_only = scan_only; b.ended = again->ended; b.unit_cap = again->unit_cap; b.mirror_ok = mirror_ok;
     b.fin = a->final || again->ended || a->flush_all; b.is_pe = a->paired != RFQ_SE;
     if (a->chunk_bases == 0) return rfq_fail(ctx, RFQ_E_ARG, "chunk_bases must be >= 1");
     const int nstreams = b.nstreams = a->paired == RFQ_PE_TWO_FILES ? 2 : 1;
@@ -650,18 +667,36 @@
     ctx->pend.clear(); ctx->pin_used = 0;
     HIPCHK(ctx, hipSetDevice(ctx->device));
     if (ctx->retried_room) { ctx->timer.begin("retry_room", ctx->stream); ctx->timer.end(ctx->stream); ctx->retried_room = false; }
+    if (ctx->mirror_fell) { ctx->timer.begin("mirror_fallback", ctx->stream); ctx->timer.end(ctx->stream); }
     HIPCHK(ctx, table(ctx->d_status, sizeof(DevStatus), b.dst));
     HIPCHK(ctx, fresh_status(ctx, b));
     if ((rc = enc_index(ctx, b, cut)) != RFQ_OK) return rc;
     if ((rc = enc_cut(ctx, b, cut, t, res, again)) != RFQ_OK || cut.n_chunks == 0) return rc;
     if (scan_only) return enc_chunk_ends(ctx, b, cut, t, res);
     EncForm f = {}; enc_form(ctx, cut, f, false);
+    if (b.mirrored) {
+        if (!f.fast) return RFQ_AGAIN_MIRROR;
+        hipLaunchKernelGGL(k_mirror_tail, dim3(64), dim3(256), 0, ctx->stream, b.fq[0], b.fq[1], (uint32_t)b.nbytes[0], (const uint32_t*)b.T.lo[0], cut.units_used, b.dst);
+        KCHK(ctx, "k_mirror_tail");
+    }
     if ((rc = enc_tables(ctx, b, cut, t)) != RFQ_OK) return rc;
     if ((rc = enc_header(ctx, b, cut, t, f)) != RFQ_OK) return rc;
     if ((rc = f.fast ? enc_gather_tiles(ctx, b, cut, t, f, guard) : enc_gather_bytes(ctx, b, cut, t, f)) != RFQ_OK) return rc;
     if ((rc = enc_coders(ctx, b, cut, t, f)) != RFQ_OK) return rc;
     if ((rc = enc_assemble(ctx, b, cut, t)) != RFQ_OK) return rc;
     return enc_verdict(ctx, b, cut, t, f, guard, res);
+}
+static int encode_impl(rfq_ctx* ctx, const rfq_encode_args* a, rfq_encode_result* res, const NormMap* nm, EncAgain* again, bool scan_only, const uint32_t* skip) {
+    const bool had_hdr = ctx->have_hdr, had_dense = ctx->dense_ok; int mirror = 0;
+    const int rc = encode_attempt(ctx, a, res, nm, again, scan_only, skip, !scan_only, &mirror);
+    if (mirror != 1 || rc == RFQ_AGAIN_LAZY) return rc;
+    if (!had_hdr) { ctx->have_hdr = false; ctx->hdr_on_device = false; memset(&ctx->h_hdr, 0, sizeof ctx->h_hdr); }
+    if (!had_dense) ctx->dense_ok = false;
+    if (rc != RFQ_OK) ctx->mirror_block = true;
+    ctx->mirror_fell = true; ctx->err.clear();
+    const int rc2 = encode_attempt(ctx, a, res, nm, again, scan_only, skip, false, &mirror);
+    if (rc2 < 0 && hipStreamSynchronize(ctx->stream) == hipSuccess) ctx->timer.collect();
+    return rc2;
 }
 static int encode_settled(rfq_ctx* ctx, const rfq_encode_args* a, rfq_encode_result* res, const NormMap* nm, bool scan_only, const uint32_t* skip) {
     for (int attempt = 0; attempt < 3; attempt++) {
@@ -699,6 +734,7 @@
 static int encode_one(rfq_ctx* ctx, const rfq_encode_args* a, rfq_encode_result* res, bool scan_only) {
     rfq_encode_args al; uint32_t skip[2];
     align_streams(a, al, skip);
+    ctx->mirror_fell = false;
     int rc = encode_settled(ctx, &al, res, nullptr, scan_only, skip);
     if (rc != RFQ_NEED_NORM) return rc;
     NormMap nm; rfq_encode_args a2; const uint32_t noskip[2] = { 0, 0 };
```

Measured after the change: 1.138 million MB/s, median of 6. 1.04x the previous value.
